# kalgeee/Uncertainty-Aware-Multimodal-Emotion-Recognition

Measured on AMD Instinct MI355X. Metric: samples/sec fwd+bwd at B=4096 (84/256/768-dim), higher is better.
Workload: dtype bf16; 1 GPU; configs[2]: fusion+DEER forward + MultiTaskDEERLoss + backward (dropout 0.3, gradients materialised in the flat buffer), B=4096/GPU, (B,84)+(B,256)+(B,768) bf16 feature blocks, random-init weights; optimiser step excluded as the metric defines (it maintains the packed weight copies and is timed separately); global_batch=4096, parallelism=single

## Files before the change

### uncertainty-aware-multimodal-emotion-recognition_amd/csrc/chain.h

```cpp
#pragma once
#include "common.h"
#include "nig.h"
#include "options.h"

namespace mmdeer {

constexpr int CHAIN_MAX_SEGS = 12;
constexpr int CHAIN_MAX_VECS = 16;
constexpr int CHAIN_VEC_FLOATS = 4864;

struct ChainSeg {
  const bf16_t* W;
  const float* bias;
  bf16_t* stash;
  const float* gamma;
  const float* beta;
  bf16_t* xln;
  float* out32;
  float* mean;
  float* rstd;
  int N, K, ldw;
  int kin_off, nout_off;
  int dcol_off;
  int ld_stash, nout;
  int relu, drop_site, drop_shift, end_layer;
  int mblocks;
  int in_aux;
  int row_group;
  int fold_groups;
  const bf16_t* mask_y;
  int ld_mask, mask_col0;
  float mask_scale;
  const float* lnb_gamma;
  const bf16_t* lnb_y;
  const float* lnb_mean;
  const float* lnb_rstd;
  bf16_t* lnb_dz;
  float* lnb_partial;
  float lnb_mask_scale;
  int residual;
  int res_add, res_dup;
  bf16_t* stash2;
  int stash_split;
};

struct ChainNig {
  int enabled;
  const bf16_t* e2;
  const bf16_t* w3;
  const float* evid;
  const float* targets;
  const float* stats;
  const float* gstats;
  int nblk;
  int nwp;
  bf16_t* dz2;
  float* partial_w;
  float* partial_b;
  float* loss_out;
  int* bin_counts;
  float mask_scale;
  LossCfg cfg;
};

struct ChainNigF {
  int enabled;
  const bf16_t* w3;
  const float* b3;
  int b3_stride;
  float* evid;
  float* nig_out;
  const float* targets;
  float* wstats;
};

struct ChainArgs {
  const bf16_t* X;
  int ldx, K0;
  int B;
  int ts;
  int groups;
  long long group_stride;
  int nseg;
  DropCtx drop;
  const bf16_t* aux_video; const bf16_t* aux_audio; bf16_t* aux_audio_pad;
  int aux_ldv, aux_lda;
  unsigned long long* stamps;
  ChainNig nig;
  ChainNigF nigf;
  ChainSeg seg[CHAIN_MAX_SEGS];
};

inline int chain_samples_per_workgroup(int B) {
  const int forced = opt(OPT_CHAIN_TS);
  return forced == 16 || forced == 32 ? forced : (B > 4096 ? 32 : 16);
}
inline int chain_workgroups(int B) { const int m = chain_samples_per_workgroup(B); return (B + m - 1) / m; }
inline int chain_samples_per_workgroup(const struct ChainArgs& a);
inline int chain_workgroups_max(int B) { return (B + 15) / 16; }

struct RepackJob {
  const bf16_t* src;
  bf16_t* dst;
  int ld_src, rows, cols, cols_valid;
  int transpose;
  int layout;
  int ld_dst, dst_col;
  int gstart;
  int pad_;
};
constexpr int REPACK_MAX = 64;
struct RepackTable { int njobs; int pad_; RepackJob job[REPACK_MAX]; };
int check_repack(RepackTable& t);
int launch_repack(RepackTable& t, hipStream_t s);

void chain_seg_defaults(ChainSeg& s);
int launch_chain(const ChainArgs& a, hipStream_t stream);
inline int chain_samples_per_workgroup(const ChainArgs& a) { return a.ts == 16 || a.ts == 32 ? a.ts : chain_samples_per_workgroup(a.B); }

}
```

### uncertainty-aware-multimodal-emotion-recognition_amd/csrc/chain.hip

```cpp
#include <type_traits>
#include "gemm_kernel.inc"
#include "chain.h"
#include "options.h"
#include "nig_dev.h"
#include "ln_rows.h"

namespace mmdeer {
namespace {

template <int S>
__device__ __forceinline__ void wr_issue(const void* p) {
  static_assert(S >= 0 && S < 8, "ring slots 0..7");
  if constexpr (S == 0)
    asm volatile("global_load_dwordx4 v[248:251], %0, off\n\tglobal_load_dwordx4 v[252:255], %0, off offset:1024" ::"v"(p)
                 : "memory", "v248", "v249", "v250", "v251", "v252", "v253", "v254", "v255");
  else if constexpr (S == 1)
    asm volatile("global_load_dwordx4 v[240:243], %0, off\n\tglobal_load_dwordx4 v[244:247], %0, off offset:1024" ::"v"(p)
                 : "memory", "v240", "v241", "v242", "v243", "v244", "v245", "v246", "v247");
  else if constexpr (S == 2)
    asm volatile("global_load_dwordx4 v[232:235], %0, off\n\tglobal_load_dwordx4 v[236:239], %0, off offset:1024" ::"v"(p)
                 : "memory", "v232", "v233", "v234", "v235", "v236", "v237", "v238", "v239");
  else if constexpr (S == 3)
    asm volatile("global_load_dwordx4 v[224:227], %0, off\n\tglobal_load_dwordx4 v[228:231], %0, off offset:1024" ::"v"(p)
                 : "memory", "v224", "v225", "v226", "v227", "v228", "v229", "v230", "v231");
  else if constexpr (S == 4)
    asm volatile("global_load_dwordx4 v[216:219], %0, off\n\tglobal_load_dwordx4 v[220:223], %0, off offset:1024" ::"v"(p)
                 : "memory", "v216", "v217", "v218", "v219", "v220", "v221", "v222", "v223");
  else if constexpr (S == 5)
    asm volatile("global_load_dwordx4 v[208:211], %0, off\n\tglobal_load_dwordx4 v[212:215], %0, off offset:1024" ::"v"(p)
                 : "memory", "v208", "v209", "v210", "v211", "v212", "v213", "v214", "v215");
  else if constexpr (S == 6)
    asm volatile("global_load_dwordx4 v[200:203], %0, off\n\tglobal_load_dwordx4 v[204:207], %0, off offset:1024" ::"v"(p)
                 : "memory", "v200", "v201", "v202", "v203", "v204", "v205", "v206", "v207");
  else
    asm volatile("global_load_dwordx4 v[192:195], %0, off\n\tglobal_load_dwordx4 v[196:199], %0, off offset:1024" ::"v"(p)
                 : "memory", "v192", "v193", "v194", "v195", "v196", "v197", "v198", "v199");
}
template <int S, int N>
__device__ __forceinline__ void wr_take(u32x4& f0, u32x4& f1) {
  unsigned r0, r1, r2, r3, r4, r5, r6, r7;
#define CH_TAKE(b0, b1, b2, b3, b4, b5, b6, b7)                                                                                  \
  asm volatile("s_waitcnt vmcnt(%8)\n\tv_mov_b32 %0, v" #b0 "\n\tv_mov_b32 %1, v" #b1 "\n\tv_mov_b32 %2, v" #b2 "\n\tv_mov_b32 %3, v" #b3   \
               "\n\tv_mov_b32 %4, v" #b4 "\n\tv_mov_b32 %5, v" #b5 "\n\tv_mov_b32 %6, v" #b6 "\n\tv_mov_b32 %7, v" #b7 "\n\ts_nop 1"         \
               : "=v"(r0), "=v"(r1), "=v"(r2), "=v"(r3), "=v"(r4), "=v"(r5), "=v"(r6), "=v"(r7)                                 \
               : "n"(N)                                                                                                         \
               : "memory")
  if constexpr (S == 0) CH_TAKE(248, 249, 250, 251, 252, 253, 254, 255);
  else if constexpr (S == 1) CH_TAKE(240, 241, 242, 243, 244, 245, 246, 247);
  else if constexpr (S == 2) CH_TAKE(232, 233, 234, 235, 236, 237, 238, 239);
  else if constexpr (S == 3) CH_TAKE(224, 225, 226, 227, 228, 229, 230, 231);
  else if constexpr (S == 4) CH_TAKE(216, 217, 218, 219, 220, 221, 222, 223);
  else if constexpr (S == 5) CH_TAKE(208, 209, 210, 211, 212, 213, 214, 215);
  else if constexpr (S == 6) CH_TAKE(200, 201, 202, 203, 204, 205, 206, 207);
  else CH_TAKE(192, 193, 194, 195, 196, 197, 198, 199);
#undef CH_TAKE
  f0 = u32x4{r0, r1, r2, r3};
  f1 = u32x4{r4, r5, r6, r7};
}

__device__ __forceinline__ unsigned chain_drop_key(unsigned long long seed, unsigned long long off, int site) {
  unsigned k = mix32((unsigned)seed ^ 0x9E3779B9u);
  k = mix32(k ^ (unsigned)(seed >> 32));
  k = mix32(k ^ (unsigned)off);
  k = mix32(k ^ (unsigned)(off >> 32) ^ ((unsigned)site * 0x85EBCA6Bu));
  return k;
}

struct ChainSegK {
  const bf16_t* W;
  int in_aux, nkt;
  int ntiles, kindb;
  int end;
  int N;
  int vec_off, dcol_off, nout_off, site;
  int shift, relu, fold, mblocks;
  int rows_out, kin_off;
  float mask_scale; int has_bias;
  const bf16_t* mask_y;
  int ld_mask, mask_col0;
};
struct ChainEndK {
  bf16_t* stash; bf16_t* xln; float* out32; float* mean; float* rstd;
  int ld_stash, nout, gb_off, has_ln;
  const bf16_t* lnb_y;
  float lnb_mask_scale;
  int res_split;
  bf16_t* stash2;
};
struct ChainVecK {
  const float* src;
  int off, n4;
};
struct ChainRecK { ChainSegK seg; ChainEndK end; };
static_assert(sizeof(ChainSegK) == 96 && sizeof(ChainEndK) == 80 && sizeof(ChainVecK) == 16 && sizeof(ChainRecK) == 176, "table record sizes");

struct ChainKArgs {
  const bf16_t* X;
  int ldx, K0;
  int B, groups;
  long long group_stride;
  int nseg, nvec;
  DropCtx drop;
  unsigned long long* stamps;
  const bf16_t* aux_video; const bf16_t* aux_audio; bf16_t* aux_audio_pad;
  int aux_ldv, aux_lda;
  ChainRecK rec[CHAIN_MAX_SEGS];
  ChainVecK vec[CHAIN_MAX_VECS];
  ChainNig nig;
  ChainNigF nigf;
};
static_assert(__builtin_offsetof(ChainKArgs, rec) % 16 == 0, "tables must be 16-byte aligned");
static_assert(sizeof(ChainKArgs) <= 4096, "kernel arguments are limited to 4 KiB");

struct ChainLnOut {
  bf16_t* stash; bf16_t* xln; float* out32; float* mean; float* rstd;
  int ld_stash, gb_off;
};

__device__ __forceinline__ float half_sum(float v, int lane) { return ln_half_sum(v, lane); }

template <int NKT>
__device__ __forceinline__ void chain_ln(unsigned char* pan, int img, int r, bool valid, long long grow, int lane, const float* vec,
                                         const ChainLnOut& o_, const unsigned char* res) {
  constexpr int KD = NKT * 64, NC = NKT / 4;
  const f32x4* gam = reinterpret_cast<const f32x4*>(vec + o_.gb_off);
  const f32x4* bet = gam + KD / 4;
  const int l32 = lane & 31;
  bf16_t* stash = o_.stash;
  bf16_t* xln = o_.xln;
  float* out32 = o_.out32;
  const int lds_ = o_.ld_stash;
  unsigned char* cell[NC];
  u32x4 raw[NC];
#pragma unroll
  for (int j = 0; j < NC; ++j) {
    const int c = l32 + 32 * j;
    cell[j] = pan + (c >> 3) * img + r * 128 + (((c & 7) ^ (r & 7)) * 16);
    raw[j] = *reinterpret_cast<const u32x4*>(cell[j]);
    if (valid && stash) store_wt16(stash + grow * lds_ + c * 8, raw[j]);
  }
  float x[NC * 8], mu, rs;
  ln_row_stats<NC>(raw, lane, x, mu, rs);
#pragma unroll
  for (int j = 0; j < NC; ++j) {
    const int c = l32 + 32 * j;
    float o[8];
    ln_chunk_out(x + 8 * j, mu, rs, gam[2 * c], gam[2 * c + 1], bet[2 * c], bet[2 * c + 1], o);
    u32x4 packed{pack_bf2(o[0], o[1]), pack_bf2(o[2], o[3]), pack_bf2(o[4], o[5]), pack_bf2(o[6], o[7])};
    if (res) {
      const u32x4 h = *reinterpret_cast<const u32x4*>(res + (cell[j] - pan));
      const unsigned pw[4] = {packed.x, packed.y, packed.z, packed.w}, hw[4] = {h.x, h.y, h.z, h.w};
#pragma unroll
      for (int e = 0; e < 4; ++e) {
        o[2 * e] = __uint_as_float(pw[e] << 16) + __uint_as_float(hw[e] << 16);
        o[2 * e + 1] = __uint_as_float(pw[e] & 0xFFFF0000u) + __uint_as_float(hw[e] & 0xFFFF0000u);
      }
      packed = u32x4{pack_bf2(o[0], o[1]), pack_bf2(o[2], o[3]), pack_bf2(o[4], o[5]), pack_bf2(o[6], o[7])};
    }
    *reinterpret_cast<u32x4*>(cell[j]) = packed;
    if (valid) {
      const long long col = grow * KD + c * 8;
      store_wt16(xln + col, packed);
      if (out32) {
        store_wt16(out32 + col, f32x4{o[0], o[1], o[2], o[3]});
        store_wt16(out32 + col + 4, f32x4{o[4], o[5], o[6], o[7]});
      }
    }
  }
  if (valid && l32 == 0) { o_.mean[grow] = mu; o_.rstd[grow] = rs; }
}

struct ChainLnbIn {
  u32x4 y[2];
  float mu, rs;
};

template <int NKT>
__device__ __forceinline__ void chain_ln_bwd(unsigned char* pan, int img, int lane, int r, bool valid, long long grow, const float* gam,
                                             const ChainLnbIn& in, float ms, bf16_t* dz, float (&gacc)[NKT * 2], float (&bacc)[NKT * 2]) {
  constexpr int KD = NKT * 64, NC = NKT / 4;
  const int l32 = lane & 31;
  unsigned char* cell[NC];
  u32x4 draw[NC], yraw[NC], packed[NC];
  float gg[NC * 8];
#pragma unroll
  for (int j = 0; j < NC; ++j) {
    const int c = l32 + 32 * j;
    cell[j] = pan + (c >> 3) * img + r * 128 + (((c & 7) ^ (r & 7)) * 16);
    draw[j] = *reinterpret_cast<const u32x4*>(cell[j]);
    yraw[j] = in.y[j];
    const f32x4 g0 = *reinterpret_cast<const f32x4*>(gam + 8 * c), g1 = *reinterpret_cast<const f32x4*>(gam + 8 * c + 4);
    gg[8 * j] = g0.x; gg[8 * j + 1] = g0.y; gg[8 * j + 2] = g0.z; gg[8 * j + 3] = g0.w;
    gg[8 * j + 4] = g1.x; gg[8 * j + 5] = g1.y; gg[8 * j + 6] = g1.z; gg[8 * j + 7] = g1.w;
  }
  ln_bwd_row<NC>(draw, yraw, gg, in.mu, in.rs, ms, lane, valid ? 1.f : 0.f, packed, gacc, bacc);
#pragma unroll
  for (int j = 0; j < NC; ++j) {
    const int c = l32 + 32 * j;
    *reinterpret_cast<u32x4*>(cell[j]) = packed[j];
    if (valid) store_wt16(dz + grow * KD + c * 8, packed[j]);
  }
}

template <int NKT>
__device__ __forceinline__ void chain_ln_bwd_fold(float* red, int wave, int lane, int tid, const float (&gacc)[NKT * 2],
                                                  const float (&bacc)[NKT * 2], float* slab) {
  ln_bwd_fold16<NKT / 4>(red, wave, lane, tid, gacc, bacc, slab);
}

template <int MS>
__device__ __forceinline__ void chain_nig_head(const ChainNig& g, unsigned char* pin, float* scratch, int row0, int B, int tid, unsigned long long* stp) {
#ifdef MMDEER_STAMPS
#define NSTAMP(i) do { if (stp && blockIdx.x == 0 && tid == 0) stp[i] = __builtin_readcyclecounter(); } while (0)
#else
#define NSTAMP(i) do {} while (0)
#endif
  NSTAMP(110);
  float* sb = scratch + MS * 195;
  float (*gs)[NIG_NSTAT] = reinterpret_cast<float (*)[NIG_NSTAT]>(sb);     sb += 108;
  f32x4* const sdE = reinterpret_cast<f32x4*>(sb);                           sb += MS * 12;
  Finals& F = *reinterpret_cast<Finals*>(sb);                                sb += (sizeof(Finals) + 15) / 16 * 4;
  float* const ftmp = sb;
  static_assert((MS * 195 + 108 + MS * 12 + (sizeof(Finals) + 15) / 16 * 4 + NIG_FINALS_TMP) * 4 <= MS * 1024, "NIG head scratch exceeds the output panel");
  const int wave = tid >> 6, lane = tid & 63, q = lane & 3;
  const int qw = wave - (8 - 3 * (MS / 16));
  const bool quad_on = qw >= 0;
  const int d = quad_on ? qw % 3 : 0;
  const int r = quad_on ? 16 * (qw / 3) + (lane >> 2) : 0;
  const int b = row0 + r;
  const bool active = quad_on && b < B;
  const int bc = b < B ? b : B - 1;
  const long long o = (long long)bc * 3 + d;
  float w[4][16], x[16];
  f32x4 ev{0.f, 0.f, 0.f, 0.f};
  float y = 0.f;
  Nig n{0.f, 1.f, 2.f, 1.f};
  Terms t{};
  if (quad_on) {
#pragma unroll
    for (int c = 0; c < 4; ++c) load_chunk16<false>(g.w3, d * 256 + c * 64 + q * 16, w[c]);
    load_chunk16<false>(g.e2, (long long)bc * 192 + d * 64 + q * 16, x);
    ev = *reinterpret_cast<const f32x4*>(g.evid + o * 4);
    y = g.targets[o];
    n = nig_act(ev);
    t = loss_terms(n, y);
  }
  const int stat_n = g.gstats ? (int)g.gstats[3 * NIG_NSTAT] : B;
  NSTAMP(111);
  compute_finals(g.gstats ? g.gstats : g.stats, g.gstats ? 1 : g.nblk, stat_n, g.cfg, F, gs, ftmp, g.gstats ? 0 : g.nwp);
  NSTAMP(112);
  if (blockIdx.x == 0 && tid == 0) write_loss(F, g.loss_out, g.bin_counts);
  if (quad_on) {
    const f32x4 gr = loss_grad(n, t, d, stat_n, g.cfg, F);
    f32x4 dE{gr.x, gr.y * softplus_grad(ev.y), gr.z * softplus_grad(ev.z), gr.w * softplus_grad(ev.w)};
    if (!active) dE = f32x4{0.f, 0.f, 0.f, 0.f};
    float dz[16];
    float* xt = scratch + r * 195 + d * 64 + q * 16;
#pragma unroll
    for (int j = 0; j < 16; ++j) {
      xt[j] = active ? x[j] : 0.f;
      const float v = nig_dx(dE, w[0][j], w[1][j], w[2][j], w[3][j]);
      dz[j] = x[j] > 0.f ? v * g.mask_scale : 0.f;
    }
    if (active) store_chunk16<false>(g.dz2, (long long)b * 192 + d * 64 + q * 16, dz);
    unsigned char* prow = pin + d * (MS * 128) + (r >> 3) * 1024 + (r & 7) * 128;
#pragma unroll
    for (int h = 0; h < 2; ++h)
      *reinterpret_cast<nig_u32x4*>(prow + (((2 * q + h) ^ (r & 7)) * 16)) =
          nig_u32x4{pack_bf2(dz[8 * h], dz[8 * h + 1]), pack_bf2(dz[8 * h + 2], dz[8 * h + 3]), pack_bf2(dz[8 * h + 4], dz[8 * h + 5]),
                    pack_bf2(dz[8 * h + 6], dz[8 * h + 7])};
    if (q == 0) sdE[r * 3 + d] = dE;
  }
  asm volatile("s_waitcnt lgkmcnt(0)" ::: "memory");
  __builtin_amdgcn_s_barrier();
  NSTAMP(114);
  for (int e = tid; e < 768; e += 512) {
    const int dd = e >> 8, c = (e >> 6) & 3, j = e & 63;
    const float* sde = reinterpret_cast<const float*>(sdE) + dd * 4 + c;
    float acc0 = 0.f, acc1 = 0.f;
#pragma unroll 8
    for (int s = 0; s < MS; s += 2) {
      acc0 = fmaf(sde[12 * s], scratch[s * 195 + dd * 64 + j], acc0);
      acc1 = fmaf(sde[12 * s + 12], scratch[(s + 1) * 195 + dd * 64 + j], acc1);
    }
    g.partial_w[(long long)blockIdx.x * 768 + e] = acc0 + acc1;
  }
  if (tid < 12) {
    const float* sde = reinterpret_cast<const float*>(sdE) + tid;
    float bs = 0.f;
    for (int s = 0; s < MS; ++s) bs += sde[12 * s];
    g.partial_b[(long long)blockIdx.x * 12 + tid] = bs;
  }
}

template <int MS>
__device__ __forceinline__ void chain_nig_tail(const ChainNigF& g, const unsigned char* pan, int row0, int B, int tid) {
  const int wave = tid >> 6, lane = tid & 63, q = lane & 3;
  const int qw = wave - (8 - 3 * (MS / 16));
  if (qw < 0) return;
  const int d = qw % 3, blk = qw / 3;
  const int r = 16 * blk + (lane >> 2);
  const int b = row0 + r;
  const bool active = b < B;
  const int bc = active ? b : B - 1;
  float w[4][16], x[16];
#pragma unroll
  for (int c = 0; c < 4; ++c) load_chunk16<false>(g.w3, d * 256 + c * 64 + q * 16, w[c]);
  {
    const unsigned char* prow = pan + d * (MS * 128) + r * 128;
#pragma unroll
    for (int h = 0; h < 2; ++h) {
      const u32x4 raw = *reinterpret_cast<const u32x4*>(prow + (((2 * q + h) ^ (r & 7)) * 16));
      const unsigned dw[4] = {raw.x, raw.y, raw.z, raw.w};
#pragma unroll
      for (int e = 0; e < 4; ++e) { x[8 * h + 2 * e] = __uint_as_float(dw[e] << 16); x[8 * h + 2 * e + 1] = __uint_as_float(dw[e] & 0xFFFF0000u); }
    }
  }
  float a0 = 0.f, a1 = 0.f, a2 = 0.f, a3 = 0.f;
#pragma unroll
  for (int j = 0; j < 16; ++j) {
    a0 = fmaf(x[j], w[0][j], a0); a1 = fmaf(x[j], w[1][j], a1);
    a2 = fmaf(x[j], w[2][j], a2); a3 = fmaf(x[j], w[3][j], a3);
  }
  a0 = quad_sum(a0); a1 = quad_sum(a1); a2 = quad_sum(a2); a3 = quad_sum(a3);
  const float* bb = g.b3 + d * g.b3_stride;
  const f32x4 ev{a0 + bb[0], a1 + bb[1], a2 + bb[2], a3 + bb[3]};
  const Nig n = nig_act(ev);
  const bool writer = active && q == 0;
  if (writer) {
    *reinterpret_cast<f32x4*>(g.evid + ((long long)b * 3 + d) * 4) = ev;
    const float alea = n.beta / (n.alpha - 1.f);
    const float epis = n.beta / (n.nu * (n.alpha - 1.f));
    const long long o = (long long)b * 3 + d, plane = (long long)B * 3;
    float* out = g.nig_out;
    out[o] = n.mu; out[plane + o] = n.nu; out[2 * plane + o] = n.alpha; out[3 * plane + o] = n.beta;
    out[4 * plane + o] = alea; out[5 * plane + o] = epis; out[6 * plane + o] = alea + epis;
  }
  if (g.targets) {
    const float y = g.targets[(long long)bc * 3 + d];
    const Terms t = loss_terms(n, y);
    float* slab = g.wstats + ((long long)((row0 >> 4) + blk) * 3 + d) * NIG_NSTAT;
    float v[NIG_NSTAT];
    v[0] = writer ? t.logprob : 0.f; v[1] = writer ? t.reg : 0.f; v[2] = writer ? t.kla : 0.f; v[3] = writer ? t.klb : 0.f; v[4] = writer ? t.u : 0.f;
#pragma unroll
    for (int k = 0; k < 10; ++k) {
      const bool in = writer && t.bin == k;
      v[5 + k] = in ? t.conf : 0.f; v[15 + k] = in ? t.aerr : 0.f; v[25 + k] = in ? 1.f : 0.f;
    }
#pragma unroll
    for (int i = 0; i < NIG_NSTAT; ++i) {
      const float sm = wave_sum(v[i]);
      if (lane == 0) slab[i] = sm;
    }
  }
}

template <int D, int VECF, int TS>
__device__ __forceinline__ void chain_body(const ChainKArgs& a) {
  constexpr int MS = 16 * TS, LOG_MS = TS == 1 ? 4 : 5, FLY = 2 * D;
  constexpr int G = D == 8 ? 4 : D;
  constexpr int PAN = TS == 1 ? MS * 1536 : MS * 1024;
  constexpr int AUXB = TS == 1 ? MS * 768 : 0;
  constexpr int AUX = 2 * PAN, RED = AUX + AUXB, VEC = RED + 32768, TAB = VEC + VECF * 4;
  constexpr int SEG_BYTES = (int)sizeof(ChainRecK);
  constexpr int VEC0 = CHAIN_MAX_SEGS * SEG_BYTES;
  constexpr int TAB_BYTES = VEC0 + CHAIN_MAX_VECS * (int)sizeof(ChainVecK);
  static_assert(TAB_BYTES % 16 == 0 && TAB_BYTES / 16 <= 512, "one 16-byte chunk of the tables per thread");
  static_assert(TAB + TAB_BYTES <= 160 * 1024, "LDS budget");
  __shared__ __attribute__((aligned(1024))) unsigned char lds[TAB + TAB_BYTES];
  float* const vec = reinterpret_cast<float*>(lds + VEC);

  const int tid = threadIdx.x, lane = tid & 63;
  const int wave = __builtin_amdgcn_readfirstlane(tid >> 6);
  const int li = lane & 15, lg = lane >> 4;
  const int r8 = lane >> 3, kchunk = ((lane & 7) ^ r8) * 8;
  const int row0 = blockIdx.x * MS;
  const int B = a.B;
  const long long gstride = a.group_stride;
  const int nseg = a.nseg, nvec = a.nvec;
#ifdef MMDEER_STAMPS
  unsigned long long* const stamps = a.stamps;
  auto stamp = [&](int i) { if (stamps && blockIdx.x == 0 && tid == 0 && i < 512) stamps[i] = __builtin_readcyclecounter(); };
  auto wstamp = [&](int i) { if (stamps && blockIdx.x == 0 && lane == 0 && i < 512) stamps[i] = __builtin_readcyclecounter(); };
#else
  auto stamp = [&](int) {};
  auto wstamp = [&](int) {};
#endif
  stamp(0);

  const unsigned long long dseed = a.drop.seed;
  const unsigned long long doff = a.drop.offset + (a.drop.offset_dev ? *a.drop.offset_dev : 0ull);
  const unsigned dthresh = a.drop.thresh;
  const float dscale = a.drop.scale;

  auto grow_of = [&](int r) -> long long { return (long long)(r >> LOG_MS) * gstride + row0 + (r & (MS - 1)); };
  auto valid_of = [&](int r) -> bool { return row0 + (r & (MS - 1)) < B; };

  const auto& KA = *(const __attribute__((address_space(4))) ChainKArgs*)__builtin_amdgcn_kernarg_segment_ptr();
  u32x4 tabv{0u, 0u, 0u, 0u};
  if (tid < TAB_BYTES / 16) {
    const unsigned char* src = (const unsigned char*)__builtin_amdgcn_kernarg_segment_ptr() + __builtin_offsetof(ChainKArgs, rec) + 16 * tid;
    asm volatile("global_load_dwordx4 %0, %1, off" : "=v"(tabv) : "v"(src) : "memory");
  }
  int rows_in = a.groups * MS;
  const bool nig_in = a.nig.enabled != 0;
  if (!nig_in) {
    const int rg = rows_in >> 3, np = (a.K0 >> 6) * rg;
    const int img = rows_in * 128;
    for (int q = wave; q < np; q += 8) {
      const int image = q / rg, g8 = q - image * rg;
      const int r = g8 * 8 + r8;
      const long long gr = valid_of(r) ? grow_of(r) : (long long)(r >> LOG_MS) * gstride;
      lds_dma16(a.X + gr * a.ldx + image * 64 + kchunk, lds + image * img + g8 * 1024);
    }
  }
  const bool has_aux = AUXB != 0 && a.aux_video != nullptr;
  if (has_aux) {
    {
      const int image = wave >> 1, g8 = wave & 1;
      const int r = g8 * 8 + r8;
      const long long gr = valid_of(r) ? grow_of(r) : 0;
      lds_dma16(a.aux_video + gr * a.aux_ldv + image * 64 + kchunk, lds + AUX + image * (MS * 128) + g8 * 1024);
    }
  }
  stamp(1);
  const unsigned char* const tab = lds + TAB;
  bool tab_ready = false;
  auto sc = [](unsigned v) -> int { return __builtin_amdgcn_readfirstlane((int)v); };
  auto sp = [](unsigned lo, unsigned hi) -> unsigned long long {
    return ((unsigned long long)(unsigned)__builtin_amdgcn_readfirstlane((int)hi) << 32) | (unsigned)__builtin_amdgcn_readfirstlane((int)lo);
  };

  const int rot = blockIdx.x >> 3;
  const int rot2 = rot & 1, rot3 = rot % 3, rot4 = rot & 3;
  auto phys_tile = [&](int nt, int ntl) -> int {
    const int ph = nt + (ntl == 4 ? rot4 : ntl == 3 ? rot3 : ntl == 2 ? rot2 : 0);
    return ph >= ntl ? ph - ntl : ph;
  };

  int p_si = 0, p_nt = 0, p_kt = 0, p_nkt = 0, p_nv = 0, p_ntiles = 0, p_kb = 0;
  const unsigned char* p_W = nullptr;
  const unsigned char* p_cur = nullptr;
  auto p_tile = [&]() __attribute__((always_inline)) {
    const int ph = phys_tile(p_nt, p_ntiles);
    const int wt = p_kb ? ph * 4 + (wave & 3) : ph * 8 + wave;
    p_cur = p_W + ((long long)wt * p_nkt) * 2048 + lane * 16;
  };
  auto p_load = [&]() __attribute__((always_inline)) {
    if (tab_ready) {
      const u32x4* rec = reinterpret_cast<const u32x4*>(tab + p_si * SEG_BYTES);
      const u32x4 q0 = rec[0], q1 = rec[1];
      p_W = reinterpret_cast<const unsigned char*>(sp(q0.x, q0.y));
      p_nkt = sc(q0.w); p_ntiles = sc(q1.x); p_kb = sc(q1.y);
    } else {
      const auto& sk = KA.rec[p_si].seg;
      p_W = reinterpret_cast<const unsigned char*>(sk.W);
      p_nkt = sk.nkt; p_ntiles = sk.ntiles; p_kb = sk.kindb;
    }
    p_nv = (p_nkt + G - 1) / G * G;
    p_nt = 0;
    p_tile();
  };
  auto issue = [&](auto slotc) __attribute__((always_inline)) {
    wr_issue<decltype(slotc)::value>(p_cur);
    if (++p_kt < p_nkt) p_cur += 2048;
    if (p_kt == p_nv) {
      p_kt = 0;
      if (++p_nt == p_ntiles) {
        if (++p_si == nseg) p_si = 0;
        p_load();
      } else {
        p_tile();
      }
    }
  };
  for (int e = wave; e < nvec; e += 8) {
    const float* src = KA.vec[e].src;
    unsigned char* dst = lds + VEC + KA.vec[e].off * 4;
    const int n4 = KA.vec[e].n4;
    for (int j = 0; j * 64 < n4; ++j) {
      if (src) { if (j * 64 + lane < n4) lds_dma16(src + 4 * (j * 64 + lane), dst + j * 1024); }
      else if (j * 64 + lane < n4) *reinterpret_cast<f32x4*>(dst + j * 1024 + lane * 16) = f32x4{0.f, 0.f, 0.f, 0.f};
    }
  }
  p_load();
  issue(std::integral_constant<int, 0>{});
  issue(std::integral_constant<int, 1>{});
  if constexpr (D >= 4) { issue(std::integral_constant<int, 2>{}); issue(std::integral_constant<int, 3>{}); }
  if constexpr (D == 8) {
    issue(std::integral_constant<int, 4>{}); issue(std::integral_constant<int, 5>{});
    issue(std::integral_constant<int, 6>{}); issue(std::integral_constant<int, 7>{});
  }
  if (has_aux) {
#pragma unroll
    for (int q = 0; q < 2; ++q) {
      const int e = tid + 512 * q, r = e >> 6, dw = e & 63;
      unsigned v = 0u;
      if (dw * 2 < a.aux_lda && valid_of(r)) v = *reinterpret_cast<const unsigned*>(a.aux_audio + grow_of(r) * a.aux_lda + 2 * dw);
      const int chunk = dw >> 2;
      *reinterpret_cast<unsigned*>(lds + AUX + (4 + (chunk >> 3)) * (MS * 128) + r * 128 + (((chunk & 7) ^ (r & 7)) * 16) + (dw & 3) * 4) = v;
    }
  }
  if (nig_in) {
    chain_nig_head<MS>(a.nig, lds, reinterpret_cast<float*>(lds + PAN), row0, B, tid, a.stamps);
    stamp(115);
  }
  asm volatile("s_waitcnt vmcnt(%1)" : "+v"(tabv) : "n"(FLY) : "memory");
  if (tid < TAB_BYTES / 16) *reinterpret_cast<u32x4*>(lds + TAB + 16 * tid) = tabv;
  tab_ready = true;
  asm volatile("s_waitcnt lgkmcnt(0)" ::: "memory");
  __builtin_amdgcn_s_barrier();
  stamp(2);
  if (has_aux && tid < 256) {
    const int r = tid >> 4, c = tid & 15;
    const u32x4 v = *reinterpret_cast<const u32x4*>(lds + AUX + (4 + (c >> 3)) * (MS * 128) + r * 128 + (((c & 7) ^ (r & 7)) * 16));
    if (valid_of(r)) store_wt16(a.aux_audio_pad + grow_of(r) * 128 + c * 8, v);
  }

  unsigned char* pin = lds;
  unsigned char* pout = lds + PAN;
  const int swz0 = (lg ^ (li & 7)) * 16, swz1 = ((4 + lg) ^ (li & 7)) * 16;

  struct SegCtl { int in_aux, N, ntiles, vec_off, dcol_off, nout_off, site, shift, relu, fold, kin_off, rows_out, has_bias, ld_mask, mask_col0; float mask_scale; const bf16_t* mask_y; };

  auto seg_body = [&](auto mbc, auto kbc, auto nktc, auto h0c, const SegCtl& sg) __attribute__((always_inline)) -> int {
    constexpr int MB = decltype(mbc)::value;
    constexpr bool KB = decltype(kbc)::value;
    constexpr int NKT = decltype(nktc)::value;
    constexpr int H0 = decltype(h0c)::value;
    constexpr int NV = (NKT + G - 1) / G * G;
    constexpr bool FLIP = D == 8 && ((NV / G) & 1) != 0;
    const bool active = !KB || wave < 4;
    const int img_in = sg.in_aux ? MS * 128 : rows_in * 128, img_out = sg.rows_out * 128;
    constexpr bool AFR_REG = TS == 1;
    const unsigned char* const sa = (sg.in_aux ? lds + AUX : pin) + (sg.kin_off >> 6) * img_in + li * 128;
    u32x4 afr[AFR_REG ? NKT * 2 : 1][MB];
    if constexpr (AFR_REG) {
#pragma unroll
      for (int c = 0; c < NKT * 2; ++c)
#pragma unroll
        for (int i = 0; i < MB; ++i) afr[c][i] = *reinterpret_cast<const u32x4*>(sa + (c >> 1) * img_in + i * 2048 + ((c & 1) ? swz1 : swz0));
    }
    u32x4 fr[2][2][MB];
    auto frag_load = [&](auto ktc) __attribute__((always_inline)) {
      constexpr int kt = decltype(ktc)::value;
#pragma unroll
      for (int i = 0; i < MB; ++i) {
        fr[kt & 1][0][i] = *reinterpret_cast<const u32x4*>(sa + kt * img_in + i * 2048 + swz0);
        fr[kt & 1][1][i] = *reinterpret_cast<const u32x4*>(sa + kt * img_in + i * 2048 + swz1);
      }
    };
    const int site = sg.site, shift = sg.shift, relu = sg.relu, fold = sg.fold & 15, N = sg.N;
    const bool res_add = (sg.fold & 16) != 0, res_dup = (sg.fold & 32) != 0;
    const unsigned dkey = site >= 0 ? chain_drop_key(dseed, doff, site) : 0u;
    auto tile = [&](auto hc, int nti) __attribute__((always_inline)) {
      constexpr int HS = decltype(hc)::value * G;
      const int nt = phys_tile(nti, sg.ntiles);
      f32x4 acc[MB];
#pragma unroll
      for (int i = 0; i < MB; ++i) acc[i] = f32x4{0.f, 0.f, 0.f, 0.f};
      u32x2 mk[MB];
      const bf16_t* mask_y = sg.mask_y;
      if (mask_y && active) {
        const int n0m = sg.mask_col0 + (KB ? nt * 64 : nt * 128) + 16 * wave + 4 * lg;
#pragma unroll
        for (int i = 0; i < MB; ++i) {
          const int r = 16 * i + li;
          const long long gr = valid_of(r) ? grow_of(r) : (long long)(r >> LOG_MS) * gstride;
          const bf16_t* q = mask_y + gr * sg.ld_mask + n0m;
          asm volatile("global_load_dwordx2 %0, %1, off" : "=v"(mk[i]) : "v"(q) : "memory");
        }
      }
      auto stage = [&](auto ktc) __attribute__((always_inline)) {
        constexpr int kt = decltype(ktc)::value;
        constexpr int S = (HS + kt) % D;
        if constexpr (kt < NKT) {
          u32x4 f0{0u, 0u, 0u, 0u}, f1{0u, 0u, 0u, 0u};
          if (active) wr_take<S, FLY - 2>(f0, f1);
          else wait_vm<FLY - 2>();
          issue(std::integral_constant<int, S>{});
          if constexpr (!AFR_REG && kt + 1 < NKT) { if (active) frag_load(std::integral_constant<int, kt + 1>{}); }
          if (active) {
            if constexpr (AFR_REG) {
#pragma unroll
              for (int i = 0; i < MB; ++i) acc[i] = mma_chunk<bf16_t>(f0, afr[2 * kt][i], acc[i]);
#pragma unroll
              for (int i = 0; i < MB; ++i) acc[i] = mma_chunk<bf16_t>(f1, afr[2 * kt + 1][i], acc[i]);
            } else {
#pragma unroll
              for (int i = 0; i < MB; ++i) acc[i] = mma_chunk<bf16_t>(f0, fr[kt & 1][0][i], acc[i]);
#pragma unroll
              for (int i = 0; i < MB; ++i) acc[i] = mma_chunk<bf16_t>(f1, fr[kt & 1][1][i], acc[i]);
            }
          }
        } else {
          wait_vm<FLY - 2>();
          issue(std::integral_constant<int, S>{});
        }
      };
      if constexpr (!AFR_REG) { if (active) frag_load(std::integral_constant<int, 0>{}); }
      stage(std::integral_constant<int, 0>{});
      if constexpr (NV > 1) stage(std::integral_constant<int, 1>{});
      if constexpr (NV > 2) stage(std::integral_constant<int, 2>{});
      if constexpr (NV > 3) stage(std::integral_constant<int, 3>{});
      if constexpr (NV > 4) stage(std::integral_constant<int, 4>{});
      if constexpr (NV > 5) stage(std::integral_constant<int, 5>{});
      if constexpr (NV > 6) stage(std::integral_constant<int, 6>{});
      if constexpr (NV > 7) stage(std::integral_constant<int, 7>{});
      if constexpr (NV > 8) stage(std::integral_constant<int, 8>{});
      if constexpr (NV > 9) stage(std::integral_constant<int, 9>{});
      if constexpr (NV > 10) stage(std::integral_constant<int, 10>{});
      if constexpr (NV > 11) stage(std::integral_constant<int, 11>{});
      if (active) {
        const int n0 = (KB ? nt * 64 : nt * 128) + 16 * wave + 4 * lg;
        const f32x4 bias4 = sg.has_bias ? *reinterpret_cast<const f32x4*>(vec + sg.vec_off + n0) : f32x4{0.f, 0.f, 0.f, 0.f};
        const unsigned dcol = (unsigned)(sg.dcol_off + n0);
        const int colb = sg.nout_off + n0;
        if (mask_y) {
#pragma unroll
          for (int i = 0; i < MB; ++i) asm volatile("s_waitcnt vmcnt(%1)" : "+v"(mk[i]) : "n"(2 * NV < FLY ? 2 * NV : FLY) : "memory");
        }
#pragma unroll
        for (int i = 0; i < MB; ++i) {
          const int r = 16 * i + li;
          f32x4 v = acc[i] + bias4;
          if (relu) { v.x = fmaxf(v.x, 0.f); v.y = fmaxf(v.y, 0.f); v.z = fmaxf(v.z, 0.f); v.w = fmaxf(v.w, 0.f); }
          if (site >= 0) {
            const unsigned rk = ((unsigned)grow_of(r) * 0x9E3779B1u) ^ dkey;
            if (shift == 0) {
              v.x = mix32(rk ^ (dcol * 0x85EBCA77u)) < dthresh ? v.x * dscale : 0.f;
              v.y = mix32(rk ^ ((dcol + 1) * 0x85EBCA77u)) < dthresh ? v.y * dscale : 0.f;
              v.z = mix32(rk ^ ((dcol + 2) * 0x85EBCA77u)) < dthresh ? v.z * dscale : 0.f;
              v.w = mix32(rk ^ ((dcol + 3) * 0x85EBCA77u)) < dthresh ? v.w * dscale : 0.f;
            } else {
              const float f = mix32(rk ^ ((dcol >> shift) * 0x85EBCA77u)) < dthresh ? dscale : 0.f;
              v.x *= f; v.y *= f; v.z *= f; v.w *= f;
            }
          }
          if (mask_y) {
            const float ms = sg.mask_scale;
            const unsigned m0 = mk[i].x, m1 = mk[i].y;
            v.x = __uint_as_float(m0 << 16) > 0.f ? v.x * ms : 0.f; v.y = __uint_as_float(m0 & 0xFFFF0000u) > 0.f ? v.y * ms : 0.f;
            v.z = __uint_as_float(m1 << 16) > 0.f ? v.z * ms : 0.f; v.w = __uint_as_float(m1 & 0xFFFF0000u) > 0.f ? v.w * ms : 0.f;
          }
          int col = colb, orow = r;
          if (fold == 1) { col += (r >> LOG_MS) * N; orow = r & (MS - 1); }
          else if (fold == 2) { const int half = N >> 1, z = col >= half; col -= z * half; orow = r + z * MS; }
          else if (fold == 3) orow = r + MS;
          const int cell_off = (col >> 6) * img_out + orow * 128 + ((((col & 63) >> 3) ^ (orow & 7)) * 16) + (col & 4) * 2;
          if (res_add) {
            const u32x2 h = *reinterpret_cast<const u32x2*>(pin + cell_off + 4 * img_out);
            const unsigned p0 = pack_bf2(v.x, v.y), p1 = pack_bf2(v.z, v.w);
            v.x = __uint_as_float(p0 << 16) + __uint_as_float(h.x << 16); v.y = __uint_as_float(p0 & 0xFFFF0000u) + __uint_as_float(h.x & 0xFFFF0000u);
            v.z = __uint_as_float(p1 << 16) + __uint_as_float(h.y << 16); v.w = __uint_as_float(p1 & 0xFFFF0000u) + __uint_as_float(h.y & 0xFFFF0000u);
          }
          const u32x2 pk{pack_bf2(v.x, v.y), pack_bf2(v.z, v.w)};
          *reinterpret_cast<u32x2*>(pout + cell_off) = pk;
          if (res_dup) *reinterpret_cast<u32x2*>(pout + cell_off + 4 * img_out) = pk;
        }
      }
    };
    if constexpr (!FLIP) {
      for (int nti = 0; nti < sg.ntiles; ++nti) tile(std::integral_constant<int, H0>{}, nti);
      return H0;
    } else {
      for (int nti = 0; nti < sg.ntiles; nti += 2) {
        tile(std::integral_constant<int, H0>{}, nti);
        if (nti + 1 < sg.ntiles) tile(std::integral_constant<int, 1 - H0>{}, nti + 1);
      }
      return (sg.ntiles & 1) ? 1 - H0 : H0;
    }
  };

  int half = 0;
  u32x4 R[11];
  auto fetch_rec = [&](int si_) __attribute__((always_inline)) {
    const u32x4* rec = reinterpret_cast<const u32x4*>(tab + si_ * SEG_BYTES);
#pragma unroll
    for (int k = 0; k < 11; ++k) R[k] = rec[k];
  };
  fetch_rec(0);
  for (int si = 0; si < nseg; ++si) {
    const u32x4 q0 = R[0], q1 = R[1], q2 = R[2], q3 = R[3], q4 = R[4], q5 = R[5];
    const u32x4 e0 = R[6], e1 = R[7], e2 = R[8], e3 = R[9], e4 = R[10];
    const int nkt = sc(q0.w), kb = sc(q1.y), endi = sc(q1.z);
    SegCtl sg;
    sg.ntiles = sc(q1.x); sg.N = sc(q1.w); sg.in_aux = sc(q0.z);
    sg.vec_off = sc(q2.x); sg.dcol_off = sc(q2.y); sg.nout_off = sc(q2.z); sg.site = sc(q2.w);
    sg.shift = sc(q3.x); sg.relu = sc(q3.y); sg.fold = sc(q3.z);
    const int mb = sc(q3.w);
    sg.rows_out = sc(q4.x); sg.kin_off = sc(q4.y);
    sg.mask_scale = __uint_as_float((unsigned)sc(q4.z)); sg.has_bias = sc(q4.w);
    sg.mask_y = reinterpret_cast<const bf16_t*>(sp(q5.x, q5.y)); sg.ld_mask = sc(q5.z); sg.mask_col0 = sc(q5.w);
    bf16_t* const stash = reinterpret_cast<bf16_t*>(sp(e0.x, e0.y));
    bf16_t* const end_xln = reinterpret_cast<bf16_t*>(sp(e0.z, e0.w));
    float* const end_out32 = reinterpret_cast<float*>(sp(e1.x, e1.y));
    float* const end_mean = reinterpret_cast<float*>(sp(e1.z, e1.w));
    float* const end_rstd = reinterpret_cast<float*>(sp(e2.x, e2.y));
    const int ld_stash = sc(e2.z), nout = sc(e2.w);
    const int gb_off = sc(e3.x), has_ln = endi >= 0 ? sc(e3.y) : 0;
    const bf16_t* const end_lnb_y = reinterpret_cast<const bf16_t*>(sp(e3.z, e3.w));
    const float lms = __uint_as_float((unsigned)sc(e4.x));
    const int res_split = endi >= 0 ? sc(e4.y) : 0;
    bf16_t* const stash2 = reinterpret_cast<bf16_t*>(sp(e4.z, e4.w));
    ChainLnbIn lnb[TS];
#pragma unroll
    for (int ps = 0; ps < TS; ++ps) { lnb[ps].y[0] = lnb[ps].y[1] = u32x4{0u, 0u, 0u, 0u}; lnb[ps].mu = 0.f; lnb[ps].rs = 0.f; }
    auto lnb_fetch = [&]() __attribute__((always_inline)) {
      const bf16_t* ly = end_lnb_y;
      const float* lmean = end_mean;
      const float* lrstd = end_rstd;
#pragma unroll
      for (int ps = 0; ps < TS; ++ps) {
        const int r = 16 * ps + 2 * wave + (lane >> 5);
        const long long gr = valid_of(r) ? grow_of(r) : 0;
        const bf16_t* q = ly + gr * nout + (lane & 31) * 8;
        asm volatile("global_load_dwordx4 %0, %1, off" : "=v"(lnb[ps].y[0]) : "v"(q) : "memory");
        if (nout == 512) asm volatile("global_load_dwordx4 %0, %1, off offset:512" : "=v"(lnb[ps].y[1]) : "v"(q) : "memory");
        asm volatile("global_load_dword %0, %1, off" : "=v"(lnb[ps].mu) : "v"(lmean + gr) : "memory");
        asm volatile("global_load_dword %0, %1, off" : "=v"(lnb[ps].rs) : "v"(lrstd + gr) : "memory");
      }
    };
    if (TS == 1 && has_ln == 2) lnb_fetch();
    stamp(3 + 3 * si);
#define CH_SEG1(MBv, KBv, NKTv, Hv) seg_body(std::integral_constant<int, MBv>{}, std::integral_constant<bool, KBv>{}, std::integral_constant<int, NKTv>{}, std::integral_constant<int, Hv>{}, sg)
#define CH_SEG(MBv, KBv, NKTv) do { if constexpr (D == 8) { if (half) half = CH_SEG1(MBv, KBv, NKTv, 1); else half = CH_SEG1(MBv, KBv, NKTv, 0); } else CH_SEG1(MBv, KBv, NKTv, 0); } while (0)
    if (!kb) {
      if (mb == TS) {
        if (nkt == 8) CH_SEG(TS, false, 8); else if (nkt == 6) CH_SEG(TS, false, 6); else if (nkt == 4) CH_SEG(TS, false, 4);
        else if (nkt == 2) CH_SEG(TS, false, 2); else if (nkt == 1) CH_SEG(TS, false, 1);
        else { if constexpr (TS == 1) CH_SEG(TS, false, 12); }
      } else {
        if (nkt == 4) CH_SEG(2 * TS, false, 4); else if (nkt == 2) CH_SEG(2 * TS, false, 2); else CH_SEG(2 * TS, false, 1);
      }
    } else {
      if (mb == TS) { if (nkt == 4) CH_SEG(TS, true, 4); else CH_SEG(TS, true, 2); }
      else CH_SEG(2 * TS, true, 2);
    }
#undef CH_SEG
#undef CH_SEG1
    stamp(4 + 3 * si);
    fetch_rec(si + 1 < nseg ? si + 1 : 0);
    if (endi >= 0) {
      const int rows_out = sg.rows_out, img_out = rows_out * 128;
      wstamp(200 + 8 * si + wave);
      asm volatile("s_waitcnt lgkmcnt(0)" ::: "memory");
      __builtin_amdgcn_s_barrier();
      stamp(130 + 4 * si);
      if (has_ln == 2) {
        stamp(100);
        if constexpr (TS == 1) {
          if (2 * sg.ntiles * ((nkt + G - 1) / G * G) >= FLY)
            asm volatile("s_waitcnt vmcnt(%4)" : "+v"(lnb[0].y[0]), "+v"(lnb[0].y[1]), "+v"(lnb[0].mu), "+v"(lnb[0].rs) : "n"(FLY) : "memory");
          else
            asm volatile("s_waitcnt vmcnt(%4)" : "+v"(lnb[0].y[0]), "+v"(lnb[0].y[1]), "+v"(lnb[0].mu), "+v"(lnb[0].rs) : "n"(2 * G) : "memory");
        } else {
          lnb_fetch();
#pragma unroll
          for (int ps = 0; ps < TS; ++ps)
            asm volatile("s_waitcnt vmcnt(0)" : "+v"(lnb[ps].y[0]), "+v"(lnb[ps].y[1]), "+v"(lnb[ps].mu), "+v"(lnb[ps].rs) : : "memory");
        }
        stamp(101);
        bf16_t* dz = end_xln;
        float* slab = end_out32 + (long long)blockIdx.x * 2 * nout;
        if (stash) {
          const int nch = nout >> 3;
          for (int rr = wave; rr < rows_out; rr += 8) {
            if (!valid_of(rr)) continue;
            for (int cc = lane; cc < nch; cc += 64)
              store_wt16(stash + grow_of(rr) * ld_stash + cc * 8,
                         *reinterpret_cast<const u32x4*>(pout + (cc >> 3) * img_out + rr * 128 + (((cc & 7) ^ (rr & 7)) * 16)));
          }
          asm volatile("s_waitcnt lgkmcnt(0)" ::: "memory");
          __builtin_amdgcn_s_barrier();
        }
        stamp(102);
        if (nout == 512) {
          float gacc[16], bacc[16];
#pragma unroll
          for (int e = 0; e < 16; ++e) gacc[e] = bacc[e] = 0.f;
#pragma unroll
          for (int ps = 0; ps < TS; ++ps) {
            const int r = 16 * ps + 2 * wave + (lane >> 5);
            chain_ln_bwd<8>(pout, img_out, lane, r, valid_of(r), grow_of(r), vec + gb_off, lnb[ps], lms, dz, gacc, bacc);
          }
          stamp(104);
          chain_ln_bwd_fold<8>(reinterpret_cast<float*>(lds + RED), wave, lane, tid, gacc, bacc, slab);
        } else {
          float gacc[8], bacc[8];
#pragma unroll
          for (int e = 0; e < 8; ++e) gacc[e] = bacc[e] = 0.f;
#pragma unroll
          for (int ps = 0; ps < TS; ++ps) {
            const int r = 16 * ps + 2 * wave + (lane >> 5);
            chain_ln_bwd<4>(pout, img_out, lane, r, valid_of(r), grow_of(r), vec + gb_off, lnb[ps], lms, dz, gacc, bacc);
          }
          chain_ln_bwd_fold<4>(reinterpret_cast<float*>(lds + RED), wave, lane, tid, gacc, bacc, slab);
        }
        stamp(103);
      } else if (has_ln) {
        const unsigned char* const ln_res = (res_split & 1) ? pin : nullptr;
        ChainLnOut o;
        o.stash = stash; o.xln = end_xln; o.out32 = end_out32;
        o.mean = end_mean; o.rstd = end_rstd;
        o.ld_stash = ld_stash; o.gb_off = gb_off;
        for (int r = 2 * wave + (lane >> 5); r < rows_out; r += 16) {
          if (nout == 512) chain_ln<8>(pout, img_out, r, valid_of(r), grow_of(r), lane, vec, o, ln_res);
          else chain_ln<4>(pout, img_out, r, valid_of(r), grow_of(r), lane, vec, o, ln_res);
        }
      } else if (stash) {
        const int nch = nout >> 3;
        const int split_ch = (res_split >> 4) ? (res_split >> 7) : nch;
        constexpr int NR = 4 * TS;
        const bool wide = TS == 1 && nch > 64;
        u32x4 raw[NR];
#pragma unroll
        for (int q = 0; q < NR; ++q) {
          const int r = wide && q >= NR / 2 ? wave + 8 * (q - NR / 2) : wave + 8 * q;
          const int c = wide && q >= NR / 2 ? lane + 64 : lane;
          if (r < rows_out && c < nch) raw[q] = *reinterpret_cast<const u32x4*>(pout + (c >> 3) * img_out + r * 128 + (((c & 7) ^ (r & 7)) * 16));
        }
        stamp(132 + 4 * si);
#pragma unroll
        for (int q = 0; q < NR; ++q) {
          const int r = wide && q >= NR / 2 ? wave + 8 * (q - NR / 2) : wave + 8 * q;
          const int c = wide && q >= NR / 2 ? lane + 64 : lane;
          if (r < rows_out && c < nch && valid_of(r)) {
            if (c < split_ch) store_wt16(stash + grow_of(r) * ld_stash + c * 8, raw[q]);
            else store_wt16(stash2 + grow_of(r) * ld_stash + (c - split_ch) * 8, raw[q]);
          }
        }
      }
      stamp(131 + 4 * si);
      if (has_ln) {
        asm volatile("s_waitcnt lgkmcnt(0)" ::: "memory");
        __builtin_amdgcn_s_barrier();
      }
      unsigned char* t = pin; pin = pout; pout = t;
      rows_in = rows_out;
    }
    stamp(5 + 3 * si);
  }
  if (a.nigf.enabled) chain_nig_tail<MS>(a.nigf, pin, row0, B, tid);
  asm volatile("s_waitcnt vmcnt(0)" ::: "memory");
}

__global__ __launch_bounds__(512) __attribute__((amdgpu_num_vgpr(112))) void chain_kernel_s16(const ChainKArgs a) {
  chain_body<4, CHAIN_VEC_FLOATS, 1>(a);
}
__global__ __launch_bounds__(512) __attribute__((amdgpu_num_vgpr(96))) void chain_kernel_s16_d8(const ChainKArgs a) {
  chain_body<8, CHAIN_VEC_FLOATS, 1>(a);
}
__global__ __launch_bounds__(512) __attribute__((amdgpu_num_vgpr(120))) void chain_kernel_s32(const ChainKArgs a) {
  chain_body<2, CHAIN_VEC_FLOATS, 2>(a);
}
__global__ __launch_bounds__(512) __attribute__((amdgpu_num_vgpr(120))) void chain_kernel_s16_d2(const ChainKArgs a) {
  chain_body<2, CHAIN_VEC_FLOATS, 1>(a);
}

}

namespace {
__global__ __launch_bounds__(256) void repack_kernel(const RepackTable t) {
  int j = 0;
  while (j + 1 < t.njobs && (int)blockIdx.x * 256 >= t.job[j + 1].gstart) ++j;
  const RepackJob& J = t.job[j];
  const int l = blockIdx.x * 256 + threadIdx.x - J.gstart;
  const int R = J.transpose ? J.cols : J.rows, Cn = J.transpose ? J.rows : J.cols;
  if (l >= R * (Cn >> 3)) return;
  int r, c0;
  bf16_t* dst;
  if (J.layout == 1) {
    const int nkt = Cn >> 6, lane = l & 63, c = (l >> 6) & 1, rest = l >> 7;
    const int kt = rest % nkt, wt = rest / nkt;
    r = wt * 16 + (lane & 15); c0 = kt * 64 + c * 32 + (lane >> 4) * 8;
    dst = J.dst + (size_t)l * 8;
  } else {
    const int per = Cn >> 3;
    int dr;
    if (J.transpose) { dr = l % R; c0 = (l / R) * 8; }
    else { dr = l / per; c0 = (l - dr * per) * 8; }
    r = dr;
    if (J.layout == 2) {
      const int h = dr / 192, rem = dr - h * 192, wn = rem / 96, rem2 = rem - wn * 96, part = rem2 >> 5, dd = rem2 & 31;
      r = part * 512 + h * 64 + wn * 32 + dd;
    }
    dst = J.dst + (size_t)dr * J.ld_dst + J.dst_col + c0;
  }
  u32x4 v;
  if (!J.transpose && J.cols_valid == J.cols && (J.ld_src & 7) == 0) {
    v = *reinterpret_cast<const u32x4*>(J.src + (size_t)r * J.ld_src + c0);
  } else {
    unsigned short e[8];
#pragma unroll
    for (int q = 0; q < 8; ++q) {
      const int rr = J.transpose ? c0 + q : r, cc = J.transpose ? r : c0 + q;
      e[q] = cc < J.cols_valid ? J.src[(size_t)rr * J.ld_src + cc] : (unsigned short)0;
    }
    v = u32x4{(unsigned)e[0] | ((unsigned)e[1] << 16), (unsigned)e[2] | ((unsigned)e[3] << 16), (unsigned)e[4] | ((unsigned)e[5] << 16),
              (unsigned)e[6] | ((unsigned)e[7] << 16)};
  }
  *reinterpret_cast<u32x4*>(dst) = v;
}
}

int check_repack(RepackTable& t) {
  MMDEER_CHECK(t.njobs >= 0 && t.njobs <= REPACK_MAX, "repack: too many jobs (%d)", t.njobs);
  int g = 0;
  for (int m = 0; m < t.njobs; ++m) {
    RepackJob& J = t.job[m];
    const int R = J.transpose ? J.cols : J.rows, Cn = J.transpose ? J.rows : J.cols;
    MMDEER_CHECK(J.src && J.dst && ((uintptr_t)J.dst % 16) == 0 && J.rows > 0 && J.cols > 0 && J.cols_valid <= J.cols, "repack: job %d pointers / sizes", m);
    MMDEER_CHECK(Cn % 8 == 0 && (J.layout != 1 || (R % 16 == 0 && Cn % 64 == 0)), "repack: job %d is %d x %d", m, R, Cn);
    MMDEER_CHECK(J.layout == 1 || (J.ld_dst % 8 == 0 && J.dst_col % 8 == 0), "repack: job %d destination alignment", m);
    MMDEER_CHECK(J.layout != 2 || (!J.transpose && J.rows == 1536 && J.cols == 512), "repack: the head-major order is that of the [1536][512] in_proj");
    J.gstart = g;
    g += (R * (Cn >> 3) + 255) / 256 * 256;
  }
  return g;
}

int launch_repack(RepackTable& t, hipStream_t s) {
  const int g = check_repack(t);
  if (g <= 0) return g;
  hipLaunchKernelGGL(repack_kernel, dim3((g + 255) / 256), dim3(256), 0, s, t);
  MMDEER_HIP(hipGetLastError());
  return 0;
}

void chain_seg_defaults(ChainSeg& s) {
  s = ChainSeg{};
  s.drop_site = -1;
}

int launch_chain(const ChainArgs& a, hipStream_t stream) {
  MMDEER_CHECK(a.nseg >= 1 && a.nseg <= CHAIN_MAX_SEGS, "chain: 1..%d segments (got %d)", CHAIN_MAX_SEGS, a.nseg);
  if (a.nig.enabled) {
    const ChainNig& g = a.nig;
    MMDEER_CHECK(a.K0 == 192 && a.groups == 1, "chain: the NIG head produces 192-wide input rows of one group");
    MMDEER_CHECK(g.e2 && g.w3 && g.evid && g.targets && (g.stats || g.gstats) && g.dz2 && g.partial_w && g.partial_b && g.nblk >= 1,
                 "chain: NIG head: NULL argument");
    MMDEER_CHECK(((uintptr_t)g.e2 % 16) == 0 && ((uintptr_t)g.w3 % 16) == 0 && ((uintptr_t)g.evid % 16) == 0 && ((uintptr_t)g.dz2 % 16) == 0,
                 "chain: NIG head: pointers must be 16-byte aligned");
  } else {
    MMDEER_CHECK(a.X && ((uintptr_t)a.X % 16) == 0 && a.ldx % 8 == 0, "chain: input rows must be 16-byte aligned");
    MMDEER_CHECK(a.ldx >= a.K0, "chain: ldx = %d is shorter than the input width K0 = %d", a.ldx, a.K0);
  }
  MMDEER_CHECK(a.B > 0, "chain: empty batch");
  MMDEER_CHECK(a.groups == 1 || a.groups == 2, "chain: groups must be 1 or 2");
  const int msamp = chain_samples_per_workgroup(a);
  const int ts = msamp / 16;
  const int nwg = (a.B + msamp - 1) / msamp;
  const int pan_cols = ts == 1 ? 768 : 512;
  MMDEER_CHECK(a.K0 % 64 == 0 && a.K0 * a.groups <= pan_cols, "chain: input width %d x %d groups does not fit the panel", a.K0, a.groups);
  if (a.aux_video) {
    MMDEER_CHECK(ts == 1 && !a.nig.enabled && a.groups == 1, "chain: the second input panel needs 16-sample workgroups and a single-group input");
    MMDEER_CHECK(a.aux_audio && a.aux_audio_pad && ((uintptr_t)a.aux_video % 16) == 0 && a.aux_ldv % 8 == 0 && ((uintptr_t)a.aux_audio % 4) == 0 &&
                     a.aux_lda % 2 == 0 && a.aux_lda <= 128 && ((uintptr_t)a.aux_audio_pad % 16) == 0,
                 "chain: second input panel: pointers / alignment");
  }
  ChainKArgs k{};
  k.aux_video = a.aux_video; k.aux_audio = a.aux_audio; k.aux_audio_pad = a.aux_audio_pad; k.aux_ldv = a.aux_ldv; k.aux_lda = a.aux_lda;
  k.X = a.X; k.ldx = a.ldx; k.K0 = a.K0; k.B = a.B; k.groups = a.groups; k.group_stride = a.group_stride; k.drop = a.drop;
  k.stamps = a.stamps;
  k.nig = a.nig;
  k.nigf = a.nigf;
  if (a.nigf.enabled) {
    const ChainSeg& last = a.seg[a.nseg - 1];
    MMDEER_CHECK(!a.nig.enabled && last.end_layer && last.nout == 192 && !last.gamma && !last.lnb_gamma && last.fold_groups == 0,
                 "chain: the NIG tail needs a plain 192-wide last layer");
    MMDEER_CHECK(a.nigf.w3 && a.nigf.b3 && a.nigf.evid && a.nigf.nig_out && (!a.nigf.targets || a.nigf.wstats) &&
                     ((uintptr_t)a.nigf.w3 % 16) == 0 && ((uintptr_t)a.nigf.evid % 16) == 0,
                 "chain: NIG tail: NULL argument / alignment");
  }
  int vec = 0, nend = 0, nvec = 0;
  int blocks_in = a.groups * ts, width_in = a.K0, layer_first_seg = 0;
  bool layer_has_group1 = false, width_in_dup = false;
  auto add_vec = [&](const float* src, int n) { ChainVecK& v = k.vec[nvec++]; v.src = src; v.off = vec; v.n4 = n / 4; vec += n; return v.off; };
  for (int i = 0; i < a.nseg; ++i) {
    const ChainSeg& s = a.seg[i];
    MMDEER_CHECK(s.W && ((uintptr_t)s.W % 16) == 0, "chain: segment %d weights (fragment-major image) must be 16-byte aligned", i);
    MMDEER_CHECK(s.N > 0 && s.N % 64 == 0 && s.K > 0 && s.K % 64 == 0 && (s.N % 128 == 0 || s.K % 128 == 0),
                 "chain: segment %d has unsupported N = %d, K = %d", i, s.N, s.K);
    MMDEER_CHECK(!s.in_aux || a.aux_video, "chain: segment %d reads a second input panel the chain does not have", i);
    MMDEER_CHECK(s.kin_off >= 0 && s.kin_off % 64 == 0 && s.kin_off + s.K <= (s.in_aux ? 384 : width_in), "chain: segment %d reads columns [%d, %d) of a %d-wide panel", i,
                 s.kin_off, s.kin_off + s.K, s.in_aux ? 384 : width_in);
    MMDEER_CHECK(s.row_group == 0 || (s.row_group == 1 && s.fold_groups == 0 && blocks_in == ts), "chain: segment %d row group", i);
    MMDEER_CHECK(s.nout_off >= 0 && s.nout_off % 64 == 0, "chain: segment %d output offset", i);
    MMDEER_CHECK(s.drop_shift >= 0 && s.drop_shift < 32, "chain: segment %d drop_shift = %d", i, s.drop_shift);
    MMDEER_CHECK(!s.bias || ((uintptr_t)s.bias % 16) == 0, "chain: segment %d bias alignment", i);
    const int mblocks = s.in_aux ? ts : s.mblocks ? s.mblocks : blocks_in;
    layer_has_group1 = layer_has_group1 || s.row_group == 1;
    MMDEER_CHECK(mblocks <= blocks_in && (mblocks == ts || mblocks == 2 * ts), "chain: segment %d m-blocks", i);
    const int seg_vecs = (s.bias ? 1 : 0) + (!s.end_layer ? 0 : s.lnb_gamma ? 1 : s.gamma ? 2 : 0);
    MMDEER_CHECK(nvec + seg_vecs <= CHAIN_MAX_VECS, "chain: more than %d bias / gamma / beta vectors", CHAIN_MAX_VECS);
    const int vec_off = s.bias ? add_vec(s.bias, s.N) : 0;
    const int kb = s.N % 128 != 0, ntl = kb ? s.N / 64 : s.N / 128, nkt = s.K / 64;
    MMDEER_CHECK(ntl <= 4, "chain: segment %d has too many column tiles", i);
    MMDEER_CHECK(kb ? ((nkt == 2 || nkt == 4) && mblocks * nkt <= 4 * ts)
                    : (((nkt == 1 || nkt == 2 || nkt == 4 || nkt == 6 || nkt == 8) && mblocks * nkt <= 8 * ts) || (nkt == 12 && ts == 1 && mblocks == 1)),
                 "chain: segment %d: K = %d with %d row blocks is not instantiated", i, s.K, mblocks);
    ChainSegK& td = k.rec[i].seg;
    td.W = s.W; td.in_aux = s.in_aux ? 1 : 0; td.nkt = nkt; td.ntiles = ntl; td.kindb = kb; td.end = -1;
    td.N = s.N; td.vec_off = vec_off; td.dcol_off = s.dcol_off; td.nout_off = s.nout_off;
    td.site = s.drop_site; td.shift = s.drop_shift; td.relu = s.relu; td.fold = s.row_group == 1 ? 3 : s.fold_groups;
    if (s.res_add || s.res_dup) {
      MMDEER_CHECK(td.fold == 0 && s.N == 256 && s.nout_off == 0 && blocks_in == ts && !s.in_aux, "chain: segment %d: residual epilogue on a 256-wide single-group layer only", i);
      MMDEER_CHECK(!s.res_add || width_in_dup, "chain: segment %d adds a bypass copy the layer above did not write", i);
      td.fold |= (s.res_add ? 16 : 0) | (s.res_dup ? 32 : 0);
    }
    td.mblocks = mblocks; td.kin_off = s.kin_off;
    td.has_bias = s.bias != nullptr;
    td.mask_y = s.mask_y; td.ld_mask = s.ld_mask; td.mask_col0 = s.mask_col0; td.mask_scale = s.mask_scale;
    MMDEER_CHECK(!s.mask_y || (((uintptr_t)s.mask_y % 8) == 0 && s.ld_mask % 4 == 0 && s.mask_col0 % 4 == 0), "chain: segment %d mask alignment", i);
    MMDEER_CHECK(!s.mask_y || (s.mask_col0 >= 0 && s.ld_mask >= s.mask_col0 + s.N), "chain: segment %d reads mask columns [%d, %d) of rows of ld_mask = %d",
                 i, s.mask_col0, s.mask_col0 + s.N, s.ld_mask);
    if (s.end_layer) {
      const int blocks_out = s.fold_groups == 1 ? blocks_in / 2 : (s.fold_groups == 2 || layer_has_group1) ? blocks_in * 2 : blocks_in;
      layer_has_group1 = false;
      MMDEER_CHECK(s.fold_groups != 1 || blocks_in == 2 * ts, "chain: segment %d folds the groups of a single-group panel", i);
      MMDEER_CHECK(s.fold_groups != 2 || (blocks_in == ts && s.nout_off == 0 && s.N == 2 * s.nout && s.nout % 64 == 0),
                   "chain: segment %d unfolds: one row group, N = 2 x the panel width", i);
      MMDEER_CHECK(s.nout % 64 == 0 && s.nout * blocks_out <= pan_cols * ts, "chain: layer ending at segment %d does not fit the panel", i);
      for (int t = layer_first_seg; t <= i; ++t)
        MMDEER_CHECK(a.seg[t].fold_groups != 0 || a.seg[t].nout_off + a.seg[t].N <= s.nout, "chain: segment %d writes columns [%d, %d) of a %d-wide panel",
                     t, a.seg[t].nout_off, a.seg[t].nout_off + a.seg[t].N, s.nout);
      for (int t = layer_first_seg; t <= i; ++t)
        MMDEER_CHECK(!(a.seg[t].res_add || a.seg[t].res_dup) || (layer_first_seg == i && s.nout == 256),
                     "chain: segment %d: a residual epilogue needs a 256-wide layer of that one segment", t);
      MMDEER_CHECK(!s.stash || (((uintptr_t)s.stash % 16) == 0 && s.ld_stash % 8 == 0), "chain: segment %d stash alignment", i);
      MMDEER_CHECK(!s.stash_split || (s.stash && !s.gamma && !s.lnb_gamma), "chain: segment %d: stash_split needs a plain stash (no LayerNorm)", i);
      {
        const int hi = s.nout - s.stash_split, stored = s.stash_split > 0 ? (s.stash_split > hi ? s.stash_split : hi) : s.nout;
        MMDEER_CHECK(!s.stash || s.ld_stash >= stored, "chain: segment %d: ld_stash = %d is shorter than the %d stored columns", i, s.ld_stash, stored);
      }
      ChainEndK& e = k.rec[i].end;
      e.stash = s.stash; e.ld_stash = s.ld_stash; e.nout = s.nout;
      if (s.lnb_gamma) {
        MMDEER_CHECK(!s.gamma && (s.nout == 256 || s.nout == 512) && blocks_out == ts, "chain: LayerNorm backward of segment %d: width %d, one row group", i, s.nout);
        MMDEER_CHECK(s.lnb_y && s.lnb_mean && s.lnb_rstd && s.lnb_dz && s.lnb_partial && ((uintptr_t)s.lnb_gamma % 16) == 0 &&
                         ((uintptr_t)s.lnb_y % 16) == 0 && ((uintptr_t)s.lnb_dz % 16) == 0 && ((uintptr_t)s.lnb_partial % 16) == 0,
                     "chain: LayerNorm backward of segment %d: pointers / alignment", i);
        e.has_ln = 2; e.xln = s.lnb_dz; e.out32 = s.lnb_partial; e.mean = const_cast<float*>(s.lnb_mean); e.rstd = const_cast<float*>(s.lnb_rstd);
        e.lnb_y = s.lnb_y; e.lnb_mask_scale = s.lnb_mask_scale;
        e.gb_off = add_vec(s.lnb_gamma, s.nout);
      } else if (s.gamma) {
        MMDEER_CHECK(s.nout == 256 || s.nout == 512, "chain: LayerNorm width %d", s.nout);
        MMDEER_CHECK(s.beta && s.xln && s.mean && s.rstd && ((uintptr_t)s.gamma % 16) == 0 && ((uintptr_t)s.beta % 16) == 0 &&
                         ((uintptr_t)s.xln % 16) == 0 && (!s.out32 || ((uintptr_t)s.out32 % 16) == 0),
                     "chain: LayerNorm of segment %d: pointers / alignment", i);
        e.has_ln = 1; e.xln = s.xln; e.out32 = s.out32; e.mean = s.mean; e.rstd = s.rstd;
        MMDEER_CHECK(!s.residual || (blocks_out == blocks_in && s.nout == width_in), "chain: residual LayerNorm of segment %d: the layer must keep the panel's geometry", i);
        e.res_split = s.residual ? 1 : 0;
        e.gb_off = add_vec(s.gamma, s.nout);
        add_vec(s.beta, s.nout);
      }
      else if (s.stash && s.stash_split) {
        MMDEER_CHECK(s.stash2 && ((uintptr_t)s.stash2 % 16) == 0 && s.stash_split % 8 == 0 && s.stash_split > 0 && s.stash_split < s.nout,
                     "chain: segment %d stash split", i);
        e.res_split = s.stash_split << 4; e.stash2 = s.stash2;
      }
      td.end = nend++;
      for (int t = layer_first_seg; t <= i; ++t) k.rec[t].seg.rows_out = blocks_out * 16;
      layer_first_seg = i + 1;
      blocks_in = blocks_out; width_in = s.nout; width_in_dup = s.res_dup != 0;
    }
  }
  MMDEER_CHECK(a.seg[a.nseg - 1].end_layer, "chain: the last segment must end its layer");
  MMDEER_CHECK(vec <= CHAIN_VEC_FLOATS, "chain: %d bias / gamma / beta floats exceed the LDS area (%d)", vec, CHAIN_VEC_FLOATS);
  k.nseg = a.nseg; k.nvec = nvec;
  if (ts == 1 && opt(OPT_CHAIN_DEPTH) == 2) hipLaunchKernelGGL(chain_kernel_s16_d2, dim3(nwg), dim3(512), 0, stream, k);
  else if (ts == 1 && opt(OPT_CHAIN_DEPTH) == 8) hipLaunchKernelGGL(chain_kernel_s16_d8, dim3(nwg), dim3(512), 0, stream, k);
  else if (ts == 1) hipLaunchKernelGGL(chain_kernel_s16, dim3(nwg), dim3(512), 0, stream, k);
  else hipLaunchKernelGGL(chain_kernel_s32, dim3(nwg), dim3(512), 0, stream, k);
  MMDEER_HIP(hipGetLastError());
  return 0;
}

}
```

### uncertainty-aware-multimodal-emotion-recognition_amd/csrc/common.h

```cpp
#pragma once
#include <hip/hip_runtime.h>
#include <stdint.h>

#include <initializer_list>

namespace mmdeer {

typedef unsigned short bf16_t;
typedef __bf16 bf16x8 __attribute__((ext_vector_type(8)));
typedef float f32x4 __attribute__((ext_vector_type(4)));

template <typename V2>
__device__ __forceinline__ void store_wt8(void* p, V2 v) {
  static_assert(sizeof(V2) == 8, "store_wt8 writes 8 bytes");
  asm volatile("global_store_dwordx2 %0, %1, off sc0 sc1" ::"v"(p), "v"(v) : "memory");
}
template <typename V4>
__device__ __forceinline__ void store_wt16(void* p, V4 v) {
  static_assert(sizeof(V4) == 16, "store_wt16 writes 16 bytes");
  asm volatile("global_store_dwordx4 %0, %1, off sc0 sc1\n\ts_nop 1" ::"v"(p), "v"(v) : "memory");
}

enum { DT_BF16 = 0, DT_F32 = 1 };

__device__ __forceinline__ float bf2f(bf16_t h) { return __uint_as_float(((unsigned)h) << 16); }
__device__ __forceinline__ bf16_t f2bf(float f) { return __builtin_bit_cast(unsigned short, (__bf16)f); }
typedef float f32x2_t __attribute__((ext_vector_type(2)));
typedef __bf16 bf16x2_t __attribute__((ext_vector_type(2)));
__device__ __forceinline__ unsigned pack_bf2(float lo, float hi) {
  return __builtin_bit_cast(unsigned, __builtin_convertvector(f32x2_t{lo, hi}, bf16x2_t));
}

template <typename T> struct Elem;
template <> struct Elem<float> {
  static constexpr int EPC = 4;
  static constexpr int KT = 32;
};
template <> struct Elem<bf16_t> {
  static constexpr int EPC = 8;
  static constexpr int KT = 64;
};

typedef unsigned Rand4 __attribute__((ext_vector_type(4)));

__host__ __device__ __forceinline__ unsigned mix32(unsigned x) {
  x ^= x >> 16; x *= 0x7FEB352Du;
  x ^= x >> 15; x *= 0x846CA68Bu;
  x ^= x >> 16;
  return x;
}

struct DropCtx {
  unsigned long long seed;
  unsigned long long offset;
  unsigned thresh;
  float scale;
  const unsigned long long* offset_dev;
};
DropCtx make_drop(float p, uint64_t seed, uint64_t offset, const uint64_t* offset_dev = nullptr);

__host__ __device__ __forceinline__ unsigned drop_key(const DropCtx& d, int site) {
  unsigned long long off = d.offset;
#if defined(__HIP_DEVICE_COMPILE__)
  if (d.offset_dev) off += *d.offset_dev;
#endif
  unsigned k = mix32((unsigned)d.seed ^ 0x9E3779B9u);
  k = mix32(k ^ (unsigned)(d.seed >> 32));
  k = mix32(k ^ (unsigned)off);
  k = mix32(k ^ (unsigned)(off >> 32) ^ ((unsigned)site * 0x85EBCA6Bu));
  return k;
}
__host__ __device__ __forceinline__ unsigned drop_rand1(unsigned key, unsigned row, unsigned c) {
  return mix32((row * 0x9E3779B1u) ^ (c * 0x85EBCA77u) ^ key);
}
__host__ __device__ __forceinline__ Rand4 drop_rand4(const DropCtx& d, int site, unsigned row, unsigned cq) {
  const unsigned key = drop_key(d, site), r = row * 0x9E3779B1u;
  return Rand4{mix32(r ^ ((4 * cq) * 0x85EBCA77u) ^ key), mix32(r ^ ((4 * cq + 1) * 0x85EBCA77u) ^ key),
               mix32(r ^ ((4 * cq + 2) * 0x85EBCA77u) ^ key), mix32(r ^ ((4 * cq + 3) * 0x85EBCA77u) ^ key)};
}
__device__ __forceinline__ f32x4 drop4(f32x4 v, unsigned rk, unsigned dcol, int shift, const DropCtx& dc) {
  if (shift == 0) {
    v.x = mix32(rk ^ (dcol * 0x85EBCA77u)) < dc.thresh ? v.x * dc.scale : 0.f;
    v.y = mix32(rk ^ ((dcol + 1) * 0x85EBCA77u)) < dc.thresh ? v.y * dc.scale : 0.f;
    v.z = mix32(rk ^ ((dcol + 2) * 0x85EBCA77u)) < dc.thresh ? v.z * dc.scale : 0.f;
    v.w = mix32(rk ^ ((dcol + 3) * 0x85EBCA77u)) < dc.thresh ? v.w * dc.scale : 0.f;
  } else {
    const float f = mix32(rk ^ ((dcol >> shift) * 0x85EBCA77u)) < dc.thresh ? dc.scale : 0.f;
    v.x *= f; v.y *= f; v.z *= f; v.w *= f;
  }
  return v;
}
__host__ __device__ __forceinline__ bool drop_keep(const DropCtx& d, int site, unsigned row, unsigned c) {
  return drop_rand1(drop_key(d, site), row, c) < d.thresh;
}

enum DropSite {
  SITE_AV_ATTN = 1,
  SITE_AV_FUSE = 2,
  SITE_TRI_ATTN = 3,
  SITE_TRI_FUSE = 4,
  SITE_OUT_PROJ = 5,
  SITE_FP0 = 6,
  SITE_FP1 = 7,
  SITE_EV0 = 8,
  SITE_EV1 = 9,
};

template <int CTRL, int ROW_MASK = 0xF>
__device__ __forceinline__ float dpp_read(float v) {
  return __builtin_bit_cast(float, __builtin_amdgcn_update_dpp(0, __builtin_bit_cast(int, v), CTRL, ROW_MASK, 0xF, true));
}
__device__ __forceinline__ float quad_sum(float v) {
  v += dpp_read<0xB1>(v);
  v += dpp_read<0x4E>(v);
  return v;
}
__device__ __forceinline__ float oct_sum(float v) {
  v = quad_sum(v);
  return v + dpp_read<0x141>(v);
}
__device__ __forceinline__ float row_sum(float v) {
  v = oct_sum(v);
  return v + dpp_read<0x140>(v);
}
__device__ __forceinline__ float wave_sum(float v) {
  v = row_sum(v);
  v += dpp_read<0x142, 0xA>(v);
  v += dpp_read<0x143, 0xC>(v);
  return __builtin_bit_cast(float, __builtin_amdgcn_readlane(__builtin_bit_cast(int, v), 63));
}

__device__ __forceinline__ float mad2(float a, float x, float b, float y) { return fmaf(a, x, b * y); }
__device__ __forceinline__ f32x4 mad2(float a, f32x4 x, float b, f32x4 y) {
  return f32x4{mad2(a, x.x, b, y.x), mad2(a, x.y, b, y.y), mad2(a, x.z, b, y.z), mad2(a, x.w, b, y.w)};
}

void set_error(const char* fmt, ...);
#define MMDEER_CHECK(cond, ...)            \
  do {                                     \
    if (!(cond)) {                         \
      ::mmdeer::set_error(__VA_ARGS__);    \
      return -1;                           \
    }                                      \
  } while (0)
#define MMDEER_HIP(call)                                                           \
  do {                                                                             \
    hipError_t e_ = (call);                                                        \
    if (e_ != hipSuccess) {                                                        \
      ::mmdeer::set_error("%s failed: %s (%s:%d)", #call, hipGetErrorString(e_), __FILE__, __LINE__); \
      return -1;                                                                   \
    }                                                                              \
  } while (0)
#define TRY(x) do { if ((x) != 0) return -1; } while (0)

#define MMDEER_LAUNCH_ACT_LDS(kernel, act_f32, grid, block, lds, stream, ...)                     \
  do {                                                                                            \
    if (act_f32) hipLaunchKernelGGL(kernel<true>, grid, block, lds, stream, __VA_ARGS__);         \
    else hipLaunchKernelGGL(kernel<false>, grid, block, lds, stream, __VA_ARGS__);                \
    MMDEER_HIP(hipGetLastError());                                                                \
  } while (0)
#define MMDEER_LAUNCH_ACT(kernel, act_f32, grid, block, stream, ...) \
  MMDEER_LAUNCH_ACT_LDS(kernel, act_f32, grid, block, 0, stream, __VA_ARGS__)

inline bool al4(const void* p) { return ((uintptr_t)p & 3) == 0; }
inline bool al8(const void* p) { return ((uintptr_t)p & 7) == 0; }
inline bool al16(const void* p) { return ((uintptr_t)p & 15) == 0; }
inline bool al_act4(int act_f32, std::initializer_list<const void*> ps) {
  for (const void* p : ps)
    if (!(act_f32 ? al16(p) : al8(p))) return false;
  return true;
}

}
```

### uncertainty-aware-multimodal-emotion-recognition_amd/csrc/layout.inc

```
X(W, ACT,  wpack,    MMDEER_FLAT_ELEMS, 0)
X(W, ACT,  wtpack,   MMDEER_FLAT_ELEMS, 0)
X(W, F32,  vpack,    MMDEER_FLAT_ELEMS, 0)
X(W, BF16, wa_pad,   INTER * AUD_PAD, 0)
X(W, BF16, wqkv_hm,  3 * FUS * FUS, 0)
X(W, F32,  wscratch, ADAM_NPART, 0)
X(W, BF16, wfpack,   MMDEER_FLAT_ELEMS, 1)
X(W, BF16, wtfpack,  MMDEER_FLAT_ELEMS, 1)
X(W, BF16, wa_frag,  INTER * AUD_PAD, 1)
X(S, BF16, audio_pad, Bz * AUD_PAD, 0)
X(S, ACT, avin, 2 * Bz * INTER, 0) X(S, ACT, avv, 2 * Bz * INTER, 0) X(S, ACT, cat, Bz * 2 * INTER, 0) X(S, ACT, y_a2, Bz * INTER, 0)
X(S, ACT, av, Bz * INTER, 0) X(S, ACT, xtok, 2 * Bz * FUS, 0) X(S, ACT, qkv, 2 * Bz * 3 * FUS, 0) X(S, ACT, obar, Bz * FUS, 0)
X(S, ACT, pool, Bz * FUS, 0) X(S, ACT, y_t3, Bz * FUS, 0) X(S, ACT, tri, Bz * FUS, 0) X(S, ACT, y_o1, Bz * FUS, 0) X(S, ACT, fused, Bz * FUS, 0)
X(S, ACT, h1, Bz * HID, 0) X(S, ACT, h2, Bz * HID, 0) X(S, ACT, e1, Bz * 3 * EV1, 0) X(S, ACT, e2, Bz * 3 * EV2, 0)
X(S, F32, probs, Bz * 8 * 4, 0) X(S, F32, evid, Bz * 12, 0)
X(S, F32, stats, 4 * nblk * 3 * NIG_NSTAT, 0)
X(S, F32, mean_a2, Bz, 0) X(S, F32, rstd_a2, Bz, 0) X(S, F32, mean_t3, Bz, 0) X(S, F32, rstd_t3, Bz, 0) X(S, F32, mean_o1, Bz, 0) X(S, F32, rstd_o1, Bz, 0)
X(S, ACT, dz2, Bz * 3 * EV2, 0) X(S, ACT, de1, Bz * 3 * EV1, 0) X(S, ACT, dh2, Bz * HID, 0) X(S, ACT, dh1, Bz * HID, 0)
X(S, ACT, dfused, Bz * FUS, 0) X(S, ACT, dz_o1, Bz * FUS, 0) X(S, ACT, dtri, Bz * FUS, 0) X(S, ACT, dz_t3, Bz * FUS, 0)
X(S, ACT, dpool, Bz * FUS, 0) X(S, ACT, dobar, Bz * FUS, 0) X(S, ACT, dqkv, 2 * Bz * 3 * FUS, 0) X(S, ACT, dxtok, 2 * Bz * FUS, 0)
X(S, ACT, dav, Bz * INTER, 0) X(S, ACT, dz_a2, Bz * INTER, 0) X(S, ACT, dcats, 2 * Bz * INTER, 0) X(S, ACT, davv, 2 * Bz * INTER, 0)
X(S, ACT, davin, 2 * Bz * INTER, 0)
X(S, F32, part_ln_o1, np * 2 * FUS, 0) X(S, F32, part_ln_t3, np * 2 * FUS, 0) X(S, F32, part_ln_a2, np * 2 * INTER, 0)
X(S, F32, part_w3, nhead * 3 * 256, 0) X(S, F32, part_b3, nhead * 3 * 4, 0)
X(S, F32, slab, SPLITK_MAX * MMDEER_FLAT_ELEMS, 0)
```

### uncertainty-aware-multimodal-emotion-recognition_amd/csrc/nig.h

```cpp
#pragma once
#include "common.h"

struct mmdeer_loss_cfg;

namespace mmdeer {

constexpr int NIG_NSTAT = 35;
constexpr int NIG_GLOBAL_STATS = 3 * NIG_NSTAT + 1;
constexpr int NIG_LOSS_OUT = 20;

struct LossCfg {
  float reg_w, kl_w, ece_w, cross_w;
  float task_w[3];
};
LossCfg loss_cfg(const mmdeer_loss_cfg& c);

constexpr int NIG_ROWS = 64;
inline int nig_nblocks(int B) { return B > 0 ? (B + NIG_ROWS - 1) / NIG_ROWS : 1; }

int launch_nig_fwd(const void* e2, const void* w3, const float* b3, int b3_stride, float* evid, float* nig_out,
                   const float* targets, float* stats, int B, int act_f32, hipStream_t s);

int launch_nig_bwd(const void* e2, const void* w3, const float* evid, const float* targets, const float* stats,
                   const float* gstats, const float* gmu, const float* gnu, const float* galpha, const float* gbeta,
                   float* devid, void* dz2, float* partial_w, float* partial_b, float* loss_out, int* bin_counts,
                   int B, int act_f32, float mask_scale, const LossCfg& cfg, int nwp, hipStream_t s);

int launch_nig_stats_sum(const float* stats, int B, float* out, int nwp, hipStream_t s);

int launch_nig_loss_stats(const float* gamma, const float* nu, const float* alpha, const float* beta,
                          const float* targets, float* stats, int B, hipStream_t s);
int launch_nig_loss_grad(const float* gamma, const float* nu, const float* alpha, const float* beta,
                         const float* targets, const float* stats, float* dgamma, float* dnu, float* dalpha,
                         float* dbeta, float* loss_out, int* bin_counts, int B, const LossCfg& cfg, hipStream_t s);

int deer_v1_nblocks(long long n);
int launch_deer_loss_v1(const float* mu, const float* nu, const float* alpha, const float* beta, const float* targets, long long n,
                        float ew, float kw, float* loss_out, float* dmu, float* dnu, float* dalpha, float* dbeta, float* partial,
                        hipStream_t s);
int launch_unc_reg_loss(const float* alpha, const float* beta, int B, int D, float dw, float sw, float* loss_out, float* dalpha,
                        float* dbeta, hipStream_t s);
constexpr int CAL_MAX_BINS = 32;
int launch_calibration_loss(const float* gamma, const float* alpha, const float* beta, const float* targets, long long n,
                            float* loss_out, int* bin_counts, float* dgamma, float* dalpha, float* dbeta, const float* edges,
                            int n_bins, hipStream_t s);

#ifdef MMDEER_STAMPS
int debug_nig_stamps(unsigned long long* out16);
#endif

}
```

### uncertainty-aware-multimodal-emotion-recognition_amd/csrc/nig.hip

```cpp
#include "nig.h"
#include "stamps.h"

namespace mmdeer {
namespace {
#ifdef MMDEER_STAMPS
__device__ unsigned long long g_nig_stamps[16];
#define GSTAMP(slot) MMDEER_STAMP((unsigned long long*)g_nig_stamps, slot, blockIdx.x == 0 && blockIdx.y == 0 && threadIdx.x == 0)
#endif
}
}
#include "nig_dev.h"

namespace mmdeer {
namespace {



template <bool F32>
__global__ __launch_bounds__(256) void nig_fwd_kernel(const void* e2, const void* w3, const float* b3, int b3_stride,
                                                      float* evid, float* nig_out, const float* targets, float* stats, int B) {
  const int d = blockIdx.y, tid = threadIdx.x, q = tid & 3;
  const int b = blockIdx.x * NIG_ROWS + (tid >> 2);
  const bool active = b < B;
  const int bc = active ? b : B - 1;
  float w[4][16];
#pragma unroll
  for (int c = 0; c < 4; ++c) load_chunk16<F32>(w3, d * 256 + c * 64 + q * 16, w[c]);
  float x[16];
  load_chunk16<F32>(e2, (long long)bc * 192 + d * 64 + q * 16, x);
  float a0 = 0.f, a1 = 0.f, a2 = 0.f, a3 = 0.f;
#pragma unroll
  for (int j = 0; j < 16; ++j) {
    a0 = fmaf(x[j], w[0][j], a0); a1 = fmaf(x[j], w[1][j], a1);
    a2 = fmaf(x[j], w[2][j], a2); a3 = fmaf(x[j], w[3][j], a3);
  }
  a0 = quad_sum(a0); a1 = quad_sum(a1); a2 = quad_sum(a2); a3 = quad_sum(a3);
  const float* bb = b3 + d * b3_stride;
  const f32x4 ev{a0 + bb[0], a1 + bb[1], a2 + bb[2], a3 + bb[3]};
  const Nig n = nig_act(ev);
  const bool writer = active && q == 0;
  if (writer) {
    *reinterpret_cast<f32x4*>(evid + ((long long)b * 3 + d) * 4) = ev;
    const float alea = n.beta / (n.alpha - 1.f);
    const float epis = n.beta / (n.nu * (n.alpha - 1.f));
    const long long o = (long long)b * 3 + d, plane = (long long)B * 3;
    nig_out[o] = n.mu; nig_out[plane + o] = n.nu; nig_out[2 * plane + o] = n.alpha; nig_out[3 * plane + o] = n.beta;
    nig_out[4 * plane + o] = alea; nig_out[5 * plane + o] = epis; nig_out[6 * plane + o] = alea + epis;
  }
  if (targets) {
    const float y = targets[(long long)bc * 3 + d];
    const Terms t = loss_terms(n, y);
    block_stats(t, writer, stats + ((long long)blockIdx.x * 3 + d) * NIG_NSTAT);
  }
}

template <bool F32>
__global__ __launch_bounds__(256) void nig_bwd_kernel(const void* e2, const void* w3, const float* evid, const float* targets,
                                                      const float* stats, const float* gstats, const float* gmu,
                                                      const float* gnu, const float* galpha, const float* gbeta, float* devid, void* dz2,
                                                      float* partial_w, float* partial_b, float* loss_out,
                                                      int* bin_counts, int B, float mask_scale, LossCfg cfg, int nwp) {
  __shared__ float gs[3][NIG_NSTAT];
  __shared__ float ftmp[NIG_FINALS_TMP];
  __shared__ f32x4 sdE[NIG_ROWS];
  __shared__ Finals F;
  __shared__ float xt[NIG_ROWS][65];
  const int d = blockIdx.y, tid = threadIdx.x, q = tid & 3, s = tid >> 2;
  const int nblk = gridDim.x;
  const int b = blockIdx.x * NIG_ROWS + s;
  const bool active = b < B;
  const int bc = active ? b : B - 1;
  const long long o = (long long)bc * 3 + d;
  GSTAMP(0);
  float w[4][16];
#pragma unroll
  for (int c = 0; c < 4; ++c) load_chunk16<F32>(w3, d * 256 + c * 64 + q * 16, w[c]);
  float x[16];
  load_chunk16<F32>(e2, (long long)bc * 192 + d * 64 + q * 16, x);
  const f32x4 ev = *reinterpret_cast<const f32x4*>(evid + o * 4);
  const bool loss_mode = targets != nullptr;
  f32x4 g{0.f, 0.f, 0.f, 0.f};
  if (loss_mode) {
    const float y = targets[o];
    GSTAMP(1);
    const int stat_n = gstats ? (int)gstats[3 * NIG_NSTAT] : B;
    compute_finals(gstats ? gstats : stats, gstats ? 1 : nblk, stat_n, cfg, F, gs, ftmp, gstats ? 0 : nwp);
    GSTAMP(2);
    if (blockIdx.x == 0 && blockIdx.y == 0 && tid == 0) write_loss(F, loss_out, bin_counts);
    const Nig n = nig_act(ev);
    const Terms t = loss_terms(n, y);
    g = loss_grad(n, t, d, stat_n, cfg, F);
    GSTAMP(3);
  } else {
    if (gmu) g.x = gmu[o];
    if (gnu) g.y = gnu[o];
    if (galpha) g.z = galpha[o];
    if (gbeta) g.w = gbeta[o];
  }
  f32x4 dE{g.x, g.y * softplus_grad(ev.y), g.z * softplus_grad(ev.z), g.w * softplus_grad(ev.w)};
  if (!active) dE = f32x4{0.f, 0.f, 0.f, 0.f};
  if (active && q == 0 && devid) *reinterpret_cast<f32x4*>(devid + o * 4) = dE;
  float dz[16];
#pragma unroll
  for (int j = 0; j < 16; ++j) {
    xt[s][q * 16 + j] = active ? x[j] : 0.f;
    const float v = nig_dx(dE, w[0][j], w[1][j], w[2][j], w[3][j]);
    dz[j] = x[j] > 0.f ? v * mask_scale : 0.f;
  }
  if (active) store_chunk16<F32>(dz2, (long long)b * 192 + d * 64 + q * 16, dz);
  if (q == 0) sdE[s] = dE;
  GSTAMP(4);
  __syncthreads();
  {
    const int c = tid >> 6, j = tid & 63;
    float acc0 = 0.f, acc1 = 0.f;
    const float* sde = reinterpret_cast<const float*>(sdE) + c;
#pragma unroll 8
    for (int r = 0; r < NIG_ROWS; r += 2) {
      acc0 = fmaf(sde[4 * r], xt[r][j], acc0);
      acc1 = fmaf(sde[4 * r + 4], xt[r + 1][j], acc1);
    }
    partial_w[((long long)blockIdx.x * 3 + d) * 256 + tid] = acc0 + acc1;
    if (j < 1) {
      float bs = 0.f;
      for (int r = 0; r < NIG_ROWS; ++r) bs += sde[4 * r];
      partial_b[((long long)blockIdx.x * 3 + d) * 4 + c] = bs;
    }
  }
  GSTAMP(5);
}

__global__ __launch_bounds__(256) void nig_loss_stats_kernel(const float* gamma, const float* nu, const float* alpha,
                                                             const float* beta, const float* targets, float* stats, int B) {
  const int d = blockIdx.y, b = blockIdx.x * 256 + threadIdx.x;
  const bool active = b < B;
  Nig n{0.f, 1.f, 2.f, 1.f};
  float y = 0.f;
  if (active) {
    const long long o = (long long)b * 3 + d;
    n = Nig{gamma[o], nu[o], alpha[o], beta[o]};
    y = targets[o];
  }
  const Terms t = loss_terms(n, y);
  block_stats(t, active, stats + ((long long)blockIdx.x * 3 + d) * NIG_NSTAT);
}

__global__ __launch_bounds__(256) void nig_loss_grad_kernel(const float* gamma, const float* nu, const float* alpha,
                                                            const float* beta, const float* targets, const float* stats,
                                                            float* dgamma, float* dnu, float* dalpha, float* dbeta,
                                                            float* loss_out, int* bin_counts, int B, LossCfg cfg) {
  __shared__ float gs[3][NIG_NSTAT];
  __shared__ float ftmp[NIG_FINALS_TMP];
  __shared__ Finals F;
  compute_finals(stats, gridDim.x, B, cfg, F, gs, ftmp);
  if (blockIdx.x == 0 && blockIdx.y == 0 && threadIdx.x == 0) write_loss(F, loss_out, bin_counts);
  const int d = blockIdx.y, b = blockIdx.x * 256 + threadIdx.x;
  if (b >= B || !dgamma) return;
  const long long o = (long long)b * 3 + d;
  const Nig n{gamma[o], nu[o], alpha[o], beta[o]};
  const Terms t = loss_terms(n, targets[o]);
  const f32x4 g = loss_grad(n, t, d, B, cfg, F);
  dgamma[o] = g.x; dnu[o] = g.y; dalpha[o] = g.z; dbeta[o] = g.w;
}


template <int K>
__device__ __forceinline__ void block_sum(float (&v)[K], float (*sm)[K]) {
  const int lane = threadIdx.x & 63, wave = threadIdx.x >> 6;
#pragma unroll
  for (int i = 0; i < K; ++i) {
    const float s = wave_sum(v[i]);
    if (lane == 0) sm[wave][i] = s;
  }
  __syncthreads();
#pragma unroll
  for (int i = 0; i < K; ++i) v[i] = (sm[0][i] + sm[1][i]) + (sm[2][i] + sm[3][i]);
  __syncthreads();
}

__global__ __launch_bounds__(256) void deer_v1_kernel(const float* mu, const float* nu, const float* alpha, const float* beta,
                                                      const float* targets, long long n, float ew, float kw, float* partial,
                                                      float* dmu, float* dnu, float* dalpha, float* dbeta) {
  __shared__ float sm[4][4];
  const long long i = blockIdx.x * 256ll + threadIdx.x;
  float v[4] = {0.f, 0.f, 0.f, 0.f};
  if (i < n) {
    const float m = mu[i], nv = nu[i], a = alpha[i], b = beta[i], y = targets[i];
    const float d = y - m, se = d * d, ah = a + 0.5f;
    const float om = b + nv * se / 2.f;
    const float kPi = 3.14159265358979323846f;
    const float nll = 0.5f * logf(kPi / nv) - a * logf(2.f * b) + lgammaf(a) - lgammaf(ah) + ah * logf(om);
    const float reg = (nv * se + 2.f * b * (1.f + nv)) / (2.f * nv * (1.f + nv));
    const float klr = 0.5f * (nv - 1.f) + a * logf(b) - lgammaf(a) + lgammaf(ah) - 0.5f * logf(2.f * kPi * b);
    v[0] = nll; v[1] = reg; v[2] = fmaxf(klr, 0.f); v[3] = se;
    if (klr != klr) v[2] = klr;
    if (dmu) {
      const float inv = 1.f / (float)n, dpsi = digamma(a) - digamma(ah);
      const float kg = (klr >= 0.f) ? kw : 0.f;
      const float g_mu = -ah * nv * d / om - ew * d / (1.f + nv);
      const float g_nu = -0.5f / nv + ah * (se / 2.f) / om + ew * (-se / (2.f * (1.f + nv) * (1.f + nv)) - b / (nv * nv)) + kg * 0.5f;
      const float g_al = -logf(2.f * b) + dpsi + logf(om) + kg * (logf(b) - dpsi);
      const float g_be = -a / b + ah / om + ew / nv + kg * (a / b - 0.5f / b);
      dmu[i] = g_mu * inv; dnu[i] = g_nu * inv; dalpha[i] = g_al * inv; dbeta[i] = g_be * inv;
    }
  }
  block_sum<4>(v, sm);
  if (threadIdx.x < 4) partial[blockIdx.x * 4 + threadIdx.x] = v[threadIdx.x];
}

__global__ __launch_bounds__(256) void deer_v1_final_kernel(const float* partial, int nblk, long long n, float ew, float kw,
                                                            float* loss_out) {
  __shared__ float sm[4][4];
  float v[4] = {0.f, 0.f, 0.f, 0.f};
  for (int b = threadIdx.x; b < nblk; b += 256)
#pragma unroll
    for (int k = 0; k < 4; ++k) v[k] += partial[b * 4 + k];
  block_sum<4>(v, sm);
  if (threadIdx.x == 0) {
    const float inv = 1.f / (float)n;
    const float nll = v[0] * inv, reg = v[1] * inv, kl = v[2] * inv;
    loss_out[0] = nll + ew * reg + kw * kl; loss_out[1] = nll; loss_out[2] = reg; loss_out[3] = kl; loss_out[4] = v[3] * inv;
  }
}

constexpr int UREG_MAX_D = 8;
__global__ __launch_bounds__(256) void unc_reg_kernel(const float* alpha, const float* beta, int B, int D, float dw, float sw,
                                                      float* loss_out, float* dalpha, float* dbeta) {
  __shared__ float sm[4][UREG_MAX_D];
  __shared__ float mean[UREG_MAX_D];
  float v[UREG_MAX_D];
#pragma unroll
  for (int d = 0; d < UREG_MAX_D; ++d) v[d] = 0.f;
  for (int b = threadIdx.x; b < B; b += 256)
#pragma unroll
    for (int d = 0; d < UREG_MAX_D; ++d)
      if (d < D) v[d] += beta[(long long)b * D + d] / (alpha[(long long)b * D + d] - 1.f + kEps);
  block_sum<UREG_MAX_D>(v, sm);
  float total = 0.f;
#pragma unroll
  for (int d = 0; d < UREG_MAX_D; ++d)
    if (d < D) { total += v[d]; if (threadIdx.x == 0) mean[d] = v[d] / (float)B; }
  __syncthreads();
#pragma unroll
  for (int d = 0; d < UREG_MAX_D; ++d) v[d] = 0.f;
  for (int b = threadIdx.x; b < B; b += 256)
#pragma unroll
    for (int d = 0; d < UREG_MAX_D; ++d)
      if (d < D) {
        const float c = beta[(long long)b * D + d] / (alpha[(long long)b * D + d] - 1.f + kEps) - mean[d];
        v[d] += c * c;
      }
  block_sum<UREG_MAX_D>(v, sm);
  float vm = 0.f;
#pragma unroll
  for (int d = 0; d < UREG_MAX_D; ++d)
    if (d < D) vm += v[d] / (float)(B - 1);
  vm /= (float)D;
  const float div = -logf(vm + kEps), spars = total / ((float)B * (float)D);
  if (threadIdx.x == 0) { loss_out[0] = dw * div + sw * spars; loss_out[1] = div; loss_out[2] = spars; }
  if (!dalpha) return;
  const float cdiv = -dw / (vm + kEps) * 2.f / ((float)D * (float)(B - 1)), cs = sw / ((float)B * (float)D);
  for (long long e = threadIdx.x; e < (long long)B * D; e += 256) {
    const int d = (int)(e % D);
    const float den = alpha[e] - 1.f + kEps, u = beta[e] / den;
    const float gu = cdiv * (u - mean[d]) + cs;
    dalpha[e] = gu * (-u / den);
    dbeta[e] = gu / den;
  }
}

struct CalEdges { float e[CAL_MAX_BINS + 1]; int nb; };
const float kCalEdges15[16] = {0.0f, 0x1.111112p-4f, 0x1.111112p-3f, 0x1.99999cp-3f, 0x1.111112p-2f, 0x1.555556p-2f,
                               0x1.99999cp-2f, 0x1.dddde0p-2f, 0x1.111110p-1f, 0x1.333332p-1f, 0x1.555554p-1f,
                               0x1.777778p-1f, 0x1.99999ap-1f, 0x1.bbbbbcp-1f, 0x1.dddddep-1f, 1.0f};
__device__ __forceinline__ int cal_bin(const float* ed, int nb, float conf) {
  int bin = -1;
  for (int k = 0; k < nb; ++k) {
    const bool in = conf >= ed[k] && (k == nb - 1 ? conf <= ed[k + 1] : conf < ed[k + 1]);
    if (in) bin = k;
  }
  return bin;
}
__global__ __launch_bounds__(256) void calibration_kernel(const float* gamma, const float* alpha, const float* beta,
                                                          const float* targets, long long n, float* loss_out, int* bin_counts,
                                                          float* dgamma, float* dalpha, float* dbeta, const CalEdges ce) {
  __shared__ float sm[4][3];
  __shared__ float sgn[CAL_MAX_BINS];
  __shared__ float ed[CAL_MAX_BINS + 1];
  const int nb = ce.nb;
  if ((int)threadIdx.x <= nb) ed[threadIdx.x] = ce.e[threadIdx.x];
  __syncthreads();
  float loss = 0.f;
  for (int k = 0; k < nb; ++k) {
    float v[3] = {0.f, 0.f, 0.f};
    for (long long i = threadIdx.x; i < n; i += 256) {
      const float conf = 1.0f / (1.0f + beta[i] / (alpha[i] - 1.f + kEps));
      if (cal_bin(ed, nb, conf) == k) {
        const float err = fabsf(targets[i] - gamma[i]);
        v[0] += 1.f; v[1] += conf; v[2] += 1.0f - fminf(fmaxf(err / 2.0f, 0.f), 1.f);
      }
    }
    block_sum<3>(v, sm);
    float sg = 0.f;
    if (v[0] > 0.f) {
      const float diff = v[1] / v[0] - v[2] / v[0];
      loss += (v[0] / (float)n) * fabsf(diff);
      sg = diff > 0.f ? 1.f : (diff < 0.f ? -1.f : 0.f);
    }
    if (threadIdx.x == 0) { sgn[k] = sg; if (bin_counts) bin_counts[k] = (int)v[0]; }
  }
  if (threadIdx.x == 0) loss_out[0] = loss;
  __syncthreads();
  if (!dgamma) return;
  const float inv = 1.f / (float)n;
  for (long long i = threadIdx.x; i < n; i += 256) {
    const float den = alpha[i] - 1.f + kEps, u = beta[i] / den, conf = 1.0f / (1.0f + u);
    const int b = cal_bin(ed, nb, conf);
    const float s = b >= 0 ? sgn[b] * inv : 0.f;
    const float d = targets[i] - gamma[i], h = fabsf(d) / 2.0f;
    const float sd = d > 0.f ? 1.f : (d < 0.f ? -1.f : 0.f);
    dgamma[i] = (h >= 0.f && h <= 1.f) ? -s * 0.5f * sd : 0.f;
    const float gu = -s * conf * conf;
    dalpha[i] = gu * (-u / den);
    dbeta[i] = gu / den;
  }
}

}

int launch_nig_fwd(const void* e2, const void* w3, const float* b3, int b3_stride, float* evid, float* nig_out,
                   const float* targets, float* stats, int B, int act_f32, hipStream_t s) {
  if (B == 0) return 0;
  dim3 grid(nig_nblocks(B), 3);
  if (act_f32) hipLaunchKernelGGL(nig_fwd_kernel<true>, grid, dim3(256), 0, s, e2, w3, b3, b3_stride, evid, nig_out, targets, stats, B);
  else hipLaunchKernelGGL(nig_fwd_kernel<false>, grid, dim3(256), 0, s, e2, w3, b3, b3_stride, evid, nig_out, targets, stats, B);
  MMDEER_HIP(hipGetLastError());
  return 0;
}

__global__ __launch_bounds__(128) void nig_stats_sum_kernel(const float* stats, int nblk, int B, float* out, int nwp) {
  const int i = threadIdx.x;
  if (i < 3 * NIG_NSTAT) {
    float acc = 0.f;
    for (int p = 0; p < nblk; ++p) {
      if (nwp == 0) { acc += stats[(long long)p * 3 * NIG_NSTAT + i]; continue; }
      float w[4];
      for (int z = 0; z < 4; ++z) w[z] = 4 * p + z < nwp ? stats[(long long)(4 * p + z) * 3 * NIG_NSTAT + i] : 0.f;
      acc += (w[0] + w[1]) + (w[2] + w[3]);
    }
    out[i] = acc;
  } else if (i == 3 * NIG_NSTAT) {
    out[i] = (float)B;
  }
}

int launch_nig_stats_sum(const float* stats, int B, float* out, int nwp, hipStream_t s) {
  MMDEER_CHECK(B > 0, "nig statistics need a non-empty batch");
  hipLaunchKernelGGL(nig_stats_sum_kernel, dim3(1), dim3(128), 0, s, stats, nig_nblocks(B), B, out, nwp);
  MMDEER_HIP(hipGetLastError());
  return 0;
}

int launch_nig_bwd(const void* e2, const void* w3, const float* evid, const float* targets, const float* stats,
                   const float* gstats, const float* gmu, const float* gnu, const float* galpha, const float* gbeta,
                   float* devid, void* dz2, float* partial_w, float* partial_b, float* loss_out, int* bin_counts,
                   int B, int act_f32, float mask_scale, const LossCfg& cfg, int nwp, hipStream_t s) {
  MMDEER_CHECK(B > 0, "nig backward needs a non-empty batch");
  dim3 grid(nig_nblocks(B), 3);
  if (act_f32)
    hipLaunchKernelGGL(nig_bwd_kernel<true>, grid, dim3(256), 0, s, e2, w3, evid, targets, stats, gstats, gmu, gnu, galpha, gbeta,
                       devid, dz2, partial_w, partial_b, loss_out, bin_counts, B, mask_scale, cfg, nwp);
  else
    hipLaunchKernelGGL(nig_bwd_kernel<false>, grid, dim3(256), 0, s, e2, w3, evid, targets, stats, gstats, gmu, gnu, galpha, gbeta,
                       devid, dz2, partial_w, partial_b, loss_out, bin_counts, B, mask_scale, cfg, nwp);
  MMDEER_HIP(hipGetLastError());
  return 0;
}

int launch_nig_loss_stats(const float* gamma, const float* nu, const float* alpha, const float* beta,
                          const float* targets, float* stats, int B, hipStream_t s) {
  MMDEER_CHECK(B > 0, "nig loss needs a non-empty batch");
  hipLaunchKernelGGL(nig_loss_stats_kernel, dim3((B + 255) / 256, 3), dim3(256), 0, s, gamma, nu, alpha, beta, targets, stats, B);
  MMDEER_HIP(hipGetLastError());
  return 0;
}

int launch_nig_loss_grad(const float* gamma, const float* nu, const float* alpha, const float* beta,
                         const float* targets, const float* stats, float* dgamma, float* dnu, float* dalpha,
                         float* dbeta, float* loss_out, int* bin_counts, int B, const LossCfg& cfg, hipStream_t s) {
  MMDEER_CHECK(B > 0, "nig loss needs a non-empty batch");
  hipLaunchKernelGGL(nig_loss_grad_kernel, dim3((B + 255) / 256, 3), dim3(256), 0, s, gamma, nu, alpha, beta, targets, stats,
                     dgamma, dnu, dalpha, dbeta, loss_out, bin_counts, B, cfg);
  MMDEER_HIP(hipGetLastError());
  return 0;
}

int deer_v1_nblocks(long long n) { return (int)((n + 255) / 256); }

int launch_deer_loss_v1(const float* mu, const float* nu, const float* alpha, const float* beta, const float* targets, long long n,
                        float ew, float kw, float* loss_out, float* dmu, float* dnu, float* dalpha, float* dbeta, float* partial,
                        hipStream_t s) {
  MMDEER_CHECK(n > 0, "deer loss needs a non-empty batch");
  const int nblk = deer_v1_nblocks(n);
  hipLaunchKernelGGL(deer_v1_kernel, dim3(nblk), dim3(256), 0, s, mu, nu, alpha, beta, targets, n, ew, kw, partial, dmu, dnu, dalpha, dbeta);
  hipLaunchKernelGGL(deer_v1_final_kernel, dim3(1), dim3(256), 0, s, partial, nblk, n, ew, kw, loss_out);
  MMDEER_HIP(hipGetLastError());
  return 0;
}

int launch_unc_reg_loss(const float* alpha, const float* beta, int B, int D, float dw, float sw, float* loss_out, float* dalpha,
                        float* dbeta, hipStream_t s) {
  MMDEER_CHECK(B > 0 && D >= 1 && D <= UREG_MAX_D, "uncertainty regularisation: B=%d must be > 0 and D=%d in 1..8", B, D);
  hipLaunchKernelGGL(unc_reg_kernel, dim3(1), dim3(256), 0, s, alpha, beta, B, D, dw, sw, loss_out, dalpha, dbeta);
  MMDEER_HIP(hipGetLastError());
  return 0;
}

int launch_calibration_loss(const float* gamma, const float* alpha, const float* beta, const float* targets, long long n,
                            float* loss_out, int* bin_counts, float* dgamma, float* dalpha, float* dbeta, const float* edges,
                            int n_bins, hipStream_t s) {
  MMDEER_CHECK(n > 0, "calibration loss needs a non-empty batch");
  MMDEER_CHECK(n_bins >= 1 && n_bins <= CAL_MAX_BINS, "calibration loss: 1 <= n_bins <= %d (got %d)", CAL_MAX_BINS, n_bins);
  CalEdges ce{};
  ce.nb = n_bins;
  const float* src = edges ? edges : kCalEdges15;
  MMDEER_CHECK(edges || n_bins == 15, "calibration loss: edges must be given unless n_bins == 15");
  for (int i = 0; i <= n_bins; ++i) ce.e[i] = src[i];
  hipLaunchKernelGGL(calibration_kernel, dim3(1), dim3(256), 0, s, gamma, alpha, beta, targets, n, loss_out, bin_counts, dgamma, dalpha, dbeta, ce);
  MMDEER_HIP(hipGetLastError());
  return 0;
}

#ifdef MMDEER_STAMPS
int debug_nig_stamps(unsigned long long* out16) {
  MMDEER_HIP(hipMemcpyFromSymbol(out16, HIP_SYMBOL(g_nig_stamps), sizeof(unsigned long long) * 16));
  return 0;
}
#endif

}
```

### uncertainty-aware-multimodal-emotion-recognition_amd/csrc/nig_dev.h

```cpp
#pragma once
#include "nig.h"

#ifndef GSTAMP
#define GSTAMP(slot) do {} while (0)
#endif

namespace mmdeer {
namespace {

typedef unsigned nig_u32x4 __attribute__((ext_vector_type(4)));

__device__ const float kEceEdges[11] = {0.0f, 0x1.99999ap-4f, 0x1.99999ap-3f, 0x1.333334p-2f, 0x1.99999ap-2f, 0x1p-1f,
                                        0x1.333334p-1f, 0x1.666666p-1f, 0x1.99999ap-1f, 0x1.ccccccp-1f, 1.0f};
constexpr float kEps = 1e-8f;
constexpr float kTwoPiEps = 6.28318530717958647692f;



struct Nig { float mu, nu, alpha, beta; };

__device__ __forceinline__ float softplus(float x) { return x > 20.f ? x : log1pf(expf(x)); }
__device__ __forceinline__ float softplus_grad(float x) {
#pragma clang fp contract(off)
  if (x > 20.f) return 1.f;
  const float z = expf(x);
  return z / (z + 1.f);
}
__device__ __forceinline__ Nig nig_act(const f32x4& ev) {
#pragma clang fp contract(off)
  Nig n;
  n.mu = ev.x;
  n.nu = softplus(ev.y) + 1e-6f;
  n.alpha = softplus(ev.z) + 1.0f;
  n.beta = softplus(ev.w) + 1e-6f;
  return n;
}

__device__ __forceinline__ float digamma(float x) {
#pragma clang fp contract(off)
  float r = 0.f;
  while (x < 6.f) { r -= 1.f / x; x += 1.f; }
  const float f = 1.f / (x * x);
  return r + logf(x) - 0.5f / x
         - f * (1.f / 12.f - f * (1.f / 120.f - f * (1.f / 252.f - f * (1.f / 240.f - f * (1.f / 132.f)))));
}

struct Terms { float logprob, reg, kla, klb, u, conf, aerr, err, A, lb; int bin; };

__device__ __forceinline__ Terms loss_terms(const Nig& n, float y) {
#pragma clang fp contract(off)
  Terms t;
  t.err = y - n.mu;
  const float e2 = t.err * t.err;
  t.A = n.beta + 0.5f * n.nu * e2 + kEps;
  t.lb = logf(n.beta + kEps);
  t.logprob = 0.5f * logf(n.nu / kTwoPiEps) + n.alpha * t.lb - lgammaf(n.alpha + kEps) - (n.alpha + 0.5f) * logf(t.A);
  t.aerr = fabsf(t.err);
  t.reg = e2 * (2.f * n.beta + n.nu * e2);
  const float am1 = n.alpha - 1.f;
  t.kla = am1 * am1;
  t.klb = t.lb * t.lb;
  t.u = n.beta / (am1 + kEps);
  t.conf = 1.0f / (1.0f + t.u);
  t.bin = -1;
#pragma unroll
  for (int k = 0; k < 10; ++k)
    if (t.conf > kEceEdges[k] && t.conf <= kEceEdges[k + 1]) t.bin = k;
  return t;
}

__device__ __forceinline__ void block_stats(const Terms& t, bool active, float* slab) {
  __shared__ float sm[4][NIG_NSTAT];
  float v[NIG_NSTAT];
  v[0] = active ? t.logprob : 0.f;
  v[1] = active ? t.reg : 0.f;
  v[2] = active ? t.kla : 0.f;
  v[3] = active ? t.klb : 0.f;
  v[4] = active ? t.u : 0.f;
#pragma unroll
  for (int k = 0; k < 10; ++k) {
    const bool in = active && t.bin == k;
    v[5 + k] = in ? t.conf : 0.f;
    v[15 + k] = in ? t.aerr : 0.f;
    v[25 + k] = in ? 1.f : 0.f;
  }
  const int lane = threadIdx.x & 63, wave = threadIdx.x >> 6;
#pragma unroll
  for (int i = 0; i < NIG_NSTAT; ++i) {
    const float s = wave_sum(v[i]);
    if (lane == 0) sm[wave][i] = s;
  }
  __syncthreads();
  if (threadIdx.x < NIG_NSTAT)
    slab[threadIdx.x] = (sm[0][threadIdx.x] + sm[1][threadIdx.x]) + (sm[2][threadIdx.x] + sm[3][threadIdx.x]);
}

struct Finals {
  float sign[3][10];
  float dcross[3];
  float out[NIG_LOSS_OUT];
  int counts[3][10];
};

constexpr int NIG_FINALS_TMP = 3 * NIG_NSTAT + 30 + 3 + 3;
__device__ __forceinline__ void compute_finals(const float* stats, int nblk, int B, const LossCfg& cfg, Finals& F,
                                               float (*gs)[NIG_NSTAT], float* tmp, int nwp = 0) {
  constexpr int NV = 3 * NIG_NSTAT;
  float* const upper = tmp; float* const ece_c = tmp + NV; float* const dim_total = ece_c + 30; float* const ubar_s = dim_total + 3;
  {
    const int i = threadIdx.x & 127, h = threadIdx.x >> 7;
    float acc = 0.f;
    if (i < NV) {
      const int per = (nblk + 1) >> 1, p0 = h * per, p1 = (p0 + per < nblk) ? p0 + per : nblk;
      if (nwp == 0) {
        for (int q = p0; q < p1; q += 16) {
          float v[16];
#pragma unroll
          for (int u = 0; u < 16; ++u) {
            const int p = q + u < p1 ? q + u : p1 - 1;
            v[u] = stats[(long long)p * NV + i];
          }
#pragma unroll
          for (int u = 0; u < 16; ++u) v[u] = q + u < p1 ? v[u] : 0.f;
          acc += ((v[0] + v[1]) + (v[2] + v[3])) + ((v[4] + v[5]) + (v[6] + v[7])) +
                 (((v[8] + v[9]) + (v[10] + v[11])) + ((v[12] + v[13]) + (v[14] + v[15])));
        }
      } else {
        for (int q = p0; q < p1; q += 16) {
          float w[16][4];
#pragma unroll
          for (int u = 0; u < 16; ++u)
#pragma unroll
            for (int z = 0; z < 4; ++z) {
              const int p = q + u < p1 ? q + u : p1 - 1, wp = 4 * p + z;
              w[u][z] = stats[(long long)(wp < nwp ? wp : nwp - 1) * NV + i];
            }
          float v[16];
#pragma unroll
          for (int u = 0; u < 16; ++u) {
            const int p = q + u < p1 ? q + u : p1 - 1;
#pragma unroll
            for (int z = 0; z < 4; ++z) w[u][z] = 4 * p + z < nwp ? w[u][z] : 0.f;
            v[u] = q + u < p1 ? (w[u][0] + w[u][1]) + (w[u][2] + w[u][3]) : 0.f;
          }
          acc += ((v[0] + v[1]) + (v[2] + v[3])) + ((v[4] + v[5]) + (v[6] + v[7])) +
                 (((v[8] + v[9]) + (v[10] + v[11])) + ((v[12] + v[13]) + (v[14] + v[15])));
        }
      }
      if (h == 1) upper[i] = acc;
    }
    __syncthreads();
    if (h == 0 && i < NV) gs[i / NIG_NSTAT][i % NIG_NSTAT] = acc + upper[i];
  }
  GSTAMP(8);
  __syncthreads();
  GSTAMP(9);
  const float N = (float)B;
  if (threadIdx.x < 30) {
    const int d = threadIdx.x / 10, k = threadIdx.x - d * 10;
    const float cnt = gs[d][25 + k];
    F.counts[d][k] = (int)cnt;
    float sg = 0.f, c = 0.f;
    if (cnt > 0.f) {
      const float diff = gs[d][5 + k] / cnt - (1.0f - gs[d][15 + k] / cnt);
      c = (cnt / N) * fabsf(diff);
      sg = diff > 0.f ? 1.f : (diff < 0.f ? -1.f : 0.f);
    }
    F.sign[d][k] = sg;
    ece_c[threadIdx.x] = c;
  }
  __syncthreads();
  if (threadIdx.x < 3) {
    const int d = threadIdx.x;
    float ece = 0.f;
    for (int k = 0; k < 10; ++k) ece += ece_c[d * 10 + k];
    const float nll = -gs[d][0] / N, reg = gs[d][1] / N;
    const float kl = gs[d][2] / N + 0.1f * (gs[d][3] / N);
    const float total = nll + cfg.reg_w * reg + cfg.kl_w * kl + cfg.ece_w * ece;
    F.out[d * 5 + 0] = total; F.out[d * 5 + 1] = nll; F.out[d * 5 + 2] = reg; F.out[d * 5 + 3] = kl; F.out[d * 5 + 4] = ece;
    ubar_s[d] = gs[d][4] / N;
    dim_total[d] = total;
  }
  __syncthreads();
  if (threadIdx.x == 0) {
    float tot = 0.f;
    for (int d = 0; d < 3; ++d) tot += cfg.task_w[d] * dim_total[d];
    const float d01 = ubar_s[0] - ubar_s[1], d02 = ubar_s[0] - ubar_s[2], d12 = ubar_s[1] - ubar_s[2];
    const float cross = (d01 * d01 + d02 * d02 + d12 * d12) / 3.f;
    F.dcross[0] = (2.f / 3.f) * (d01 + d02);
    F.dcross[1] = (2.f / 3.f) * (-d01 + d12);
    F.dcross[2] = (2.f / 3.f) * (-d02 - d12);
    if (cfg.cross_w > 0.f) tot += cfg.cross_w * cross;
    F.out[15] = cross;
    F.out[16] = tot / 3.f;
    F.out[17] = (F.out[1] + F.out[6] + F.out[11]) / 3.f;
    F.out[18] = (F.out[2] + F.out[7] + F.out[12]) / 3.f;
    F.out[19] = (F.out[3] + F.out[8] + F.out[13]) / 3.f;
  }
  GSTAMP(10);
  __syncthreads();
}

__device__ __forceinline__ void write_loss(const Finals& F, float* loss_out, int* bin_counts) {
  if (loss_out)
    for (int i = 0; i < NIG_LOSS_OUT; ++i) loss_out[i] = F.out[i];
  if (bin_counts)
    for (int i = 0; i < 30; ++i) bin_counts[i] = F.counts[i / 10][i % 10];
}

__device__ __forceinline__ f32x4 loss_grad(const Nig& n, const Terms& t, int d, int B, const LossCfg& cfg, const Finals& F) {
#pragma clang fp contract(off)
  const float invN = 1.f / (float)B;
  const float cd = cfg.task_w[d] / 3.f;
  const float e2 = t.err * t.err;
  const float ah = n.alpha + 0.5f;
  const float sg = (t.bin >= 0) ? F.sign[d][t.bin] : 0.f;
  const float den = (n.alpha - 1.f) + kEps;
  const float du_db = 1.f / den, du_da = -t.u / den;
  const float dconf_du = -t.conf * t.conf;
  const float serr = t.err > 0.f ? 1.f : (t.err < 0.f ? -1.f : 0.f);
  const float gu = (cfg.cross_w / 3.f) * F.dcross[d] * invN;
  f32x4 g;
  g.x = cd * invN * (-(ah * n.nu * t.err) / t.A + cfg.reg_w * (2.f * n.beta + 2.f * n.nu * e2) * (-2.f * t.err)
                     + cfg.ece_w * sg * (-serr));
  g.y = cd * invN * (-(0.5f / n.nu - ah * 0.5f * e2 / t.A) + cfg.reg_w * e2 * e2);
  g.z = cd * invN * (-(t.lb - digamma(n.alpha + kEps) - logf(t.A)) + cfg.kl_w * 2.f * (n.alpha - 1.f)
                     + cfg.ece_w * sg * dconf_du * du_da)
        + gu * du_da;
  g.w = cd * invN * (-(n.alpha / (n.beta + kEps) - ah / t.A) + cfg.reg_w * 2.f * e2
                     + cfg.kl_w * 0.2f * t.lb / (n.beta + kEps) + cfg.ece_w * sg * dconf_du * du_db)
        + gu * du_db;
  return g;
}

__device__ __forceinline__ float nig_dx(const f32x4& dE, float w0, float w1, float w2, float w3) {
  return fmaf(dE.w, w3, fmaf(dE.z, w2, fmaf(dE.y, w1, dE.x * w0)));
}

template <bool F32>
__device__ __forceinline__ void load_chunk16(const void* base, long long idx, float (&x)[16]) {
  if constexpr (F32) {
    const float* p = reinterpret_cast<const float*>(base) + idx;
#pragma unroll
    for (int i = 0; i < 4; ++i) {
      const f32x4 a = *reinterpret_cast<const f32x4*>(p + 4 * i);
      x[4 * i] = a.x; x[4 * i + 1] = a.y; x[4 * i + 2] = a.z; x[4 * i + 3] = a.w;
    }
  } else {
    const bf16_t* p = reinterpret_cast<const bf16_t*>(base) + idx;
#pragma unroll
    for (int i = 0; i < 2; ++i) {
      const nig_u32x4 a = *reinterpret_cast<const nig_u32x4*>(p + 8 * i);
      x[8 * i + 0] = __uint_as_float(a.x << 16); x[8 * i + 1] = __uint_as_float(a.x & 0xFFFF0000u);
      x[8 * i + 2] = __uint_as_float(a.y << 16); x[8 * i + 3] = __uint_as_float(a.y & 0xFFFF0000u);
      x[8 * i + 4] = __uint_as_float(a.z << 16); x[8 * i + 5] = __uint_as_float(a.z & 0xFFFF0000u);
      x[8 * i + 6] = __uint_as_float(a.w << 16); x[8 * i + 7] = __uint_as_float(a.w & 0xFFFF0000u);
    }
  }
}

template <bool F32>
__device__ __forceinline__ void store_chunk16(void* base, long long idx, const float (&x)[16]) {
  if constexpr (F32) {
    float* p = reinterpret_cast<float*>(base) + idx;
#pragma unroll
    for (int i = 0; i < 4; ++i) *reinterpret_cast<f32x4*>(p + 4 * i) = f32x4{x[4 * i], x[4 * i + 1], x[4 * i + 2], x[4 * i + 3]};
  } else {
    bf16_t* p = reinterpret_cast<bf16_t*>(base) + idx;
#pragma unroll
    for (int i = 0; i < 2; ++i)
      *reinterpret_cast<nig_u32x4*>(p + 8 * i) = nig_u32x4{pack_bf2(x[8 * i], x[8 * i + 1]), pack_bf2(x[8 * i + 2], x[8 * i + 3]),
                                                   pack_bf2(x[8 * i + 4], x[8 * i + 5]), pack_bf2(x[8 * i + 6], x[8 * i + 7])};
  }
}
}
}
```

### uncertainty-aware-multimodal-emotion-recognition_amd/csrc/stackc.hip

```cpp
#include <cstring>

#include "../../include/mmdeer.h"
#include "attention.h"
#include "common.h"
#include "gemm.h"
#include "nig.h"
#include "optim.h"
#include "options.h"
#include "chain.h"
#include "rowops.h"

namespace mmdeer {
namespace {

constexpr int TRACE_MAX = 32;
struct Trace { void** ev = nullptr; int max = 0, n = 0; const char* label[TRACE_MAX]; };
thread_local Trace g_trace;
int trace_mark(const char* label, hipStream_t s) {
  Trace& t = g_trace;
  if (!t.ev || t.n >= t.max || t.n >= TRACE_MAX) return 0;
  if (hipEventRecord((hipEvent_t)t.ev[t.n], s) != hipSuccess) { set_error("trace: hipEventRecord failed"); return -1; }
  t.label[t.n++] = label;
  return 0;
}
#define MARK(label) do { if (trace_mark(label, s) != 0) return -1; } while (0)

struct ParamInfo { const char* name; int rows, cols; long long off; int is_matrix; };
#define X(idx, ident, rows, cols, off, ismat, name) {name, rows, cols, off, ismat},
constexpr ParamInfo kParams[] = {
#include "params.inc"
};
#undef X
enum ParamId {
#define X(idx, ident, rows, cols, off, ismat, name) ident = idx,
#include "params.inc"
#undef X
};
static_assert(MMDEER_NUM_PARAMS == MMDEER_NUM_PARAMS_ABI, "parameter table out of sync with the public header");

constexpr int P_AUD_W = MMDEER_P_AUDIO_VISUAL_AUDIO_PROJECTION_WEIGHT, P_AUD_B = MMDEER_P_AUDIO_VISUAL_AUDIO_PROJECTION_BIAS;
constexpr int P_VID_W = MMDEER_P_AUDIO_VISUAL_VIDEO_PROJECTION_WEIGHT, P_VID_B = MMDEER_P_AUDIO_VISUAL_VIDEO_PROJECTION_BIAS;
constexpr int P_AIN_W = MMDEER_P_AUDIO_VISUAL_CROSS_ATTENTION_IN_PROJ_WEIGHT, P_AIN_B = MMDEER_P_AUDIO_VISUAL_CROSS_ATTENTION_IN_PROJ_BIAS;
constexpr int P_AOUT_W = MMDEER_P_AUDIO_VISUAL_CROSS_ATTENTION_OUT_PROJ_WEIGHT, P_AOUT_B = MMDEER_P_AUDIO_VISUAL_CROSS_ATTENTION_OUT_PROJ_BIAS;
constexpr int P_AVF_W = MMDEER_P_AUDIO_VISUAL_FUSION_LAYERS_0_WEIGHT, P_AVF_B = MMDEER_P_AUDIO_VISUAL_FUSION_LAYERS_0_BIAS;
constexpr int P_AVF_G = MMDEER_P_AUDIO_VISUAL_FUSION_LAYERS_3_WEIGHT, P_AVF_BT = MMDEER_P_AUDIO_VISUAL_FUSION_LAYERS_3_BIAS;
constexpr int P_AVP_W = MMDEER_P_TRIMODAL_AUDIOVISUAL_PROJECTION_WEIGHT, P_AVP_B = MMDEER_P_TRIMODAL_AUDIOVISUAL_PROJECTION_BIAS;
constexpr int P_TXT_W = MMDEER_P_TRIMODAL_TEXT_PROJECTION_WEIGHT, P_TXT_B = MMDEER_P_TRIMODAL_TEXT_PROJECTION_BIAS;
constexpr int P_TIN_W = MMDEER_P_TRIMODAL_MODALITY_ATTENTION_IN_PROJ_WEIGHT, P_TIN_B = MMDEER_P_TRIMODAL_MODALITY_ATTENTION_IN_PROJ_BIAS;
constexpr int P_TOUT_W = MMDEER_P_TRIMODAL_MODALITY_ATTENTION_OUT_PROJ_WEIGHT, P_TOUT_B = MMDEER_P_TRIMODAL_MODALITY_ATTENTION_OUT_PROJ_BIAS;
constexpr int P_TFF_W = MMDEER_P_TRIMODAL_FINAL_0_WEIGHT, P_TFF_B = MMDEER_P_TRIMODAL_FINAL_0_BIAS;
constexpr int P_TFF_G = MMDEER_P_TRIMODAL_FINAL_3_WEIGHT, P_TFF_BT = MMDEER_P_TRIMODAL_FINAL_3_BIAS;
constexpr int P_OP_W = MMDEER_P_OUTP0_WEIGHT, P_OP_B = MMDEER_P_OUTP0_BIAS, P_OP_G = MMDEER_P_OUTP3_WEIGHT, P_OP_BT = MMDEER_P_OUTP3_BIAS;
constexpr int P_FP0_W = MMDEER_P_FP0_WEIGHT, P_FP0_B = MMDEER_P_FP0_BIAS, P_FP1_W = MMDEER_P_FP3_WEIGHT, P_FP1_B = MMDEER_P_FP3_BIAS;
constexpr int P_EV0_W = MMDEER_P_HEAD0_EV0_WEIGHT, P_EV0_B = MMDEER_P_HEAD0_EV0_BIAS;
constexpr int P_EV1_W = MMDEER_P_HEAD0_EV3_WEIGHT, P_EV1_B = MMDEER_P_HEAD0_EV3_BIAS;
constexpr int P_EV2_W = MMDEER_P_HEAD0_EV6_WEIGHT, P_EV2_B = MMDEER_P_HEAD0_EV6_BIAS;

constexpr int AUD = MMDEER_AUDIO_DIM, VID = MMDEER_VIDEO_DIM, TXT = MMDEER_TEXT_DIM, INTER = MMDEER_INTER_DIM;
constexpr int FUS = MMDEER_FUSION_DIM, HID = MMDEER_HIDDEN_DIM, EV1 = 128, EV2 = 64;
constexpr int SPLITK_MAX = 8;
constexpr int AUD_PAD = 128;

struct Layout {
  using ACT = char; using BF16 = char; using F32 = float;
#define X(buf, kind, name, elems, bf16_only) kind* name;
#include "layout.inc"
#undef X
  size_t wbytes;
  size_t bytes;
};

inline size_t align_up(size_t x, size_t a = 256) { return (x + a - 1) / a * a; }

Layout make_layout(void* base, void* wbase, int B, int f32) {
  Layout L{};
  const size_t size_ACT = f32 ? 4 : 2, size_BF16 = 2, size_F32 = 4;
  const size_t Bz = (size_t)(B > 0 ? B : 1), nblk = (size_t)nig_nblocks(B);
  const size_t np = (size_t)(ln_bwd_nparts(B) > chain_workgroups_max(B) ? ln_bwd_nparts(B) : chain_workgroups_max(B));
  const size_t nhead = nblk > (size_t)chain_workgroups_max(B) ? nblk : (size_t)chain_workgroups_max(B);
  char* const base_W = reinterpret_cast<char*>(wbase);
  char* const base_S = reinterpret_cast<char*>(base);
  size_t off_W = 0, off_S = 0;
#define X(buf, kind, name, elems, bf16_only)                                                      \
  L.name = reinterpret_cast<Layout::kind*>(base_##buf ? base_##buf + off_##buf : nullptr);        \
  off_##buf += align_up((bf16_only) && f32 ? 0 : (size_t)(elems) * size_##kind);
#include "layout.inc"
#undef X
  L.wbytes = off_W;
  L.bytes = off_S;
  return L;
}

long long layout_offset(char buf, int batch, int f32, const char* name) {
  if (!name || batch < 0) return -1;
  char* const base = reinterpret_cast<char*>(uintptr_t(1) << 40);
  const Layout L = make_layout(base, base, batch, f32);
#define X(b, kind, field, elems, bf16_only) \
  if (buf == #b[0] && strcmp(name, #field) == 0) return reinterpret_cast<const char*>(L.field) - base;
#include "layout.inc"
#undef X
  return -1;
}

enum : unsigned {
  IMG_FRAG = 1,
  IMG_FRAGT = 2,
  IMG_WT = 4,
  IMG_PAD = 8,
  IMG_HM = 16,
  IMG_CHAIN = IMG_FRAG | IMG_FRAGT | IMG_WT,
};
struct ImageRange {
  int pid, row0, rows;
  unsigned img;
  int s_pid, s_row0, s_rows;
  int wt_pid, wt_ld;
  constexpr int cols() const { return kParams[pid].cols; }
  constexpr long long off() const { return kParams[pid].off + (long long)row0 * cols(); }
  constexpr long long s_off() const { return kParams[s_pid].off + (long long)s_row0 * cols(); }
  constexpr int s_row() const { return (int)((off() - s_off()) / cols()); }
  constexpr int wt_col() const { return (int)((off() - kParams[wt_pid].off) / cols()); }
};
constexpr ImageRange whole(int pid, unsigned img) {
  return {pid, 0, kParams[pid].rows, img, pid, 0, kParams[pid].rows, pid, kParams[pid].rows};
}
constexpr ImageRange stacked(int pid, int first, int n, unsigned img) {
  return {pid, 0, kParams[pid].rows, img, first, 0, n * kParams[pid].rows, first, n * kParams[pid].rows};
}
constexpr ImageRange kImages[] = {
    whole(P_AUD_W, IMG_PAD),
    whole(P_VID_W, IMG_FRAG),
    {P_AIN_W, 0, 2 * INTER, IMG_WT, P_AIN_W, 0, 3 * INTER, P_AIN_W, 3 * INTER},
    {P_AIN_W, 2 * INTER, INTER, IMG_CHAIN, P_AIN_W, 2 * INTER, INTER, P_AIN_W, 3 * INTER},
    whole(P_AOUT_W, IMG_CHAIN), whole(P_AVF_W, IMG_CHAIN), whole(P_AVP_W, IMG_CHAIN),
    whole(P_TXT_W, IMG_FRAG),
    whole(P_TIN_W, IMG_HM | IMG_WT),
    whole(P_TOUT_W, IMG_CHAIN), whole(P_TFF_W, IMG_CHAIN), whole(P_OP_W, IMG_CHAIN), whole(P_FP0_W, IMG_CHAIN), whole(P_FP1_W, IMG_CHAIN),
    stacked(P_EV0_W, P_EV0_W, 3, IMG_CHAIN), stacked(P_EV0_W + 1, P_EV0_W, 3, IMG_CHAIN), stacked(P_EV0_W + 2, P_EV0_W, 3, IMG_CHAIN),
    whole(P_EV1_W, IMG_CHAIN), whole(P_EV1_W + 1, IMG_CHAIN), whole(P_EV1_W + 2, IMG_CHAIN),
};
constexpr int kNumImages = sizeof(kImages) / sizeof(kImages[0]);
static_assert(kNumImages <= ADAM_MAX_IMAGED, "the fused optimiser step takes one AdamImaged per range");

struct Plan {
  bool chains;
  bool in_chain;
  bool nig_tail;
  int nwp;
  bool bchain, dchain;
  bool nigfold;
};
Plan make_plan(int B, int f32, int phase, bool g_fused, bool inputs_bf16, bool targets) {
  Plan p{};
  p.chains = !f32 && opt(OPT_CHAIN) && B >= opt(OPT_CHAIN_MIN) && B <= opt(OPT_CHAIN_MAX);
  p.in_chain = p.chains && opt(OPT_CHAIN_IN) && inputs_bf16 && chain_samples_per_workgroup(B) == 16;
  p.nig_tail = p.chains && opt(OPT_CHAIN_NIGF);
  p.nwp = p.nig_tail ? (B + 15) / 16 : 0;
  const bool bwd = p.chains && opt(OPT_CHAIN_BWD);
  p.bchain = bwd && !g_fused;
  p.dchain = bwd && phase == 0;
  p.nigfold = p.bchain && opt(OPT_CHAIN_NIG) && targets;
  return p;
}

struct Rows { void* p; int ld; };
struct Layer {
  int pidW, pidB;
  int N, K, M;
  Rows in, out;
  int in_f32;
  Rows dout, din;
  int relu, site;
  Rows mask;
  int shift = 0;
  int w_row0 = 0;
  int wt_ld;
  int heads = 1;
  bool padded = false;
  int row0 = 0;
  int aux_col = -1;
  bool open = false;
  bool cat_out = false;
  bool cat_in = false;
  int regen = -1;
  int regen_shift = 0;
  int pidG = -1, pidBt = -1;
  void* xln = nullptr; float* out32 = nullptr; float* mean = nullptr; float* rstd = nullptr; float* part = nullptr;
};
Layer linear(int pidW, int pidB, int N, int K, int M, Rows in, int in_f32, Rows out, Rows dout, Rows din, int relu = 0, int site = -1,
             Rows mask = {nullptr, 0}) {
  Layer l{pidW, pidB, N, K, M, in, out, in_f32, dout, din, relu, site, mask};
  l.wt_ld = N;
  return l;
}
void layer_norm(Layer& l, int pidG, int pidBt, void* xln, float* out32, float* mean, float* rstd, float* part) {
  l.pidG = pidG; l.pidBt = pidBt; l.xln = xln; l.out32 = out32; l.mean = mean; l.rstd = rstd; l.part = part;
}

struct Net { Layer vid, aud, txt, avv, aout, avf, avp, tin, tout, tff, op, fp0, fp1, ev0, ev1; };
Net make_net(const Layout& L, int B, int f32, const void* audio, const void* video, const void* text, int in_f32, float* av32,
             float* tri32, float* fused32) {
  const size_t es = f32 ? 4 : 2;
  auto in = [](const void* p, int ld) { return Rows{const_cast<void*>(p), ld}; };
  const Rows none{nullptr, 0};
  Net n;
  n.vid = linear(P_VID_W, P_VID_B, INTER, VID, B, in(video, VID), in_f32, {L.avin, INTER}, {L.davin, INTER}, none);
  n.vid.aux_col = 0; n.vid.open = true;
  n.aud = linear(P_AUD_W, P_AUD_B, INTER, f32 ? AUD : AUD_PAD, B, f32 ? in(audio, AUD) : Rows{L.audio_pad, AUD_PAD}, f32 ? in_f32 : 0,
                 {L.avin, INTER}, {L.davin, INTER}, none);
  n.aud.padded = !f32; n.aud.row0 = B; n.aud.aux_col = VID;
  const Rows tok0{L.xtok, 2 * FUS}, tok1{L.xtok + (size_t)FUS * es, 2 * FUS}, dtok0{L.dxtok, 2 * FUS}, dtok1{L.dxtok + (size_t)FUS * es, 2 * FUS};
  n.txt = linear(P_TXT_W, P_TXT_B, FUS, TXT, B, in(text, TXT), in_f32, tok1, dtok1, none);
  n.avv = linear(P_AIN_W, P_AIN_B, INTER, INTER, 2 * B, {L.avin, INTER}, f32, {L.avv, INTER}, {L.davv, INTER}, {L.davin, INTER}, 0, SITE_AV_ATTN);
  n.avv.shift = 5; n.avv.w_row0 = 2 * INTER; n.avv.wt_ld = 3 * INTER;
  n.aout = linear(P_AOUT_W, P_AOUT_B, INTER, INTER, 2 * B, {L.avv, INTER}, f32, {L.cat, 2 * INTER}, {L.dcats, INTER}, {L.davv, INTER});
  n.aout.cat_out = true; n.aout.regen = SITE_AV_ATTN; n.aout.regen_shift = 5;
  n.avf = linear(P_AVF_W, P_AVF_B, INTER, 2 * INTER, B, {L.cat, 2 * INTER}, f32, {L.y_a2, INTER}, {L.dz_a2, INTER}, {L.dcats, INTER}, 1, SITE_AV_FUSE);
  n.avf.cat_in = true;
  layer_norm(n.avf, P_AVF_G, P_AVF_BT, L.av, av32, L.mean_a2, L.rstd_a2, L.part_ln_a2);
  n.avp = linear(P_AVP_W, P_AVP_B, FUS, INTER, B, {L.av, INTER}, f32, tok0, dtok0, {L.dav, INTER});
  n.tin = linear(P_TIN_W, P_TIN_B, 3 * FUS, FUS, 2 * B, {L.xtok, FUS}, f32, {L.qkv, 3 * FUS}, {L.dqkv, 3 * FUS}, {L.dxtok, FUS});
  n.tout = linear(P_TOUT_W, P_TOUT_B, FUS, FUS, B, {L.obar, FUS}, f32, {L.pool, FUS}, {L.dpool, FUS}, {L.dobar, FUS});
  n.tff = linear(P_TFF_W, P_TFF_B, FUS, FUS, B, {L.pool, FUS}, f32, {L.y_t3, FUS}, {L.dz_t3, FUS}, {L.dpool, FUS}, 1, SITE_TRI_FUSE);
  layer_norm(n.tff, P_TFF_G, P_TFF_BT, L.tri, tri32, L.mean_t3, L.rstd_t3, L.part_ln_t3);
  n.op = linear(P_OP_W, P_OP_B, FUS, FUS, B, {L.tri, FUS}, f32, {L.y_o1, FUS}, {L.dz_o1, FUS}, {L.dtri, FUS}, 1, SITE_OUT_PROJ);
  layer_norm(n.op, P_OP_G, P_OP_BT, L.fused, fused32, L.mean_o1, L.rstd_o1, L.part_ln_o1);
  n.fp0 = linear(P_FP0_W, P_FP0_B, HID, FUS, B, {L.fused, FUS}, f32, {L.h1, HID}, {L.dh1, HID}, {L.dfused, FUS}, 1, SITE_FP0);
  n.fp1 = linear(P_FP1_W, P_FP1_B, HID, HID, B, {L.h1, HID}, f32, {L.h2, HID}, {L.dh2, HID}, {L.dh1, HID}, 1, SITE_FP1, {L.h1, HID});
  n.ev0 = linear(P_EV0_W, P_EV0_B, 3 * EV1, HID, B, {L.h2, HID}, f32, {L.e1, 3 * EV1}, {L.de1, 3 * EV1}, {L.dh2, HID}, 1, SITE_EV0, {L.h2, HID});
  n.ev1 = linear(P_EV1_W, P_EV1_B, EV2, EV1, B, {L.e1, 3 * EV1}, f32, {L.e2, 3 * EV2}, {L.dz2, 3 * EV2}, {L.de1, 3 * EV1}, 1, SITE_EV1, {L.e1, 3 * EV1});
  n.ev1.heads = 3;
  return n;
}

struct Exec {
  int B, f32;
  int slice_div = 1;
  size_t es;
  bool drop_on;
  bool bump;
  float mask_scale;
  DropCtx dc;
  const Layout* L;
  hipStream_t s;

  const char* W(int pid) const { return L->wpack + (size_t)kParams[pid].off * es; }
  const float* V(int pid) const { return L->vpack + kParams[pid].off; }
  const char* WT(int pid) const { return L->wtpack + (size_t)kParams[pid].off * es; }
  const bf16_t* WF(int pid, size_t elem_off = 0) const { return reinterpret_cast<const bf16_t*>(L->wfpack) + kParams[pid].off + elem_off; }
  const bf16_t* WTF(int pid, size_t elem_off = 0) const { return reinterpret_cast<const bf16_t*>(L->wtfpack) + kParams[pid].off + elem_off; }
  char* at(const Rows& r, int row0) const { return reinterpret_cast<char*>(r.p) + (size_t)row0 * r.ld * es; }
  static bf16_t* bf(const void* p) { return reinterpret_cast<bf16_t*>(const_cast<void*>(p)); }

  GemmProblem fwd(const Layer& l) const {
    GemmProblem p;
    gemm_problem_defaults(p);
    p.A = l.in.p; p.a_f32 = l.in_f32; p.lda = l.in.ld;
    p.B = l.padded ? L->wa_pad : W(l.pidW) + (size_t)l.w_row0 * l.K * es; p.b_f32 = f32; p.ldb = l.K;
    p.C = at(l.out, l.row0); p.c_f32 = f32; p.ldc = l.out.ld;
    p.bias = V(l.pidB) + l.w_row0;
    p.M = l.M; p.N = l.N; p.K = l.K;
    p.relu = l.relu;
    p.drop_site = drop_on ? l.site : -1; p.drop_shift = l.shift;
    if (l.heads > 1) { p.batch = l.heads; p.sA = l.K; p.sB = (long long)l.N * l.K; p.sC = l.N; p.sBias = l.N; }
    if (l.cat_out) { p.M = l.M / 2; p.batch = 2; p.sA = (long long)p.M * l.in.ld; p.sC = l.N; }
    return p;
  }
  void fwd_seg(ChainArgs& c, const Layer& l) const {
    for (int z = 0; z < l.heads; ++z) {
      ChainSeg q;
      chain_seg_defaults(q);
      q.W = l.padded ? bf(L->wa_frag) : WF(l.pidW, ((size_t)l.w_row0 + (size_t)z * l.N) * l.K);
      q.bias = V(l.pidB) + l.w_row0 + z * l.N;
      q.N = l.N; q.K = l.K; q.ldw = l.K;
      q.relu = l.relu; q.drop_site = drop_on ? l.site : -1; q.drop_shift = l.shift;
      q.kin_off = z * l.K; q.nout_off = z * l.N; q.dcol_off = z * l.N;
      if (l.aux_col >= 0) { q.in_aux = 1; q.kin_off = l.aux_col; }
      q.row_group = l.row0 ? 1 : 0;
      q.fold_groups = l.cat_out ? 1 : 0;
      if (z == l.heads - 1 && !l.open) {
        q.end_layer = 1; q.nout = (l.cat_out ? 2 : l.heads) * l.N; q.stash = bf(l.out.p); q.ld_stash = l.out.ld;
        if (l.pidG >= 0) { q.gamma = V(l.pidG); q.beta = V(l.pidBt); q.xln = bf(l.xln); q.out32 = l.out32; q.mean = l.mean; q.rstd = l.rstd; }
      }
      c.seg[c.nseg++] = q;
    }
  }
  int fwd_ln(const Layer& l, const Layer& norm) const {
    GemmGroup g{};
    g.nprob = 1;
    g.p[0] = fwd(l);
    g.drop = dc;
    return launch_gemm_ln(g, norm.out.p, V(norm.pidG), V(norm.pidBt), norm.xln, norm.out32, norm.mean, norm.rstd, s);
  }
  int ln_fwd(const Layer& l) const {
    return launch_ln_fwd(l.out.p, l.xln, l.out32, l.mean, l.rstd, V(l.pidG), V(l.pidBt), l.M, l.N, f32, s);
  }
  int ln_bwd(const Layer& l, const Layer& next) const {
    return launch_ln_bwd(next.din.p, l.out.p, l.mean, l.rstd, V(l.pidG), l.dout.p, l.part, l.M, l.N, f32, mask_scale, s);
  }
  GemmProblem dx(const Layer& l) const {
    GemmProblem p;
    gemm_problem_defaults(p);
    p.A = l.dout.p; p.a_f32 = f32; p.lda = l.dout.ld;
    p.B = WT(l.pidW) + (size_t)l.w_row0 * es; p.b_f32 = f32; p.ldb = l.wt_ld;
    p.C = l.din.p; p.c_f32 = f32; p.ldc = l.din.ld;
    p.M = l.M; p.N = l.K; p.K = l.N;
    p.Y = l.mask.p; p.y_f32 = f32; p.ldy = l.mask.ld; p.mask_scale = mask_scale;
    if (drop_on && l.regen >= 0) { p.regen_site = l.regen; p.drop_shift = l.regen_shift; }
    if (l.heads > 1) { p.batch = l.heads; p.sA = l.N; p.sB = (long long)l.N * l.K; p.sC = l.K; p.sY = l.K; }
    if (l.cat_in) { p.N = l.K / 2; p.batch = 2; p.sB = (long long)p.N * l.N; p.sC = (long long)l.M * l.din.ld; }
    return p;
  }
  void dx_seg(ChainArgs& c, const Layer& l, const Layer* norm = nullptr) const {
    for (int z = 0; z < l.heads; ++z) {
      ChainSeg q;
      chain_seg_defaults(q);
      q.W = WTF(l.pidW, ((size_t)l.w_row0 + (size_t)z * l.N) * l.K);
      q.N = l.K; q.K = l.N; q.ldw = l.N;
      q.kin_off = z * l.N; q.nout_off = z * l.K;
      if (l.mask.p) { q.mask_y = bf(l.mask.p); q.ld_mask = l.mask.ld; q.mask_col0 = z * l.K; q.mask_scale = mask_scale; }
      if (drop_on && l.regen >= 0) { q.drop_site = l.regen; q.drop_shift = l.regen_shift; }
      q.fold_groups = l.cat_in ? 2 : 0;
      if (z == l.heads - 1) {
        q.end_layer = 1; q.nout = l.cat_in ? l.K / 2 : l.heads * l.K; q.stash = bf(l.din.p); q.ld_stash = l.din.ld;
        if (norm) {
          q.lnb_gamma = V(norm->pidG); q.lnb_y = bf(norm->out.p); q.lnb_mean = norm->mean; q.lnb_rstd = norm->rstd;
          q.lnb_dz = bf(norm->dout.p); q.lnb_partial = norm->part; q.lnb_mask_scale = mask_scale;
        }
      }
      c.seg[c.nseg++] = q;
    }
  }
  GemmProblem dw(const Layer& l, float* grads) const {
    const int cols = kParams[l.pidW].cols;
    GemmProblem p;
    gemm_problem_defaults(p);
    p.A = at(l.dout, l.row0); p.a_f32 = f32; p.lda = l.dout.ld; p.trans_a = 1;
    p.B = l.in.p; p.b_f32 = l.in_f32; p.ldb = l.in.ld; p.trans_b = 1;
    p.C = grads + kParams[l.pidW].off + (long long)l.w_row0 * cols; p.c_f32 = 1; p.ldc = cols;
    p.bias_grad = grads + kParams[l.pidB].off + l.w_row0;
    p.M = l.N; p.N = cols; p.K = l.M;
    if (l.heads > 1) { p.batch = l.heads; p.sA = l.N; p.sB = l.K; p.sC = (long long)l.N * l.K; p.sBiasGrad = l.N; }
    set_split(p, grads);
    return p;
  }
  void set_split(GemmProblem& p, float* grads) const {
    const int nk = gemm_ktiles(p.K, f32);
    int kst = ksteps_target(f32);
    if (!f32 && opt(OPT_DW_TILE) == 2 && opt(OPT_KSTEPS) == 0) { kst = B / 64 / slice_div; kst = kst < 4 ? 4 : kst > 128 ? 128 : kst; }
    int sk = (nk + kst - 1) / kst;
    const int cap = opt(OPT_SPLITK_MAX) < SPLITK_MAX ? opt(OPT_SPLITK_MAX) : SPLITK_MAX;
    if (sk > cap) sk = cap;
    if (sk < 1) sk = 1;
    p.splitk = sk;
    p.slab_stride = MMDEER_FLAT_ELEMS;
    p.slab_c = L->slab + (reinterpret_cast<float*>(p.C) - grads);
    p.slab_b = p.bias_grad ? L->slab + (p.bias_grad - grads) : nullptr;
  }
  static void add_slab_segments(ReduceTable& t, const GemmProblem& p) {
    if (p.splitk <= 1) return;
    const long long csz = (long long)(p.batch - 1) * p.sC + (long long)(p.M - 1) * p.ldc + p.N;
    int k = t.nseg;
    t.src[k] = p.slab_c; t.dst[k] = reinterpret_cast<float*>(p.C); t.nparts[k] = p.splitk;
    t.n[k] = (int)((csz + 3) / 4 * 4); t.stride[k] = p.slab_stride; ++k;
    if (p.bias_grad) {
      const long long bsz = (long long)(p.batch - 1) * p.sBiasGrad + p.M;
      t.src[k] = p.slab_b; t.dst[k] = p.bias_grad; t.nparts[k] = p.splitk;
      t.n[k] = (int)((bsz + 3) / 4 * 4); t.stride[k] = p.slab_stride; ++k;
    }
    t.nseg = k;
  }
  void add_ln_segment(ReduceTable& t, const Layer& l, float* grads, bool chained) const {
    const int k = t.nseg++;
    t.src[k] = l.part; t.dst[k] = grads + kParams[l.pidG].off; t.nparts[k] = chained ? chain_workgroups(B) : ln_bwd_nparts(B);
    t.n[k] = 2 * l.N; t.stride[k] = 2 * l.N;
  }
  ChainArgs chain(const Rows& x, int K0, int groups, long long group_stride) const {
    ChainArgs c{};
    c.X = bf(x.p); c.ldx = x.ld; c.K0 = K0; c.B = B; c.groups = groups; c.group_stride = group_stride;
    c.drop = dc;
    return c;
  }
  int run(GemmGroup& g) const {
    g.drop = dc;
    return launch_gemm_group(g, f32, pick_tile(g), s);
  }
  int run1(const GemmProblem& p) const {
    GemmGroup g{};
    g.nprob = 1;
    g.p[0] = p;
    return run(g);
  }
};
Exec make_exec(const Layout& L, int B, int f32, hipStream_t s, int training, float dropout_p, uint64_t seed, uint64_t offset,
               const uint64_t* offset_dev, int bump_offset_dev) {
  Exec X;
  X.B = B; X.f32 = f32; X.es = f32 ? 4 : 2; X.L = &L; X.s = s;
  X.drop_on = training && dropout_p > 0.f;
  X.bump = bump_offset_dev && offset_dev;
  X.dc = make_drop(dropout_p, seed, offset + (X.bump ? 1 : 0), offset_dev);
  X.mask_scale = X.drop_on ? X.dc.scale : 1.f;
  return X;
}


int check_weights(const void* w, size_t w_bytes, int f32) {
  MMDEER_CHECK(w != nullptr, "weights buffer is NULL");
  MMDEER_CHECK(((uintptr_t)w % 256) == 0, "weights buffer must be 256-byte aligned");
  const size_t need = mmdeer_weights_bytes(f32);
  MMDEER_CHECK(w_bytes >= need, "weights buffer too small: %zu bytes given, %zu needed", w_bytes, need);
  return 0;
}
int check_common(int batch, const void* ws, size_t ws_bytes, const void* w, size_t w_bytes, int f32) {
  MMDEER_CHECK(batch >= 0, "batch must be >= 0 (got %d)", batch);
  MMDEER_CHECK(ws != nullptr, "workspace is NULL");
  MMDEER_CHECK(((uintptr_t)ws % 256) == 0, "workspace must be 256-byte aligned");
  const size_t need = mmdeer_workspace_bytes(batch, f32);
  MMDEER_CHECK(ws_bytes >= need, "workspace too small: %zu bytes given, %zu needed for batch %d", ws_bytes, need, batch);
  return check_weights(w, w_bytes, f32);
}

int pack_transposed_weights(const void* const* params, const Layout& L, int f32, hipStream_t s) {
  PackTTable tt{};
  for (const ImageRange& r : kImages) {
    if (!(r.img & IMG_WT)) continue;
    const int k = tt.nmat++;
    tt.src[k] = reinterpret_cast<const float*>(params[r.pid]) + (long long)r.row0 * r.cols();
    tt.dst_off[k] = kParams[r.wt_pid].off;
    tt.rows[k] = r.rows; tt.cols[k] = r.cols();
    tt.ld_dst[k] = r.wt_ld; tt.dst_col[k] = r.wt_col();
  }
  return launch_pack_transposed(tt, L.wtpack, f32, s);
}

int repack_images(const Layout& L, bool with_transposed, hipStream_t s) {
  RepackTable t{};
  const bf16_t* wp = reinterpret_cast<const bf16_t*>(L.wpack);
  auto job = [&](long long src_off, int rows, int cols_valid, int cols, int transpose, int layout, char* dst_base, long long dst_off,
                 int ld_dst = 0, int dst_col = 0) {
    RepackJob& J = t.job[t.njobs++];
    J.src = wp + src_off; J.ld_src = cols_valid; J.rows = rows; J.cols = cols; J.cols_valid = cols_valid;
    J.transpose = transpose; J.layout = layout;
    J.dst = reinterpret_cast<bf16_t*>(dst_base) + dst_off; J.ld_dst = ld_dst; J.dst_col = dst_col;
  };
  auto for_runs = [&](unsigned kind, auto emit) {
    for (int i = 0, j; i < kNumImages; i = j) {
      const ImageRange& a = kImages[i];
      j = i + 1;
      if (!(a.img & kind)) continue;
      int rows = a.rows;
      for (; j < kNumImages; rows += kImages[j++].rows) {
        const ImageRange& b = kImages[j];
        const bool same = kind == IMG_WT ? (b.wt_pid == a.wt_pid && b.wt_ld == a.wt_ld) : (b.s_pid == a.s_pid && b.s_row0 == a.s_row0 && b.s_rows == a.s_rows);
        if (!(b.img & kind) || !same || b.off() != a.off() + (long long)rows * a.cols()) break;
      }
      emit(a, rows);
    }
  };
  for_runs(IMG_FRAG, [&](const ImageRange& a, int rows) { job(a.off(), rows, a.cols(), a.cols(), 0, 1, L.wfpack, a.off()); });
  for (const ImageRange& r : kImages) {
    if (r.img & IMG_PAD) {
      job(r.off(), r.rows, r.cols(), AUD_PAD, 0, 0, L.wa_pad, 0, AUD_PAD, 0);
      job(r.off(), r.rows, r.cols(), AUD_PAD, 0, 1, L.wa_frag, 0);
    }
    if (r.img & IMG_HM) job(r.off(), r.rows, r.cols(), r.cols(), 0, 2, L.wqkv_hm, 0, r.cols(), 0);
  }
  if (with_transposed) {
    for_runs(IMG_WT, [&](const ImageRange& a, int rows) { job(a.off(), rows, a.cols(), a.cols(), 1, 0, L.wtpack, kParams[a.wt_pid].off, a.wt_ld, a.wt_col()); });
    bool whole_s = true;
    for_runs(IMG_FRAGT, [&](const ImageRange& a, int rows) {
      whole_s = whole_s && rows == a.s_rows;
      job(a.off(), rows, a.cols(), a.cols(), 1, 1, L.wtfpack, a.s_off());
    });
    MMDEER_CHECK(whole_s, "image table: the ranges of a matrix with a fragment-major W^T image must be neighbours and cover it");
  }
  return launch_repack(t, s);
}

int pack_params(const void* const* params, const Layout& L, int f32, hipStream_t s) {
  PackTable t{};
  t.nseg = MMDEER_NUM_PARAMS;
  for (int i = 0; i < MMDEER_NUM_PARAMS; ++i) {
    t.src[i] = reinterpret_cast<const float*>(params[i]);
    t.dst_off[i] = kParams[i].off;
    t.n[i] = kParams[i].rows * kParams[i].cols;
    t.is_vec[i] = kParams[i].is_matrix ? 0 : 1;
  }
  TRY(launch_pack_params(t, L.wpack, f32, L.vpack, s));
  if (f32) return pack_transposed_weights(params, L, f32, s);
  return repack_images(L, true, s);
}
int check_params(const void* const* params, const char* who) {
  for (int i = 0; i < MMDEER_NUM_PARAMS; ++i)
    MMDEER_CHECK(params[i] != nullptr && ((uintptr_t)params[i] % 16) == 0, "%s: params[%d] (%s) must be non-NULL and 16-byte aligned", who, i, kParams[i].name);
  return 0;
}

}
}

using namespace mmdeer;

extern "C" {

int mmdeer_num_params(void) { return MMDEER_NUM_PARAMS; }
const char* mmdeer_param_name(int i) { return (i >= 0 && i < MMDEER_NUM_PARAMS) ? kParams[i].name : ""; }
int mmdeer_param_rows(int i) { return (i >= 0 && i < MMDEER_NUM_PARAMS) ? kParams[i].rows : -1; }
int mmdeer_param_cols(int i) { return (i >= 0 && i < MMDEER_NUM_PARAMS) ? kParams[i].cols : -1; }
long long mmdeer_param_offset(int i) { return (i >= 0 && i < MMDEER_NUM_PARAMS) ? kParams[i].off : -1; }
long long mmdeer_flat_elems(void) { return MMDEER_FLAT_ELEMS; }

size_t mmdeer_workspace_bytes(int batch, int compute_f32) { return make_layout(nullptr, nullptr, batch, compute_f32).bytes; }
size_t mmdeer_weights_bytes(int compute_f32) { return make_layout(nullptr, nullptr, 0, compute_f32).wbytes; }
long long mmdeer_workspace_offset(int batch, int compute_f32, const char* name) { return layout_offset('S', batch, compute_f32 ? 1 : 0, name); }
long long mmdeer_weights_offset(int compute_f32, const char* name) { return layout_offset('W', 0, compute_f32 ? 1 : 0, name); }

int mmdeer_trace_begin(void** events, int n_events) {
  MMDEER_CHECK(events != nullptr && n_events > 0, "trace_begin: no events");
  g_trace = Trace{};
  g_trace.ev = events; g_trace.max = n_events;
  return 0;
}
int mmdeer_trace_end(void) { const int n = g_trace.n; g_trace.ev = nullptr; return n; }
const char* mmdeer_trace_label(int i) { return (i >= 0 && i < g_trace.n && i < TRACE_MAX) ? g_trace.label[i] : ""; }

long long mmdeer_bucket_begin(int b) {
  switch (b) { case 0: return kParams[P_FP0_W].off; case 1: return kParams[P_AVP_W].off; case 2: return 0; default: return -1; }
}
long long mmdeer_bucket_end(int b) {
  switch (b) { case 0: return MMDEER_FLAT_ELEMS; case 1: return kParams[P_FP0_W].off; case 2: return kParams[P_AVP_W].off; default: return -1; }
}

int mmdeer_forward(const mmdeer_forward_args* a) {
  MMDEER_CHECK(a != nullptr, "args is NULL");
  const int B = a->batch, f32 = a->compute_f32 ? 1 : 0;
  TRY(check_common(B, a->workspace, a->workspace_bytes, a->weights, a->weights_bytes, f32));
  MMDEER_CHECK(!(f32 && a->inputs_bf16), "bf16 inputs need compute_f32 = 0");
  MMDEER_CHECK(a->dropout_p >= 0.f && a->dropout_p < 1.f, "dropout_p must be in [0,1) (got %f)", a->dropout_p);
  MMDEER_CHECK(!(a->bump_offset_dev && (f32 || B == 0)), "bump_offset_dev needs bf16 compute and a non-empty batch");
  hipStream_t s = (hipStream_t)a->stream;
  const Layout L = make_layout(a->workspace, a->weights, B, f32);
  if (a->repack) {
    MMDEER_CHECK(a->params != nullptr, "params is NULL");
    for (int i = 0; i < MMDEER_NUM_PARAMS; ++i) {
      MMDEER_CHECK(a->params[i] != nullptr, "params[%d] (%s) is NULL", i, kParams[i].name);
      MMDEER_CHECK(((uintptr_t)a->params[i] % 16) == 0, "params[%d] (%s) must be 16-byte aligned", i, kParams[i].name);
    }
    TRY(pack_params(a->params, L, f32, s));
  }
  if (B == 0) return 0;
  MMDEER_CHECK(a->audio && a->video && a->text, "audio / video / text must be non-NULL");
  MMDEER_CHECK(a->nig_out != nullptr, "nig_out is NULL");

  const Exec X = make_exec(L, B, f32, s, a->training, a->dropout_p, a->seed, a->offset, a->offset_dev, a->bump_offset_dev);
  const int in_f32 = a->inputs_bf16 ? 0 : 1;
  const Plan plan = make_plan(B, f32, 0, false, !in_f32, false);
  const Net n = make_net(L, B, f32, a->audio, a->video, a->text, in_f32, a->audiovisual_features, a->trimodal_features, a->fused_features);

  if (!f32 && !plan.in_chain) {
    PadTable pt{};
    pt.src[0] = a->audio; pt.dst[0] = L.audio_pad; pt.src_f32[0] = in_f32; pt.rows[0] = B; pt.cols[0] = AUD; pt.ld_dst[0] = AUD_PAD;
    pt.nseg = 1;
    TRY(launch_pad_cols(pt, s));
    MARK("pad_cols (audio 84 -> 128)");
  }
  if (!plan.in_chain) {
    GemmGroup g{};
    g.nprob = 3;
    g.p[0] = X.fwd(n.vid);
    g.p[1] = X.fwd(n.aud);
    g.p[2] = X.fwd(n.txt);
    TRY(X.run(g));
    MARK("F1 input projections (3 problems)");
  }
  const bool lnf = !f32 && opt(OPT_LN_FUSED);
  if (plan.chains) {
    ChainArgs c = X.chain(n.avv.in, n.avv.K, 2, B);
    if (plan.in_chain) {
      c = X.chain(n.txt.in, n.txt.K, 1, B);
      c.aux_video = Exec::bf(n.vid.in.p); c.aux_ldv = n.vid.in.ld;
      c.aux_audio = reinterpret_cast<const bf16_t*>(a->audio); c.aux_lda = AUD;
      c.aux_audio_pad = reinterpret_cast<bf16_t*>(L.audio_pad);
      X.fwd_seg(c, n.txt);
      X.fwd_seg(c, n.vid);
      X.fwd_seg(c, n.aud);
    }
    X.fwd_seg(c, n.avv);
    X.fwd_seg(c, n.aout);
    X.fwd_seg(c, n.avf);
    X.fwd_seg(c, n.avp);
    TRY(launch_chain(c, s));
    MARK(plan.in_chain ? "chain F1-F6 (input projections + audio-visual fusion)" : "chain F2-F6 (audio-visual fusion)");
  } else {
    TRY(X.run1(X.fwd(n.avv)));
    TRY(X.run1(X.fwd(n.aout)));
    TRY(X.run1(X.fwd(n.avf)));
    if (lnf) {
      TRY(X.fwd_ln(n.avp, n.avf));
    } else {
      TRY(X.ln_fwd(n.avf));
      TRY(X.run1(X.fwd(n.avp)));
    }
  }
  if (!plan.chains) MARK("F2-F6 separate launches");
  if (a->prof_events[0]) MMDEER_HIP(hipEventRecord((hipEvent_t)a->prof_events[0], s));
  if (!f32 && opt(OPT_FUSED_ATTN)) {
    void* qkv_out = (a->training && !opt(OPT_QKV_RECOMPUTE)) ? L.qkv : nullptr;
    TRY(launch_tri_fused_fwd(L.xtok, L.wqkv_hm, X.V(P_TIN_B), L.obar, L.probs, qkv_out, B, X.drop_on ? 1 : 0, X.dc, s));
    if (a->prof_events[1]) MMDEER_HIP(hipEventRecord((hipEvent_t)a->prof_events[1], s));
    MARK("tri_fused_kernel<0> (in_proj + attention)");
    TRY(launch_tri_attn_weights(L.probs, a->trimodal_attention, a->av_attention, B, X.drop_on ? 1 : 0, X.dc, s));
    if (a->trimodal_attention || a->av_attention) MARK("attention weights");
  } else {
    TRY(X.run1(X.fwd(n.tin)));
    if (a->prof_events[1]) MMDEER_HIP(hipEventRecord((hipEvent_t)a->prof_events[1], s));
    TRY(launch_tri_attn_fwd(L.qkv, L.obar, L.probs, a->trimodal_attention, a->av_attention, B, f32, X.drop_on ? 1 : 0, X.dc, s));
    MARK("in_proj GEMM + attention (unfused)");
  }
  if (plan.chains) {
    ChainArgs c = X.chain(n.tout.in, n.tout.K, 1, 0);
    X.fwd_seg(c, n.tout);
    X.fwd_seg(c, n.tff);
    X.fwd_seg(c, n.op);
    X.fwd_seg(c, n.fp0);
    X.fwd_seg(c, n.fp1);
    X.fwd_seg(c, n.ev0);
    X.fwd_seg(c, n.ev1);
    if (plan.nig_tail) {
      ChainNigF& g = c.nigf;
      g.enabled = 1;
      g.w3 = reinterpret_cast<const bf16_t*>(X.W(P_EV2_W)); g.b3 = X.V(P_EV2_B); g.b3_stride = 64;
      g.evid = L.evid; g.nig_out = a->nig_out; g.targets = a->targets; g.wstats = L.stats;
    }
#ifdef MMDEER_STAMPS
    c.stamps = reinterpret_cast<unsigned long long*>(L.slab);
#endif
    TRY(launch_chain(c, s));
    MARK(plan.nig_tail ? "chain F9-F18 (trimodal fusion tail + head + NIG)" : "chain F9-F17 (trimodal fusion tail + head)");
  } else {
    TRY(X.run1(X.fwd(n.tout)));
    TRY(X.run1(X.fwd(n.tff)));
    if (lnf) {
      TRY(X.fwd_ln(n.op, n.tff));
      TRY(X.fwd_ln(n.fp0, n.op));
    } else {
      TRY(X.ln_fwd(n.tff));
      TRY(X.run1(X.fwd(n.op)));
      TRY(X.ln_fwd(n.op));
      TRY(X.run1(X.fwd(n.fp0)));
    }
    TRY(X.run1(X.fwd(n.fp1)));
    TRY(X.run1(X.fwd(n.ev0)));
    TRY(X.run1(X.fwd(n.ev1)));
  }
  if (!plan.chains) MARK("F9-F17 separate launches");
  if (!plan.nig_tail) {
    TRY(launch_nig_fwd(L.e2, X.W(P_EV2_W), X.V(P_EV2_B), 64, L.evid, a->nig_out, a->targets, L.stats, B, f32, s));
    MARK("nig_fwd (head's last layer + loss statistics)");
  }
  return 0;
}

int mmdeer_backward(const mmdeer_backward_args* a) {
  MMDEER_CHECK(a != nullptr, "args is NULL");
  const int B = a->batch, f32 = a->compute_f32 ? 1 : 0;
  TRY(check_common(B, a->workspace, a->workspace_bytes, a->weights, a->weights_bytes, f32));
  MMDEER_CHECK(B > 0, "backward needs a non-empty batch");
  MMDEER_CHECK(a->grads != nullptr, "grads is NULL");
  MMDEER_CHECK(a->audio && a->video && a->text, "audio / video / text must be non-NULL");
  hipStream_t s = (hipStream_t)a->stream;
  const Layout L = make_layout(a->workspace, a->weights, B, f32);
  Exec X = make_exec(L, B, f32, s, a->training, a->dropout_p, a->seed, a->offset, a->offset_dev, a->bump_offset_dev);
  const Net n = make_net(L, B, f32, a->audio, a->video, a->text, a->inputs_bf16 ? 0 : 1, nullptr, nullptr, nullptr);
  float* G = a->grads;
  const LossCfg cfg = loss_cfg(a->loss);
  const int nblk = nig_nblocks(B);


  auto reduce_head = [&](ReduceTable& t, int nparts) {
    int k = t.nseg;
    t.src[k] = L.part_w3; t.dst[k] = G + kParams[P_EV2_W].off; t.nparts[k] = nparts; t.n[k] = 768; t.stride[k] = 768; ++k;
    for (int d = 0; d < 3; ++d) {
      t.src[k] = L.part_b3 + d * 4; t.dst[k] = G + kParams[P_EV2_B + d].off; t.nparts[k] = nparts; t.n[k] = 4; t.stride[k] = 12; ++k;
    }
    t.nseg = k;
  };
  GemmGroup dwg{};
  ReduceTable rt{};
  auto add_dw = [&](const Layer& l) { dwg.p[dwg.nprob++] = X.dw(l, G); };
  const int phase = a->phase;
  MMDEER_CHECK(phase >= 0 && phase <= 2, "backward: phase must be 0, 1 or 2 (got %d)", phase);
  const Plan plan = make_plan(B, f32, phase, a->g_fused != nullptr, a->inputs_bf16 != 0, a->targets != nullptr);
  auto finish = [&](int first_bucket, int last_bucket) -> int {
    if (dwg.nprob > 0) {
      TRY(X.run(dwg));
      MARK("weight gradients (all problems, one launch)");
      for (int i = 0; i < dwg.nprob; ++i) Exec::add_slab_segments(rt, dwg.p[i]);
    }
    if (X.bump && (phase == 0 || phase == 2)) rt.bump = reinterpret_cast<unsigned long long*>(const_cast<uint64_t*>(a->offset_dev));
    TRY(launch_reduce_partials(rt, s));
    MARK("reduce_partials (fold)");
    for (int b = first_bucket; b <= last_bucket; ++b)
      if (a->bucket_events[b]) MMDEER_HIP(hipEventRecord((hipEvent_t)a->bucket_events[b], s));
    return 0;
  };

  if (phase != 2) {
  if (!plan.nigfold)
    TRY(launch_nig_bwd(L.e2, X.W(P_EV2_W), L.evid, a->targets, L.stats, a->targets ? a->global_stats : nullptr, a->g_mu, a->g_nu, a->g_alpha, a->g_beta, nullptr,
                       L.dz2, L.part_w3, L.part_b3, a->loss_out, a->bin_counts, B, f32, X.mask_scale, cfg, plan.nwp, s));
  if (!plan.nigfold) MARK("nig_bwd (head's last layer backward + loss gradient)");
  if (plan.bchain) {
    ChainArgs c = X.chain(n.ev1.dout, n.ev1.heads * n.ev1.N, 1, 0);
    X.dx_seg(c, n.ev1);
    X.dx_seg(c, n.ev0);
    X.dx_seg(c, n.fp1);
    X.dx_seg(c, n.fp0, &n.op);
    X.dx_seg(c, n.op, &n.tff);
    X.dx_seg(c, n.tff);
    X.dx_seg(c, n.tout);
    if (plan.nigfold) {
      ChainNig& g = c.nig;
      g.enabled = 1;
      g.e2 = reinterpret_cast<const bf16_t*>(L.e2); g.w3 = reinterpret_cast<const bf16_t*>(X.W(P_EV2_W)); g.evid = L.evid;
      g.targets = a->targets; g.stats = L.stats; g.gstats = a->global_stats; g.nblk = nblk; g.nwp = plan.nwp;
      g.dz2 = reinterpret_cast<bf16_t*>(L.dz2); g.partial_w = L.part_w3; g.partial_b = L.part_b3;
      g.loss_out = a->loss_out; g.bin_counts = a->bin_counts; g.mask_scale = X.mask_scale; g.cfg = cfg;
    }
#ifdef MMDEER_STAMPS
    c.stamps = reinterpret_cast<unsigned long long*>(L.davin);
#endif
    TRY(launch_chain(c, s));
    MARK(plan.nigfold ? "chain B1-B10 (head backward + loss gradient + head / trimodal dX)" : "chain B2-B10 (head / trimodal dX)");
  } else {
    TRY(X.run1(X.dx(n.ev1)));
    TRY(X.run1(X.dx(n.ev0)));
    TRY(X.run1(X.dx(n.fp1)));
    TRY(X.run1(X.dx(n.fp0)));
  }
  if (a->g_fused) TRY(launch_add_f32(L.dfused, f32, a->g_fused, (long long)B * FUS, s));
  add_dw(n.ev1);
  add_dw(n.ev0);
  add_dw(n.fp1);
  add_dw(n.fp0);
  reduce_head(rt, plan.nigfold ? chain_workgroups(B) : nblk);

  if (!plan.bchain) {
    TRY(X.ln_bwd(n.op, n.fp0));
    TRY(X.run1(X.dx(n.op)));
    TRY(X.ln_bwd(n.tff, n.op));
    TRY(X.run1(X.dx(n.tff)));
    TRY(X.run1(X.dx(n.tout)));
  }
  if (!plan.bchain) MARK("B2-B10 separate launches");
  if (!f32 && opt(OPT_FUSED_ATTN) && opt(OPT_QKV_RECOMPUTE)) {
    TRY(launch_tri_fused_bwd(L.xtok, L.wqkv_hm, X.V(P_TIN_B), L.dobar, L.probs, L.dqkv, B, X.drop_on ? 1 : 0, X.dc, s));
    MARK("tri_fused_kernel<1> (attention backward, recompute)");
  } else {
    TRY(launch_tri_attn_bwd(L.qkv, L.dobar, L.probs, L.dqkv, B, f32, X.drop_on ? 1 : 0, X.dc, s));
    MARK("attention backward (unfused)");
  }
  TRY(X.run1(X.dx(n.tin)));
  MARK("in_proj dX GEMM");
  if (!plan.dchain) TRY(X.run1(X.dx(n.avp)));
  add_dw(n.op);
  add_dw(n.tff);
  add_dw(n.tout);
  add_dw(n.tin);
  add_dw(n.avp);
  add_dw(n.txt);
  X.add_ln_segment(rt, n.op, G, plan.bchain);
  X.add_ln_segment(rt, n.tff, G, plan.bchain);
  if (phase == 1) return finish(0, 1);
  }

  if (phase == 2) X.slice_div = 8;
  if (plan.dchain) {
    ChainArgs c = X.chain(n.avp.dout, n.avp.N, 1, B);
    X.dx_seg(c, n.avp, &n.avf);
    X.dx_seg(c, n.avf);
    X.dx_seg(c, n.aout);
    X.dx_seg(c, n.avv);
    TRY(launch_chain(c, s));
    MARK("chain B13-B17 (audio-visual dX)");
  } else {
    TRY(X.ln_bwd(n.avf, n.avp));
    TRY(X.run1(X.dx(n.avf)));
    TRY(X.run1(X.dx(n.aout)));
    TRY(X.run1(X.dx(n.avv)));
  }
  add_dw(n.avf);
  add_dw(n.aout);
  add_dw(n.avv);
  add_dw(n.vid);
  add_dw(n.aud);
  X.add_ln_segment(rt, n.avf, G, plan.dchain);
  if (!plan.dchain) MARK("B13-B17 separate launches");
  return finish(phase == 2 ? 2 : 0, 2);
}


int mmdeer_adamw_step(const mmdeer_adamw_args* a) {
  MMDEER_CHECK(a != nullptr, "args is NULL");
  const int f32 = a->compute_f32 ? 1 : 0;
  TRY(check_weights(a->weights, a->weights_bytes, f32));
  MMDEER_CHECK(a->params && a->grads && a->exp_avg && a->exp_avg_sq && a->lr, "adamw: params / grads / exp_avg / exp_avg_sq / lr must be non-NULL");
  MMDEER_CHECK(a->step >= 1, "adamw: step must be >= 1 (got %d)", a->step);
  MMDEER_CHECK(a->beta1 >= 0.f && a->beta1 < 1.f && a->beta2 >= 0.f && a->beta2 < 1.f && a->eps > 0.f, "adamw: bad betas / eps");
  const void* const* cparams = const_cast<const void* const*>(a->params);
  TRY(check_params(cparams, "adamw"));
  hipStream_t s = (hipStream_t)a->stream;
  const Layout L = make_layout(nullptr, a->weights, 0, f32);
  const bool images = !f32 && opt(OPT_ADAM_FUSED);
  AdamTable t{};
  AdamImagedTable im{};
  im.base = reinterpret_cast<bf16_t*>(a->weights);
  const bool wt_on = a->pack_transposed != 0;
  auto rel = [&](const char* base, long long elem) { return (int)((reinterpret_cast<const bf16_t*>(base) - im.base) + elem); };
  bool imaged[MMDEER_NUM_PARAMS] = {};
  for (int i = 0; images && i < kNumImages; ++i) {
    const ImageRange& r = kImages[i];
    imaged[r.pid] = true;
    AdamImaged& M = im.m[im.n++];
    M.param = reinterpret_cast<float*>(a->params[r.pid]) + (long long)r.row0 * r.cols(); M.off = r.off();
    M.rows = r.rows; M.cols = r.cols(); M.cols_pad = (r.cols() + 63) / 64 * 64; M.lr = a->lr[r.pid];
    M.frag = M.fragT = M.wt = M.rowpad = M.hm = -1;
    if (r.img & IMG_FRAG) { M.frag = rel(L.wfpack, r.s_off()); M.frag_nkt = r.cols() / 64; M.frag_row0 = r.s_row(); }
    if ((r.img & IMG_FRAGT) && wt_on) { M.fragT = rel(L.wtfpack, r.s_off()); M.fragT_nkt = r.s_rows / 64; M.fragT_col0 = r.s_row(); }
    if ((r.img & IMG_WT) && wt_on) { M.wt = rel(L.wtpack, kParams[r.wt_pid].off); M.wt_ld = r.wt_ld; M.wt_col0 = r.wt_col(); }
    if (r.img & IMG_PAD) { M.rowpad = rel(L.wa_pad, 0); M.rowpad_ld = AUD_PAD; M.frag = rel(L.wa_frag, 0); M.frag_nkt = AUD_PAD / 64; M.frag_row0 = r.row0; }
    if (r.img & IMG_HM) { M.hm = rel(L.wqkv_hm, 0); M.hm_row0 = r.row0; }
  }
  for (int i = 0; i < MMDEER_NUM_PARAMS; ++i) {
    if (imaged[i]) continue;
    const int k = t.nseg++;
    t.param[k] = reinterpret_cast<float*>(a->params[i]);
    t.off[k] = kParams[i].off;
    t.n[k] = kParams[i].rows * kParams[i].cols;
    t.is_vec[k] = kParams[i].is_matrix ? 0 : 1;
    t.lr[k] = a->lr[i];
  }
  t.grads = a->grads; t.exp_avg = a->exp_avg; t.exp_avg_sq = a->exp_avg_sq;
  t.partials = L.wscratch;
  t.norm_out = a->grad_norm;
  t.flat_elems = MMDEER_FLAT_ELEMS;
  t.beta1 = a->beta1; t.beta2 = a->beta2; t.eps = a->eps; t.weight_decay = a->weight_decay;
  t.bias_corr1 = 1.f - powf(a->beta1, (float)a->step);
  t.bias_corr2 = 1.f - powf(a->beta2, (float)a->step);
  t.max_norm = a->max_grad_norm; t.grad_scale = a->grad_scale;
  if (images) return launch_adamw_pack_images(t, im, reinterpret_cast<bf16_t*>(L.wpack), L.vpack, s);
  TRY(launch_adamw_pack(t, L.wpack, f32, L.vpack, s));
  if (f32) { if (a->pack_transposed) TRY(pack_transposed_weights(cparams, L, f32, s)); }
  else TRY(repack_images(L, a->pack_transposed != 0, s));
  return 0;
}

int mmdeer_pack_weights(const void* const* params, void* weights, size_t weights_bytes, int compute_f32, void* stream) {
  const int f32 = compute_f32 ? 1 : 0;
  MMDEER_CHECK(params != nullptr, "pack_weights: params is NULL");
  TRY(check_weights(weights, weights_bytes, f32));
  TRY(check_params(params, "pack_weights"));
  return pack_params(params, make_layout(nullptr, weights, 0, f32), f32, (hipStream_t)stream);
}

int mmdeer_loss_stats(const void* workspace, size_t workspace_bytes, int batch, int compute_f32, float* out, void* stream) {
  static_assert(MMDEER_GLOBAL_STATS == NIG_GLOBAL_STATS, "public header out of sync with nig.h");
  MMDEER_CHECK(workspace && out, "loss_stats: NULL argument");
  MMDEER_CHECK(batch > 0, "loss_stats: batch must be > 0 (got %d)", batch);
  const Layout L = make_layout(const_cast<void*>(workspace), nullptr, batch, compute_f32 ? 1 : 0);
  MMDEER_CHECK(workspace_bytes >= L.bytes, "loss_stats: workspace of %zu bytes is smaller than the %zu of this batch", workspace_bytes, L.bytes);
  return launch_nig_stats_sum(L.stats, batch, out, make_plan(batch, compute_f32 ? 1 : 0, 0, false, false, false).nwp, (hipStream_t)stream);
}

}
```

Measured before the change: 15.22 million samples/s.

## Fold NIG loss statistics in-kernel with last-arriver atomic reduction

```diff
diff --git a/uncertainty-aware-multimodal-emotion-recognition_amd/csrc/chain.h b/uncertainty-aware-multimodal-emotion-recognition_amd/csrc/chain.h
--- a/uncertainty-aware-multimodal-emotion-recognition_amd/csrc/chain.h
+++ b/uncertainty-aware-multimodal-emotion-recognition_amd/csrc/chain.h
@@ -53,7 +53,6 @@
   const float* stats;
   const float* gstats;
   int nblk;
-  int nwp;
   bf16_t* dz2;
   float* partial_w;
   float* partial_b;
@@ -72,6 +71,9 @@
   float* nig_out;
   const float* targets;
   float* wstats;
+  float* stats;
+  float* sums;
+  unsigned* arrive;
 };
 
 struct ChainArgs {
@@ -85,6 +87,7 @@
   DropCtx drop;
   const bf16_t* aux_video; const bf16_t* aux_audio; bf16_t* aux_audio_pad;
   int aux_ldv, aux_lda;
+  unsigned* zero; int zero_n;
   unsigned long long* stamps;
   ChainNig nig;
   ChainNigF nigf;
diff --git a/uncertainty-aware-multimodal-emotion-recognition_amd/csrc/chain.hip b/uncertainty-aware-multimodal-emotion-recognition_amd/csrc/chain.hip
--- a/uncertainty-aware-multimodal-emotion-recognition_amd/csrc/chain.hip
+++ b/uncertainty-aware-multimodal-emotion-recognition_amd/csrc/chain.hip
@@ -102,6 +102,7 @@
   int nseg, nvec;
   DropCtx drop;
   unsigned long long* stamps;
+  unsigned* zero; int zero_n;
   const bf16_t* aux_video; const bf16_t* aux_audio; bf16_t* aux_audio_pad;
   int aux_ldv, aux_lda;
   ChainRecK rec[CHAIN_MAX_SEGS];
@@ -247,7 +248,7 @@
   }
   const int stat_n = g.gstats ? (int)g.gstats[3 * NIG_NSTAT] : B;
   NSTAMP(111);
-  compute_finals(g.gstats ? g.gstats : g.stats, g.gstats ? 1 : g.nblk, stat_n, g.cfg, F, gs, ftmp, g.gstats ? 0 : g.nwp);
+  compute_finals(g.gstats ? g.gstats : g.stats, g.gstats ? 1 : g.nblk, stat_n, g.cfg, F, gs, ftmp);
   NSTAMP(112);
   if (blockIdx.x == 0 && tid == 0) write_loss(F, g.loss_out, g.bin_counts);
   if (quad_on) {
@@ -340,6 +341,7 @@
     const float y = g.targets[(long long)bc * 3 + d];
     const Terms t = loss_terms(n, y);
     float* slab = g.wstats + ((long long)((row0 >> 4) + blk) * 3 + d) * NIG_NSTAT;
+    float mine = 0.f;
     float v[NIG_NSTAT];
     v[0] = writer ? t.logprob : 0.f; v[1] = writer ? t.reg : 0.f; v[2] = writer ? t.kla : 0.f; v[3] = writer ? t.klb : 0.f; v[4] = writer ? t.u : 0.f;
 #pragma unroll
@@ -350,9 +352,45 @@
 #pragma unroll
     for (int i = 0; i < NIG_NSTAT; ++i) {
       const float sm = wave_sum(v[i]);
-      if (lane == 0) slab[i] = sm;
-    }
-  }
+      mine = lane == i ? sm : mine;
+    }
+    if (lane < NIG_NSTAT) store_wt4(slab + lane, mine);
+  }
+}
+
+template <int MS>
+__device__ __forceinline__ void chain_nig_fold(const ChainNigF& g, float* scratch, int row0, int B, int tid) {
+  constexpr int NV = 3 * NIG_NSTAT, GW = NIG_ROWS / MS;
+  unsigned* const last = reinterpret_cast<unsigned*>(scratch);
+  float (*gs)[NIG_NSTAT] = reinterpret_cast<float (*)[NIG_NSTAT]>(scratch + 4);
+  float* const upper = scratch + 4 + NV + 3;
+  const int blk = row0 / NIG_ROWS, nblk = (B + NIG_ROWS - 1) / NIG_ROWS, nwg = (B + MS - 1) / MS, nwp = (B + 15) >> 4;
+  const int here = nwg - blk * GW < GW ? nwg - blk * GW : GW;
+  asm volatile("s_waitcnt vmcnt(0)" ::: "memory");
+  __syncthreads();
+  if (tid == 0) *last = arrive(g.arrive + 1 + blk) == (unsigned)(here - 1);
+  __syncthreads();
+  if (!*last) return;
+  if (tid < NV) {
+    float w[4];
+#pragma unroll
+    for (int z = 0; z < 4; ++z) {
+      const int wp = 4 * blk + z;
+      w[z] = load_dev(g.wstats + (long long)(wp < nwp ? wp : nwp - 1) * NV + tid);
+    }
+#pragma unroll
+    for (int z = 0; z < 4; ++z) w[z] = 4 * blk + z < nwp ? w[z] : 0.f;
+    store_wt4(g.stats + (long long)blk * NV + tid, (w[0] + w[1]) + (w[2] + w[3]));
+  }
+  asm volatile("s_waitcnt vmcnt(0)" ::: "memory");
+  __syncthreads();
+  if (tid == 0) *last = arrive(g.arrive) == (unsigned)(nblk - 1);
+  __syncthreads();
+  if (!*last) return;
+  sum_partials<true>(g.stats, nblk, gs, upper);
+  __syncthreads();
+  if (tid < NV) g.sums[tid] = gs[tid / NIG_NSTAT][tid % NIG_NSTAT];
+  if (tid == NV) g.sums[NV] = (float)B;
 }
 
 template <int D, int VECF, int TS>
@@ -388,6 +426,7 @@
 #endif
   stamp(0);
 
+  if (blockIdx.x == 0 && tid < a.zero_n) a.zero[tid] = 0u;
   const unsigned long long dseed = a.drop.seed;
   const unsigned long long doff = a.drop.offset + (a.drop.offset_dev ? *a.drop.offset_dev : 0ull);
   const unsigned dthresh = a.drop.thresh;
@@ -841,7 +880,13 @@
     }
     stamp(5 + 3 * si);
   }
-  if (a.nigf.enabled) chain_nig_tail<MS>(a.nigf, pin, row0, B, tid);
+  if (a.nigf.enabled) {
+    stamp(120);
+    chain_nig_tail<MS>(a.nigf, pin, row0, B, tid);
+    stamp(121);
+    if (a.nigf.targets) chain_nig_fold<MS>(a.nigf, reinterpret_cast<float*>(lds + RED), row0, B, tid);
+    stamp(122);
+  }
   asm volatile("s_waitcnt vmcnt(0)" ::: "memory");
 }
 
@@ -963,13 +1008,16 @@
   k.aux_video = a.aux_video; k.aux_audio = a.aux_audio; k.aux_audio_pad = a.aux_audio_pad; k.aux_ldv = a.aux_ldv; k.aux_lda = a.aux_lda;
   k.X = a.X; k.ldx = a.ldx; k.K0 = a.K0; k.B = a.B; k.groups = a.groups; k.group_stride = a.group_stride; k.drop = a.drop;
   k.stamps = a.stamps;
+  MMDEER_CHECK(a.zero_n >= 0 && a.zero_n <= 512 && (a.zero_n == 0 || a.zero), "chain: at most 512 words to zero (got %d)", a.zero_n);
+  k.zero = a.zero; k.zero_n = a.zero_n;
   k.nig = a.nig;
   k.nigf = a.nigf;
   if (a.nigf.enabled) {
     const ChainSeg& last = a.seg[a.nseg - 1];
     MMDEER_CHECK(!a.nig.enabled && last.end_layer && last.nout == 192 && !last.gamma && !last.lnb_gamma && last.fold_groups == 0,
                  "chain: the NIG tail needs a plain 192-wide last layer");
-    MMDEER_CHECK(a.nigf.w3 && a.nigf.b3 && a.nigf.evid && a.nigf.nig_out && (!a.nigf.targets || a.nigf.wstats) &&
+    MMDEER_CHECK(a.nigf.w3 && a.nigf.b3 && a.nigf.evid && a.nigf.nig_out &&
+                     (!a.nigf.targets || (a.nigf.wstats && a.nigf.stats && a.nigf.sums && a.nigf.arrive)) &&
                      ((uintptr_t)a.nigf.w3 % 16) == 0 && ((uintptr_t)a.nigf.evid % 16) == 0,
                  "chain: NIG tail: NULL argument / alignment");
   }
diff --git a/uncertainty-aware-multimodal-emotion-recognition_amd/csrc/common.h b/uncertainty-aware-multimodal-emotion-recognition_amd/csrc/common.h
--- a/uncertainty-aware-multimodal-emotion-recognition_amd/csrc/common.h
+++ b/uncertainty-aware-multimodal-emotion-recognition_amd/csrc/common.h
@@ -19,6 +19,17 @@
 __device__ __forceinline__ void store_wt16(void* p, V4 v) {
   static_assert(sizeof(V4) == 16, "store_wt16 writes 16 bytes");
   asm volatile("global_store_dwordx4 %0, %1, off sc0 sc1\n\ts_nop 1" ::"v"(p), "v"(v) : "memory");
+}
+
+typedef __attribute__((address_space(1))) unsigned dev_u32;
+__device__ __forceinline__ void store_wt4(float* p, float v) {
+  asm volatile("global_store_dword %0, %1, off sc0 sc1" ::"v"(p), "v"(v) : "memory");
+}
+__device__ __forceinline__ float load_dev(const float* p) {
+  return __uint_as_float(__hip_atomic_load((const dev_u32*)p, __ATOMIC_RELAXED, __HIP_MEMORY_SCOPE_AGENT));
+}
+__device__ __forceinline__ unsigned arrive(unsigned* counter) {
+  return __hip_atomic_fetch_add((dev_u32*)counter, 1u, __ATOMIC_RELAXED, __HIP_MEMORY_SCOPE_AGENT);
 }
 
 enum { DT_BF16 = 0, DT_F32 = 1 };
diff --git a/uncertainty-aware-multimodal-emotion-recognition_amd/csrc/layout.inc b/uncertainty-aware-multimodal-emotion-recognition_amd/csrc/layout.inc
--- a/uncertainty-aware-multimodal-emotion-recognition_amd/csrc/layout.inc
+++ b/uncertainty-aware-multimodal-emotion-recognition_amd/csrc/layout.inc
@@ -13,7 +13,8 @@
 X(S, ACT, pool, Bz * FUS, 0) X(S, ACT, y_t3, Bz * FUS, 0) X(S, ACT, tri, Bz * FUS, 0) X(S, ACT, y_o1, Bz * FUS, 0) X(S, ACT, fused, Bz * FUS, 0)
 X(S, ACT, h1, Bz * HID, 0) X(S, ACT, h2, Bz * HID, 0) X(S, ACT, e1, Bz * 3 * EV1, 0) X(S, ACT, e2, Bz * 3 * EV2, 0)
 X(S, F32, probs, Bz * 8 * 4, 0) X(S, F32, evid, Bz * 12, 0)
-X(S, F32, stats, 4 * nblk * 3 * NIG_NSTAT, 0)
+X(S, F32, stats, nblk * 3 * NIG_NSTAT, 0)
+X(S, F32, nigsum, 3 * nblk * 3 * NIG_NSTAT, 0)
 X(S, F32, mean_a2, Bz, 0) X(S, F32, rstd_a2, Bz, 0) X(S, F32, mean_t3, Bz, 0) X(S, F32, rstd_t3, Bz, 0) X(S, F32, mean_o1, Bz, 0) X(S, F32, rstd_o1, Bz, 0)
 X(S, ACT, dz2, Bz * 3 * EV2, 0) X(S, ACT, de1, Bz * 3 * EV1, 0) X(S, ACT, dh2, Bz * HID, 0) X(S, ACT, dh1, Bz * HID, 0)
 X(S, ACT, dfused, Bz * FUS, 0) X(S, ACT, dz_o1, Bz * FUS, 0) X(S, ACT, dtri, Bz * FUS, 0) X(S, ACT, dz_t3, Bz * FUS, 0)
diff --git a/uncertainty-aware-multimodal-emotion-recognition_amd/csrc/nig.h b/uncertainty-aware-multimodal-emotion-recognition_amd/csrc/nig.h
--- a/uncertainty-aware-multimodal-emotion-recognition_amd/csrc/nig.h
+++ b/uncertainty-aware-multimodal-emotion-recognition_amd/csrc/nig.h
@@ -7,6 +7,8 @@
 
 constexpr int NIG_NSTAT = 35;
 constexpr int NIG_GLOBAL_STATS = 3 * NIG_NSTAT + 1;
+constexpr int NIG_ARRIVE_WORD = 128;
+static_assert(NIG_ARRIVE_WORD >= NIG_GLOBAL_STATS && NIG_ARRIVE_WORD + 2 <= 3 * 3 * NIG_NSTAT, "nigsum holds both for every nblk >= 1");
 constexpr int NIG_LOSS_OUT = 20;
 
 struct LossCfg {
@@ -24,9 +26,9 @@
 int launch_nig_bwd(const void* e2, const void* w3, const float* evid, const float* targets, const float* stats,
                    const float* gstats, const float* gmu, const float* gnu, const float* galpha, const float* gbeta,
                    float* devid, void* dz2, float* partial_w, float* partial_b, float* loss_out, int* bin_counts,
-                   int B, int act_f32, float mask_scale, const LossCfg& cfg, int nwp, hipStream_t s);
+                   int B, int act_f32, float mask_scale, const LossCfg& cfg, hipStream_t s);
 
-int launch_nig_stats_sum(const float* stats, int B, float* out, int nwp, hipStream_t s);
+int launch_nig_stats_sum(const float* stats, int B, float* out, hipStream_t s);
 
 int launch_nig_loss_stats(const float* gamma, const float* nu, const float* alpha, const float* beta,
                           const float* targets, float* stats, int B, hipStream_t s);
diff --git a/uncertainty-aware-multimodal-emotion-recognition_amd/csrc/nig.hip b/uncertainty-aware-multimodal-emotion-recognition_amd/csrc/nig.hip
--- a/uncertainty-aware-multimodal-emotion-recognition_amd/csrc/nig.hip
+++ b/uncertainty-aware-multimodal-emotion-recognition_amd/csrc/nig.hip
@@ -59,7 +59,7 @@
                                                       const float* stats, const float* gstats, const float* gmu,
                                                       const float* gnu, const float* galpha, const float* gbeta, float* devid, void* dz2,
                                                       float* partial_w, float* partial_b, float* loss_out,
-                                                      int* bin_counts, int B, float mask_scale, LossCfg cfg, int nwp) {
+                                                      int* bin_counts, int B, float mask_scale, LossCfg cfg) {
   __shared__ float gs[3][NIG_NSTAT];
   __shared__ float ftmp[NIG_FINALS_TMP];
   __shared__ f32x4 sdE[NIG_ROWS];
@@ -84,7 +84,7 @@
     const float y = targets[o];
     GSTAMP(1);
     const int stat_n = gstats ? (int)gstats[3 * NIG_NSTAT] : B;
-    compute_finals(gstats ? gstats : stats, gstats ? 1 : nblk, stat_n, cfg, F, gs, ftmp, gstats ? 0 : nwp);
+    compute_finals(gstats ? gstats : stats, gstats ? 1 : nblk, stat_n, cfg, F, gs, ftmp);
     GSTAMP(2);
     if (blockIdx.x == 0 && blockIdx.y == 0 && tid == 0) write_loss(F, loss_out, bin_counts);
     const Nig n = nig_act(ev);
@@ -338,25 +338,20 @@
   return 0;
 }
 
-__global__ __launch_bounds__(128) void nig_stats_sum_kernel(const float* stats, int nblk, int B, float* out, int nwp) {
+__global__ __launch_bounds__(128) void nig_stats_sum_kernel(const float* stats, int nblk, int B, float* out) {
   const int i = threadIdx.x;
   if (i < 3 * NIG_NSTAT) {
     float acc = 0.f;
-    for (int p = 0; p < nblk; ++p) {
-      if (nwp == 0) { acc += stats[(long long)p * 3 * NIG_NSTAT + i]; continue; }
-      float w[4];
-      for (int z = 0; z < 4; ++z) w[z] = 4 * p + z < nwp ? stats[(long long)(4 * p + z) * 3 * NIG_NSTAT + i] : 0.f;
-      acc += (w[0] + w[1]) + (w[2] + w[3]);
-    }
+    for (int p = 0; p < nblk; ++p) acc += stats[(long long)p * 3 * NIG_NSTAT + i];
     out[i] = acc;
   } else if (i == 3 * NIG_NSTAT) {
     out[i] = (float)B;
   }
 }
 
-int launch_nig_stats_sum(const float* stats, int B, float* out, int nwp, hipStream_t s) {
+int launch_nig_stats_sum(const float* stats, int B, float* out, hipStream_t s) {
   MMDEER_CHECK(B > 0, "nig statistics need a non-empty batch");
-  hipLaunchKernelGGL(nig_stats_sum_kernel, dim3(1), dim3(128), 0, s, stats, nig_nblocks(B), B, out, nwp);
+  hipLaunchKernelGGL(nig_stats_sum_kernel, dim3(1), dim3(128), 0, s, stats, nig_nblocks(B), B, out);
   MMDEER_HIP(hipGetLastError());
   return 0;
 }
@@ -364,15 +359,15 @@
 int launch_nig_bwd(const void* e2, const void* w3, const float* evid, const float* targets, const float* stats,
                    const float* gstats, const float* gmu, const float* gnu, const float* galpha, const float* gbeta,
                    float* devid, void* dz2, float* partial_w, float* partial_b, float* loss_out, int* bin_counts,
-                   int B, int act_f32, float mask_scale, const LossCfg& cfg, int nwp, hipStream_t s) {
+                   int B, int act_f32, float mask_scale, const LossCfg& cfg, hipStream_t s) {
   MMDEER_CHECK(B > 0, "nig backward needs a non-empty batch");
   dim3 grid(nig_nblocks(B), 3);
   if (act_f32)
     hipLaunchKernelGGL(nig_bwd_kernel<true>, grid, dim3(256), 0, s, e2, w3, evid, targets, stats, gstats, gmu, gnu, galpha, gbeta,
-                       devid, dz2, partial_w, partial_b, loss_out, bin_counts, B, mask_scale, cfg, nwp);
+                       devid, dz2, partial_w, partial_b, loss_out, bin_counts, B, mask_scale, cfg);
   else
     hipLaunchKernelGGL(nig_bwd_kernel<false>, grid, dim3(256), 0, s, e2, w3, evid, targets, stats, gstats, gmu, gnu, galpha, gbeta,
-                       devid, dz2, partial_w, partial_b, loss_out, bin_counts, B, mask_scale, cfg, nwp);
+                       devid, dz2, partial_w, partial_b, loss_out, bin_counts, B, mask_scale, cfg);
   MMDEER_HIP(hipGetLastError());
   return 0;
 }
diff --git a/uncertainty-aware-multimodal-emotion-recognition_amd/csrc/nig_dev.h b/uncertainty-aware-multimodal-emotion-recognition_amd/csrc/nig_dev.h
--- a/uncertainty-aware-multimodal-emotion-recognition_amd/csrc/nig_dev.h
+++ b/uncertainty-aware-multimodal-emotion-recognition_amd/csrc/nig_dev.h
@@ -102,56 +102,38 @@
   int counts[3][10];
 };
 
+template <bool DEV>
+__device__ __forceinline__ void sum_partials(const float* stats, int nblk, float (*gs)[NIG_NSTAT], float* upper) {
+  constexpr int NV = 3 * NIG_NSTAT;
+  const int i = threadIdx.x & 127, h = threadIdx.x >> 7;
+  float acc = 0.f;
+  if (i < NV) {
+    const int per = (nblk + 1) >> 1, p0 = h * per, p1 = (p0 + per < nblk) ? p0 + per : nblk;
+    for (int q = p0; q < p1; q += 16) {
+      float v[16];
+#pragma unroll
+      for (int u = 0; u < 16; ++u) {
+        const int p = q + u < p1 ? q + u : p1 - 1;
+        const float* src = stats + (long long)p * NV + i;
+        if constexpr (DEV) v[u] = load_dev(src); else v[u] = *src;
+      }
+#pragma unroll
+      for (int u = 0; u < 16; ++u) v[u] = q + u < p1 ? v[u] : 0.f;
+      acc += ((v[0] + v[1]) + (v[2] + v[3])) + ((v[4] + v[5]) + (v[6] + v[7])) +
+             (((v[8] + v[9]) + (v[10] + v[11])) + ((v[12] + v[13]) + (v[14] + v[15])));
+    }
+    if (h == 1) upper[i] = acc;
+  }
+  __syncthreads();
+  if (h == 0 && i < NV) gs[i / NIG_NSTAT][i % NIG_NSTAT] = acc + upper[i];
+}
+
 constexpr int NIG_FINALS_TMP = 3 * NIG_NSTAT + 30 + 3 + 3;
 __device__ __forceinline__ void compute_finals(const float* stats, int nblk, int B, const LossCfg& cfg, Finals& F,
-                                               float (*gs)[NIG_NSTAT], float* tmp, int nwp = 0) {
+                                               float (*gs)[NIG_NSTAT], float* tmp) {
   constexpr int NV = 3 * NIG_NSTAT;
   float* const upper = tmp; float* const ece_c = tmp + NV; float* const dim_total = ece_c + 30; float* const ubar_s = dim_total + 3;
-  {
-    const int i = threadIdx.x & 127, h = threadIdx.x >> 7;
-    float acc = 0.f;
-    if (i < NV) {
-      const int per = (nblk + 1) >> 1, p0 = h * per, p1 = (p0 + per < nblk) ? p0 + per : nblk;
-      if (nwp == 0) {
-        for (int q = p0; q < p1; q += 16) {
-          float v[16];
-#pragma unroll
-          for (int u = 0; u < 16; ++u) {
-            const int p = q + u < p1 ? q + u : p1 - 1;
-            v[u] = stats[(long long)p * NV + i];
-          }
-#pragma unroll
-          for (int u = 0; u < 16; ++u) v[u] = q + u < p1 ? v[u] : 0.f;
-          acc += ((v[0] + v[1]) + (v[2] + v[3])) + ((v[4] + v[5]) + (v[6] + v[7])) +
-                 (((v[8] + v[9]) + (v[10] + v[11])) + ((v[12] + v[13]) + (v[14] + v[15])));
-        }
-      } else {
-        for (int q = p0; q < p1; q += 16) {
-          float w[16][4];
-#pragma unroll
-          for (int u = 0; u < 16; ++u)
-#pragma unroll
-            for (int z = 0; z < 4; ++z) {
-              const int p = q + u < p1 ? q + u : p1 - 1, wp = 4 * p + z;
-              w[u][z] = stats[(long long)(wp < nwp ? wp : nwp - 1) * NV + i];
-            }
-          float v[16];
-#pragma unroll
-          for (int u = 0; u < 16; ++u) {
-            const int p = q + u < p1 ? q + u : p1 - 1;
-#pragma unroll
-            for (int z = 0; z < 4; ++z) w[u][z] = 4 * p + z < nwp ? w[u][z] : 0.f;
-            v[u] = q + u < p1 ? (w[u][0] + w[u][1]) + (w[u][2] + w[u][3]) : 0.f;
-          }
-          acc += ((v[0] + v[1]) + (v[2] + v[3])) + ((v[4] + v[5]) + (v[6] + v[7])) +
-                 (((v[8] + v[9]) + (v[10] + v[11])) + ((v[12] + v[13]) + (v[14] + v[15])));
-        }
-      }
-      if (h == 1) upper[i] = acc;
-    }
-    __syncthreads();
-    if (h == 0 && i < NV) gs[i / NIG_NSTAT][i % NIG_NSTAT] = acc + upper[i];
-  }
+  sum_partials<false>(stats, nblk, gs, upper);
   GSTAMP(8);
   __syncthreads();
   GSTAMP(9);
diff --git a/uncertainty-aware-multimodal-emotion-recognition_amd/csrc/stackc.hip b/uncertainty-aware-multimodal-emotion-recognition_amd/csrc/stackc.hip
--- a/uncertainty-aware-multimodal-emotion-recognition_amd/csrc/stackc.hip
+++ b/uncertainty-aware-multimodal-emotion-recognition_amd/csrc/stackc.hip
@@ -146,7 +146,6 @@
   bool chains;
   bool in_chain;
   bool nig_tail;
-  int nwp;
   bool bchain, dchain;
   bool nigfold;
 };
@@ -155,7 +154,6 @@
   p.chains = !f32 && opt(OPT_CHAIN) && B >= opt(OPT_CHAIN_MIN) && B <= opt(OPT_CHAIN_MAX);
   p.in_chain = p.chains && opt(OPT_CHAIN_IN) && inputs_bf16 && chain_samples_per_workgroup(B) == 16;
   p.nig_tail = p.chains && opt(OPT_CHAIN_NIGF);
-  p.nwp = p.nig_tail ? (B + 15) / 16 : 0;
   const bool bwd = p.chains && opt(OPT_CHAIN_BWD);
   p.bchain = bwd && !g_fused;
   p.dchain = bwd && phase == 0;
@@ -589,6 +587,9 @@
     X.fwd_seg(c, n.aout);
     X.fwd_seg(c, n.avf);
     X.fwd_seg(c, n.avp);
+    if (plan.nig_tail && a->targets) {
+      c.zero = reinterpret_cast<unsigned*>(L.nigsum + NIG_ARRIVE_WORD); c.zero_n = 1 + nig_nblocks(B);
+    }
     TRY(launch_chain(c, s));
     MARK(plan.in_chain ? "chain F1-F6 (input projections + audio-visual fusion)" : "chain F2-F6 (audio-visual fusion)");
   } else {
@@ -630,7 +631,9 @@
       ChainNigF& g = c.nigf;
       g.enabled = 1;
       g.w3 = reinterpret_cast<const bf16_t*>(X.W(P_EV2_W)); g.b3 = X.V(P_EV2_B); g.b3_stride = 64;
-      g.evid = L.evid; g.nig_out = a->nig_out; g.targets = a->targets; g.wstats = L.stats;
+      g.evid = L.evid; g.nig_out = a->nig_out; g.targets = a->targets;
+      g.wstats = reinterpret_cast<float*>(L.dqkv); g.stats = L.stats; g.sums = L.nigsum;
+      g.arrive = reinterpret_cast<unsigned*>(L.nigsum + NIG_ARRIVE_WORD);
     }
 #ifdef MMDEER_STAMPS
     c.stamps = reinterpret_cast<unsigned long long*>(L.slab);
@@ -706,9 +709,10 @@
   };
 
   if (phase != 2) {
+  const float* const gstats = !a->targets ? nullptr : a->global_stats ? a->global_stats : plan.nig_tail ? L.nigsum : nullptr;
   if (!plan.nigfold)
-    TRY(launch_nig_bwd(L.e2, X.W(P_EV2_W), L.evid, a->targets, L.stats, a->targets ? a->global_stats : nullptr, a->g_mu, a->g_nu, a->g_alpha, a->g_beta, nullptr,
-                       L.dz2, L.part_w3, L.part_b3, a->loss_out, a->bin_counts, B, f32, X.mask_scale, cfg, plan.nwp, s));
+    TRY(launch_nig_bwd(L.e2, X.W(P_EV2_W), L.evid, a->targets, L.stats, gstats, a->g_mu, a->g_nu, a->g_alpha, a->g_beta, nullptr,
+                       L.dz2, L.part_w3, L.part_b3, a->loss_out, a->bin_counts, B, f32, X.mask_scale, cfg, s));
   if (!plan.nigfold) MARK("nig_bwd (head's last layer backward + loss gradient)");
   if (plan.bchain) {
     ChainArgs c = X.chain(n.ev1.dout, n.ev1.heads * n.ev1.N, 1, 0);
@@ -723,7 +727,7 @@
       ChainNig& g = c.nig;
       g.enabled = 1;
       g.e2 = reinterpret_cast<const bf16_t*>(L.e2); g.w3 = reinterpret_cast<const bf16_t*>(X.W(P_EV2_W)); g.evid = L.evid;
-      g.targets = a->targets; g.stats = L.stats; g.gstats = a->global_stats; g.nblk = nblk; g.nwp = plan.nwp;
+      g.targets = a->targets; g.stats = L.stats; g.gstats = gstats; g.nblk = nblk;
       g.dz2 = reinterpret_cast<bf16_t*>(L.dz2); g.partial_w = L.part_w3; g.partial_b = L.part_b3;
       g.loss_out = a->loss_out; g.bin_counts = a->bin_counts; g.mask_scale = X.mask_scale; g.cfg = cfg;
     }
@@ -869,7 +873,7 @@
   MMDEER_CHECK(batch > 0, "loss_stats: batch must be > 0 (got %d)", batch);
   const Layout L = make_layout(const_cast<void*>(workspace), nullptr, batch, compute_f32 ? 1 : 0);
   MMDEER_CHECK(workspace_bytes >= L.bytes, "loss_stats: workspace of %zu bytes is smaller than the %zu of this batch", workspace_bytes, L.bytes);
-  return launch_nig_stats_sum(L.stats, batch, out, make_plan(batch, compute_f32 ? 1 : 0, 0, false, false, false).nwp, (hipStream_t)stream);
-}
-
-}
+  return launch_nig_stats_sum(L.stats, batch, out, (hipStream_t)stream);
+}
+
+}
```

Result: no change. 15.22 million samples/s, median of 2 (-0.0%).
